# taylorlu/voicepuppet

Hardware: AMD Instinct MI355X
Metric: PixReferNet G+D step frames/sec @256x256 bs=32 (higher is better)
Workload: dtype bf16; 1 GPU; PixReferNet G+D training step (G + 3xD + VGG16-conv3_3 perceptual + TF-Adam x2), 256x256, ngf=ndf=64, global batch 32 = 32 per GPU; global_batch=32, per_gpu_batch=32, parallelism=dp1

## Files before the change

include/vp_hip.h:

```cpp
#ifndef VP_HIP_H_
#define VP_HIP_H_

#include <stddef.h>
#include <stdint.h>

#ifdef __cplusplus
extern "C" {
#endif

enum vp_status { VP_OK = 0, VP_ERR_ARG = -1, VP_ERR_HIP = -2, VP_ERR_WORKSPACE = -3, VP_ERR_STATE = -4 };
enum vp_dtype { VP_F32 = 0, VP_BF16 = 1 };
enum vp_act { VP_ACT_NONE = 0, VP_ACT_LRELU = 1, VP_ACT_RELU = 2, VP_ACT_TANH = 3, VP_ACT_SIGMOID = 4, VP_ACT_RELU6 = 5, VP_ACT_LEAKY = 6 };

int vp_version(void);
const char* vp_last_error(void);

typedef struct vp_pixrefer_desc {
  int batch;
  int height;
  int ngf, ndf;
  int dtype;
  int training;
  float l1_weight;
  float gan_weight;
// ... 97 lines not shown
  int batch, samples;
} vp_logmel_desc;
typedef struct vp_logmel vp_logmel_t;
size_t vp_logmel_workspace_bytes(const vp_logmel_desc* d);
int vp_logmel_frames(const vp_logmel_desc* d);
int vp_logmel_create(const vp_logmel_desc* d, void* workspace, size_t workspace_bytes, void* stream, vp_logmel_t** out);
void vp_logmel_destroy(vp_logmel_t* h);
int vp_logmel_forward(vp_logmel_t* h, const float* pcm, float* out, void* stream);

typedef struct vp_bfmnet_desc {
  int batch;
  int frames;
  int num_mel_bins;
  int trunk_dtype;
} vp_bfmnet_desc;
typedef struct vp_bfmnet vp_bfmnet_t;
size_t vp_bfmnet_param_count(void);
int vp_bfmnet_param_info(int index, char* name, int name_cap, size_t* offset, int* ndim, int64_t shape[4]);
size_t vp_bfmnet_workspace_bytes(const vp_bfmnet_desc* d);
int vp_bfmnet_create(const vp_bfmnet_desc* d, void* workspace, size_t workspace_bytes, const float* params,
                     void* stream, vp_bfmnet_t** out);
void vp_bfmnet_destroy(vp_bfmnet_t* h);
int vp_bfmnet_params_changed(vp_bfmnet_t* h);
int vp_bfmnet_forward(vp_bfmnet_t* h, const float* ears, const float* mfccs, const int* seq_len, float* out, void* stream);
int vp_bfmnet_set_decoder_dropout(vp_bfmnet_t* h, const float* mask0, const float* mask1);
int vp_bfmnet_tensor(vp_bfmnet_t* h, const char* name, void** ptr, int64_t shape[4]);

typedef struct vp_bfmstream_desc {
  int struct_bytes;
  int max_chunk_frames;
  int num_mel_bins;
  int trunk_dtype;
  int sample_rate;
  float lower_hz, upper_hz;
} vp_bfmstream_desc;
size_t vp_bfmstream_desc_size(void);
typedef struct vp_bfmstream vp_bfmstream_t;
int vp_bfmstream_context(const vp_bfmstream_desc* d, int* left_mel, int* right_mel, int* left_frames, int* right_frames, int* window_frames);
long long vp_bfmstream_frames_after(const vp_bfmstream_desc* d, long long samples, int finished);
size_t vp_bfmstream_workspace_bytes(const vp_bfmstream_desc* d);
int vp_bfmstream_create(const vp_bfmstream_desc* d, void* workspace, size_t workspace_bytes, const float* params, void* stream,
                        vp_bfmstream_t** out);
void vp_bfmstream_destroy(vp_bfmstream_t* h);
int vp_bfmstream_params_changed(vp_bfmstream_t* h);
int vp_bfmstream_reset(vp_bfmstream_t* h, void* stream);
int vp_bfmstream_ready(const vp_bfmstream_t* h, long long n_new_samples);
int vp_bfmstream_ready_finish(const vp_bfmstream_t* h);
int vp_bfmstream_push(vp_bfmstream_t* h, const float* pcm, long long n, const float* ears, float* coeff_out, void* stream);
int vp_bfmstream_finish(vp_bfmstream_t* h, const float* ears, float* coeff_out, void* stream);
int vp_bfmstream_tensor(vp_bfmstream_t* h, const char* name, void** ptr, int64_t shape[4]);
#define VP_BFMSTREAM_GROUP_MAX_SLOTS 128
typedef struct vp_bfmstream_group_desc {
  int struct_bytes;
  int slots;
  int max_chunk_frames;
  int num_mel_bins;
  int trunk_dtype;
  int sample_rate;
  float lower_hz, upper_hz;
} vp_bfmstream_group_desc;
size_t vp_bfmstream_group_desc_size(void);
typedef struct vp_bfmstream_group vp_bfmstream_group_t;
size_t vp_bfmstream_group_workspace_bytes(const vp_bfmstream_group_desc* d);
int vp_bfmstream_group_plan_info(const vp_bfmstream_group_desc* d, int bucket, int gemm, int info[8]);
int vp_bfmstream_group_create(const vp_bfmstream_group_desc* d, void* workspace, size_t workspace_bytes, const float* params, void* stream,
                              vp_bfmstream_group_t** out);
void vp_bfmstream_group_destroy(vp_bfmstream_group_t* h);
int vp_bfmstream_group_params_changed(vp_bfmstream_group_t* h);
int vp_bfmstream_group_reset_slot(vp_bfmstream_group_t* h, int slot, void* stream);
long long vp_bfmstream_group_ready(const vp_bfmstream_group_t* h, const long long* n, const int* finish, int* k);
int vp_bfmstream_group_push(vp_bfmstream_group_t* h, const float* pcm, const long long* n, const int* finish, const float* ears, float* coeff_out,
                            void* stream);
int vp_bfmstream_group_tensor(vp_bfmstream_group_t* h, const char* name, void** ptr, int64_t shape[4]);
int vp_gru_seq_state(const float* xg, const float* xc, const float* whg, const float* whc, float* hstate, float* out, int b, int t, int t0,
                     int n, void* stream);

int vp_maxpool2x2_fwd(const void* x, void* y, int n, int h, int w, int c, int dtype, void* stream);
int vp_maxpool2x2_bwd(const void* x, const void* dy, void* dx, int n, int h, int w, int c, int dtype, void* stream);
int vp_maxpool2x2_bwd_code(const void* code, const void* dy, void* dx, int n, int h, int w, int c, int dtype, void* stream);
int vp_composite_fwd(const float* gen_out4, const float* targets, float* out4, float* outputs, float* outputs_fg, int n, int hw,
                     void* stream);
int vp_gan_loss(const float* logits, void* seed_d, void* seed_g, float* predict, float* losses, int m, float gan_weight, int dtype,
                void* stream);
int vp_dwconv7x3_bn_act(const float* x, const float* w, const float* bias, float* y, int b, int h, int wd, int c, void* stream);
int vp_dwconv7x3_bn_act_t(const void* x, const float* w, const float* bias, void* y, int dtype, int b, int h, int wd, int c, void* stream);
int vp_conv_first_fwd(const float* x, const float* w, const float* bias, float* y, int b, int h, int w_in, int cout, void* stream);
size_t vp_dwproj_workspace_bytes(int ce, int cout);
int vp_dwproj_fwd(const float* ex, const float* w_dw, const float* b_dw, const float* w_proj, const float* b_proj, float* y, int add, int b, int h,
                  int w, int ce, int cout, void* workspace, void* stream);
int vp_maxpool_hw(const float* x, float* y, int b, int h, int w, int c, int kh, int kw, int sh, int sw, void* stream);
int vp_gru_seq(const float* xg, const float* xc, const float* whg, const float* whc, const int* seq_len, float* out, int b, int t,
               void* stream);

size_t vp_render_colors_workspace_bytes(int batch, int h, int w);
int vp_render_colors(unsigned char* image, unsigned char* face_mask, const float* vertices, const int* triangles,
                     const float* colors, float* depth_buffer, int ntri, int nver, int h, int w, int c, int batch,
                     void* workspace, void* stream);

typedef struct vp_bfm_model {
  int nver, ntri;
  const double* meanshape;
  const double* idBase;
  const double* exBase;
  const double* meantex;
  const double* texBase;
  const int* tri;
  const int* point_buf;
  double center[3];
  double focal, image_center;
  double sh[5];
} vp_bfm_model;
size_t vp_bfm_reconstruct_workspace_bytes(int nver, int ntri, int frames);
int vp_bfm_reconstruct(const vp_bfm_model* m, const float* coeff, const double* rotation, int frames, int shared_texture,
                       double* face_shape, double* face_texture, double* face_color, double* face_projection, double* z_buffer,
                       float* vertices, float* colors, void* workspace, size_t workspace_bytes, void* stream);
int vp_bfm_reconstruct_rows(const vp_bfm_model* m, const float* coeff, const double* rotation, int frames, const int* tex_src, int textures,
                            const int* tex_row, float* vertices, float* colors, void* workspace, size_t workspace_bytes, void* stream);

size_t vp_bn_train_workspace_bytes(size_t pixels, int c);
int vp_bn_train_fwd(const float* x, size_t pixels, int c, const float* beta, float eps, float* mean, float* var, float* rstd, float* scale,
                    float* shift, void* workspace, void* stream);
int vp_bn_train_bwd(const float* x, const float* dz, size_t pixels, int c, const float* mean, const float* rstd, float* dx, float* dbeta,
                    void* workspace, void* stream);
int vp_bn_act_train_bwd(const float* x, const float* da, size_t pixels, int c, const float* mean, const float* rstd, const float* shift, int act,
                        float* dx, float* dbeta, void* workspace, void* stream);
int vp_affine_act_fwd(const float* x, const float* scale, const float* shift, const float* mask, size_t pixels, int c, int act, float* y, void* stream);
int vp_affine_act_add_fwd(const float* x, const float* scale, const float* shift, const float* mask, const float* add, size_t pixels, int c, int act,
                          float* y, void* stream);
int vp_act_bwd(const float* dy, const float* ya, const float* mask, size_t n, int act, float* dx, void* stream);
int vp_dwconv7x3_raw(const float* x, const float* w, float* y, int b, int h, int wd, int c, void* stream);
int vp_dwconv7x3_bwd_data(const float* dy, const float* w, float* dx, int b, int h, int wd, int c, void* stream);
size_t vp_dwconv7x3_wgrad_workspace_bytes(int b, int h, int wd, int c);
int vp_dwconv7x3_wgrad(const float* x, const float* dy, float* dw, int b, int h, int wd, int c, void* workspace, void* stream);
int vp_maxpool_hw_bwd(const float* x, const float* dy, float* dx, int b, int h, int w, int c, int kh, int kw, int sh, int sw, void* stream);
int vp_stem_im2col(const float* x, float* col, int b, int h, int w, void* stream);
int vp_gru_train_fwd(const float* xg, const float* xc, const float* whg, const float* whc, const int* seq_len, float* out, float* r, float* u, float* c,
                     float* hprev, int b, int t, void* stream);
int vp_colsum_f32(const float* x, int rows, int cols, float* out, void* stream);
int vp_gru_split_recurrent(const float* gates_kernel, const float* cand_kernel, float* whg, float* whc, float* whg_t, float* whc_t, void* stream);
int vp_mul_f32(const float* a, const float* b, float* out, size_t n, void* stream);
int vp_add_ears_f32(float* out, const float* ears, int rows, void* stream);
int vp_gru_train_bwd(const float* dout, const float* whg_t, const float* whc_t, const int* seq_len, const float* r, const float* u, const float* c,
                     const float* hprev, float* dag, float* dac, int b, int t, void* stream);
int vp_vertex_loss_partials(int b, int j);
int vp_bfm_vertex_loss(const float* d, const float* vmask, const int* seq_len, int b, int t, int j, float* gd, double* partial, void* stream);
int vp_sumsq_partials(size_t n);
int vp_sumsq(const float* x, size_t n, double* partial, void* stream);
int vp_l2_regulariser(const float* params, const float* mask, float* grads, size_t n, float scale, double* partial, void* stream);
int vp_sum_f64(const double* partial, int n, double scale, const double* add, double* out, void* stream);
int vp_bfm_step_report(const double* loss_data, const double* reg, double half_l2, const double* sumsq, double* out3, void* stream);
int vp_clip_scale_f32(float* grads, size_t n, const double* sumsq, float clip, void* stream);
int vp_adam_tf_clipped(float* params, float* grads, float* m, float* v, size_t n, const float* lr_t, const double* sumsq, float clip, float beta1,
                       float beta2, float eps, void* stream);
int vp_moving_update(float* moving, const float* batch, const float* factor, size_t n, float decay, void* stream);

size_t vp_mm_workspace_bytes(int P, int K, int N);
int vp_mm_fwd_f32(const float* x, int ldx, const float* w, int ldw, int w_transposed, const float* bias, float* y, int ldy,
                  int P, int K, int N, void* workspace, void* stream);
int vp_mm_bwd_data_f32(const float* dy, int lddy, const float* w, int ldw, int w_transposed, float* dx, int lddx, int accumulate,
                       int P, int K, int N, void* workspace, void* stream);
int vp_mm_bwd_weight_f32(const float* x, int ldx, const float* dy, int lddy, float* dw, int P, int K, int k_real, int N,
                         void* workspace, void* stream);
size_t vp_mm_packed_bytes(int P, int K, int N, int dir);
size_t vp_mm_pack_desc_bytes(void);
int vp_mm_pack_desc(size_t w_off, int ldw, int w_transposed, int P, int K, int N, int dir, size_t dst_off, void* desc);
int vp_mm_pack_table(const void* device_descs, int n, const float* master, void* packed, void* stream);
// ... 81 lines not shown
```

voicepuppet_amd/_lib.py:

```python
import ctypes
import os

_HERE = os.path.dirname(os.path.abspath(__file__))
LIB_PATH = os.environ.get("VP_LIB", os.path.join(_HERE, "libvp_hip.so"))

VP_F32, VP_BF16 = 0, 1
ACT_NONE, ACT_LRELU, ACT_RELU, ACT_TANH, ACT_SIGMOID = 0, 1, 2, 3, 4


class PixReferDesc(ctypes.Structure):
  _fields_ = [("batch", ctypes.c_int), ("height", ctypes.c_int), ("ngf", ctypes.c_int), ("ndf", ctypes.c_int),
              ("dtype", ctypes.c_int), ("training", ctypes.c_int), ("l1_weight", ctypes.c_float),
              ("gan_weight", ctypes.c_float), ("per_sample_bn", ctypes.c_int),
              ("streams", ctypes.c_int), ("d_backward_fork", ctypes.c_int), ("d_beside_vgg", ctypes.c_int)]


class ConvDesc(ctypes.Structure):
  _fields_ = [("kind", ctypes.c_int), ("n", ctypes.c_int), ("h", ctypes.c_int), ("w", ctypes.c_int),
              ("cin", ctypes.c_int), ("cout", ctypes.c_int), ("ksize", ctypes.c_int), ("stride", ctypes.c_int),
              ("pad", ctypes.c_int), ("dtype", ctypes.c_int), ("in_act", ctypes.c_int), ("out_act", ctypes.c_int)]


class LogMelDesc(ctypes.Structure):
  _fields_ = [("sample_rate", ctypes.c_int), ("num_mel_bins", ctypes.c_int), ("win_length", ctypes.c_int),
# ... 112 lines not shown
    "vp_adam_tf": (ctypes.c_int, [_P, _P, _P, _P, ctypes.c_size_t, ctypes.c_int, ctypes.c_float, ctypes.c_float,
                                  ctypes.c_float, ctypes.c_float, _P]),
    "vp_conv_workspace_bytes": (ctypes.c_size_t, [ctypes.POINTER(ConvDesc)]),
    "vp_conv_fwd": (ctypes.c_int, [ctypes.POINTER(ConvDesc), _P, _P, _P, _P, _P, _P, _P, _P]),
    "vp_conv_bwd_data": (ctypes.c_int, [ctypes.POINTER(ConvDesc), _P, _P, _P, _P, _P]),
    "vp_conv_bwd_weight": (ctypes.c_int, [ctypes.POINTER(ConvDesc), _P, _P, _P, _P, _P, _P, _P]),
    "vp_conv3x3_c64_bwd_data_pooled_workspace_bytes": (ctypes.c_size_t, [ctypes.POINTER(ConvDesc)]),
    "vp_conv3x3_c64_bwd_data_pooled": (ctypes.c_int, [ctypes.POINTER(ConvDesc), _P, _P, _P, _P, _P, _P, ctypes.c_int, _P]),
    "vp_bn_workspace_bytes": (ctypes.c_size_t, [ctypes.c_int, ctypes.c_int, ctypes.c_int]),
    "vp_bn_stats": (ctypes.c_int, [_P, ctypes.c_int, ctypes.c_int, ctypes.c_int, _P, _P, ctypes.c_float, _P, _P, _P, _P, _P, _P]),
    "vp_logmel_workspace_bytes": (ctypes.c_size_t, [ctypes.POINTER(LogMelDesc)]),
    "vp_logmel_frames": (ctypes.c_int, [ctypes.POINTER(LogMelDesc)]),
    "vp_logmel_create": (ctypes.c_int, [ctypes.POINTER(LogMelDesc), _P, ctypes.c_size_t, _P, ctypes.POINTER(_P)]),
    "vp_logmel_destroy": (None, [_P]),
    "vp_logmel_forward": (ctypes.c_int, [_P, _P, _P, _P]),
    "vp_bfmnet_param_count": (ctypes.c_size_t, []),
    "vp_bfmnet_param_info": (ctypes.c_int, [ctypes.c_int, ctypes.c_char_p, ctypes.c_int, ctypes.POINTER(ctypes.c_size_t),
                                            ctypes.POINTER(ctypes.c_int), ctypes.POINTER(ctypes.c_int64)]),
    "vp_bfmnet_workspace_bytes": (ctypes.c_size_t, [ctypes.POINTER(BfmNetDesc)]),
    "vp_bfmnet_create": (ctypes.c_int, [ctypes.POINTER(BfmNetDesc), _P, ctypes.c_size_t, _P, _P, ctypes.POINTER(_P)]),
    "vp_bfmnet_destroy": (None, [_P]),
    "vp_bfmnet_params_changed": (ctypes.c_int, [_P]),
    "vp_bfmnet_forward": (ctypes.c_int, [_P, _P, _P, _P, _P, _P]),
    "vp_bfmnet_set_decoder_dropout": (ctypes.c_int, [_P, _P, _P]),
    "vp_bfmnet_tensor": (ctypes.c_int, [_P, ctypes.c_char_p, ctypes.POINTER(_P), ctypes.POINTER(ctypes.c_int64)]),
    "vp_bfmstream_desc_size": (ctypes.c_size_t, []),
    "vp_bfmstream_context": (ctypes.c_int, [ctypes.POINTER(BfmStreamDesc)] + [ctypes.POINTER(ctypes.c_int)] * 5),
    "vp_bfmstream_frames_after": (ctypes.c_longlong, [ctypes.POINTER(BfmStreamDesc), ctypes.c_longlong, ctypes.c_int]),
    "vp_bfmstream_workspace_bytes": (ctypes.c_size_t, [ctypes.POINTER(BfmStreamDesc)]),
    "vp_bfmstream_create": (ctypes.c_int, [ctypes.POINTER(BfmStreamDesc), _P, ctypes.c_size_t, _P, _P, ctypes.POINTER(_P)]),
    "vp_bfmstream_destroy": (None, [_P]),
    "vp_bfmstream_params_changed": (ctypes.c_int, [_P]),
    "vp_bfmstream_reset": (ctypes.c_int, [_P, _P]),
    "vp_bfmstream_ready": (ctypes.c_int, [_P, ctypes.c_longlong]),
    "vp_bfmstream_ready_finish": (ctypes.c_int, [_P]),
    "vp_bfmstream_push": (ctypes.c_int, [_P, _P, ctypes.c_longlong, _P, _P, _P]),
    "vp_bfmstream_finish": (ctypes.c_int, [_P, _P, _P, _P]),
    "vp_bfmstream_tensor": (ctypes.c_int, [_P, ctypes.c_char_p, ctypes.POINTER(_P), ctypes.POINTER(ctypes.c_int64)]),
    "vp_bfmstream_group_desc_size": (ctypes.c_size_t, []),
    "vp_puppet_desc_size": (ctypes.c_size_t, []),
    "vp_puppet_workspace_bytes": (ctypes.c_size_t, [ctypes.POINTER(PuppetDesc)]),
    "vp_puppet_create": (ctypes.c_int, [ctypes.POINTER(PuppetDesc), _P, ctypes.c_size_t, _P, ctypes.POINTER(_P)]),
    "vp_puppet_destroy": (None, [_P]),
    "vp_puppet_attach": (ctypes.c_int, [_P, ctypes.c_int, _P, _P, _P, ctypes.c_int, ctypes.c_int, ctypes.c_int, _P]),
    "vp_puppet_set_backgrounds": (ctypes.c_int, [_P, _P, ctypes.c_int]),
    "vp_puppet_splice": (ctypes.c_int, [_P, _P, ctypes.c_int, _P, ctypes.c_int, _P, _P]),
    "vp_puppet_condition": (ctypes.c_int, [_P, _P, ctypes.c_int, _P, ctypes.c_int, _P, _P, _P, _P]),
    "vp_puppet_tensor": (ctypes.c_int, [_P, ctypes.c_char_p, ctypes.POINTER(_P), ctypes.POINTER(ctypes.c_int64)]),
    "vp_puppet_slot_info": (ctypes.c_int, [_P, ctypes.c_int, ctypes.POINTER(ctypes.c_int)]),
    "vp_jpeg_desc_size": (ctypes.c_size_t, []),
    "vp_jpeg_workspace_bytes": (ctypes.c_size_t, [ctypes.POINTER(JpegDesc)]),
    "vp_jpeg_frame_capacity": (ctypes.c_size_t, [ctypes.POINTER(JpegDesc)]),
    "vp_jpeg_create": (ctypes.c_int, [ctypes.POINTER(JpegDesc), _P, ctypes.c_size_t, _P, ctypes.POINTER(_P)]),
    "vp_jpeg_encode": (ctypes.c_int, [_P, _P, ctypes.c_int, _P, ctypes.c_size_t, _P, _P]),
    "vp_jpeg_tensor": (ctypes.c_int, [_P, ctypes.c_char_p, ctypes.POINTER(_P), ctypes.POINTER(ctypes.c_int64)]),
    "vp_jpeg_header": (ctypes.c_int, [_P, _P, ctypes.c_size_t, ctypes.POINTER(ctypes.c_size_t)]),
    "vp_jpeg_destroy": (None, [_P]),
    "vp_pcmin_desc_size": (ctypes.c_size_t, []),
    "vp_pcmin_ratio": (ctypes.c_int, [ctypes.c_int, ctypes.c_int] + [ctypes.POINTER(ctypes.c_int)] * 4),
    "vp_pcmin_bank": (ctypes.c_int, [ctypes.c_int, ctypes.c_int, _P]),
    "vp_pcmin_samples_after": (ctypes.c_longlong, [ctypes.c_int, ctypes.c_int, ctypes.c_longlong, ctypes.c_int]),
    "vp_pcmin_workspace_bytes": (ctypes.c_size_t, [ctypes.POINTER(PcmInDesc)]),
    "vp_pcmin_create": (ctypes.c_int, [ctypes.POINTER(PcmInDesc), _P, ctypes.c_size_t, _P, ctypes.POINTER(_P)]),
    "vp_pcmin_destroy": (None, [_P]),
    "vp_pcmin_open_slot": (ctypes.c_int, [_P, ctypes.c_int, ctypes.c_int, ctypes.c_int, ctypes.c_int, _P]),
    "vp_pcmin_ready": (ctypes.c_longlong, [_P, ctypes.POINTER(ctypes.c_longlong), ctypes.POINTER(ctypes.c_int), ctypes.POINTER(ctypes.c_longlong)]),
    "vp_pcmin_push": (ctypes.c_int, [_P, _P, ctypes.POINTER(ctypes.c_longlong), ctypes.POINTER(ctypes.c_int), _P, _P]),
    "vp_bfm_reconstruct_rows": (ctypes.c_int, [ctypes.POINTER(BfmModel), _P, _P, ctypes.c_int, _P, ctypes.c_int, _P, _P, _P, _P, ctypes.c_size_t, _P]),
    "vp_bfmstream_group_workspace_bytes": (ctypes.c_size_t, [ctypes.POINTER(BfmStreamGroupDesc)]),
    "vp_bfmstream_group_plan_info": (ctypes.c_int, [ctypes.POINTER(BfmStreamGroupDesc), ctypes.c_int, ctypes.c_int, ctypes.POINTER(ctypes.c_int)]),
    "vp_bfmstream_group_create": (ctypes.c_int, [ctypes.POINTER(BfmStreamGroupDesc), _P, ctypes.c_size_t, _P, _P, ctypes.POINTER(_P)]),
    "vp_bfmstream_group_destroy": (None, [_P]),
    "vp_bfmstream_group_params_changed": (ctypes.c_int, [_P]),
    "vp_bfmstream_group_reset_slot": (ctypes.c_int, [_P, ctypes.c_int, _P]),
    "vp_bfmstream_group_ready": (ctypes.c_longlong, [_P, ctypes.POINTER(ctypes.c_longlong), ctypes.POINTER(ctypes.c_int), ctypes.POINTER(ctypes.c_int)]),
    "vp_bfmstream_group_push": (ctypes.c_int, [_P, _P, ctypes.POINTER(ctypes.c_longlong), ctypes.POINTER(ctypes.c_int), _P, _P, _P]),
    "vp_bfmstream_group_tensor": (ctypes.c_int, [_P, ctypes.c_char_p, ctypes.POINTER(_P), ctypes.POINTER(ctypes.c_int64)]),
    "vp_gru_seq_state": (ctypes.c_int, [_P, _P, _P, _P, _P, _P, ctypes.c_int, ctypes.c_int, ctypes.c_int, ctypes.c_int, _P]),
    "vp_maxpool2x2_fwd": (ctypes.c_int, [_P, _P, ctypes.c_int, ctypes.c_int, ctypes.c_int, ctypes.c_int, ctypes.c_int, _P]),
    "vp_maxpool2x2_bwd": (ctypes.c_int, [_P, _P, _P, ctypes.c_int, ctypes.c_int, ctypes.c_int, ctypes.c_int, ctypes.c_int, _P]),
    "vp_maxpool2x2_bwd_code": (ctypes.c_int, [_P, _P, _P, ctypes.c_int, ctypes.c_int, ctypes.c_int, ctypes.c_int, ctypes.c_int, _P]),
    "vp_composite_fwd": (ctypes.c_int, [_P, _P, _P, _P, _P, ctypes.c_int, ctypes.c_int, _P]),
    "vp_gan_loss": (ctypes.c_int, [_P, _P, _P, _P, _P, ctypes.c_int, ctypes.c_float, ctypes.c_int, _P]),
    "vp_dwconv7x3_bn_act": (ctypes.c_int, [_P, _P, _P, _P, ctypes.c_int, ctypes.c_int, ctypes.c_int, ctypes.c_int, _P]),
    "vp_dwconv7x3_bn_act_t": (ctypes.c_int, [_P, _P, _P, _P] + [ctypes.c_int] * 5 + [_P]),
    "vp_conv_first_fwd": (ctypes.c_int, [_P, _P, _P, _P] + [ctypes.c_int] * 4 + [_P]),
    "vp_dwproj_workspace_bytes": (ctypes.c_size_t, [ctypes.c_int, ctypes.c_int]),
    "vp_dwproj_fwd": (ctypes.c_int, [_P] * 6 + [ctypes.c_int] * 6 + [_P, _P]),
    "vp_maxpool_hw": (ctypes.c_int, [_P, _P, ctypes.c_int, ctypes.c_int, ctypes.c_int, ctypes.c_int, ctypes.c_int, ctypes.c_int, ctypes.c_int,
                                     ctypes.c_int, _P]),
    "vp_gru_seq": (ctypes.c_int, [_P, _P, _P, _P, _P, _P, ctypes.c_int, ctypes.c_int, _P]),
    "vp_bfm_reconstruct_workspace_bytes": (ctypes.c_size_t, [ctypes.c_int, ctypes.c_int, ctypes.c_int]),
    "vp_bfm_reconstruct": (ctypes.c_int, [_P, _P, _P, ctypes.c_int, ctypes.c_int, _P, _P, _P, _P, _P, _P, _P, _P, ctypes.c_size_t, _P]),
    "vp_render_colors_workspace_bytes": (ctypes.c_size_t, [ctypes.c_int, ctypes.c_int, ctypes.c_int]),
    "vp_render_colors": (ctypes.c_int, [_P, _P, _P, _P, _P, _P, ctypes.c_int, ctypes.c_int, ctypes.c_int, ctypes.c_int, ctypes.c_int,
                                        ctypes.c_int, _P, _P]),
    "vp_bn_train_workspace_bytes": (ctypes.c_size_t, [ctypes.c_size_t, ctypes.c_int]),
    "vp_bn_train_fwd": (ctypes.c_int, [_P, ctypes.c_size_t, ctypes.c_int, _P, ctypes.c_float, _P, _P, _P, _P, _P, _P, _P]),
    "vp_bn_train_bwd": (ctypes.c_int, [_P, _P, ctypes.c_size_t, ctypes.c_int, _P, _P, _P, _P, _P, _P]),
    "vp_affine_act_fwd": (ctypes.c_int, [_P, _P, _P, _P, ctypes.c_size_t, ctypes.c_int, ctypes.c_int, _P, _P]),
    "vp_affine_act_add_fwd": (ctypes.c_int, [_P, _P, _P, _P, _P, ctypes.c_size_t, ctypes.c_int, ctypes.c_int, _P, _P]),
    "vp_act_bwd": (ctypes.c_int, [_P, _P, _P, ctypes.c_size_t, ctypes.c_int, _P, _P]),
    "vp_dwconv7x3_raw": (ctypes.c_int, [_P, _P, _P, ctypes.c_int, ctypes.c_int, ctypes.c_int, ctypes.c_int, _P]),
    "vp_dwconv7x3_bwd_data": (ctypes.c_int, [_P, _P, _P, ctypes.c_int, ctypes.c_int, ctypes.c_int, ctypes.c_int, _P]),
    "vp_dwconv7x3_wgrad_workspace_bytes": (ctypes.c_size_t, [ctypes.c_int, ctypes.c_int, ctypes.c_int, ctypes.c_int]),
    "vp_bn_act_train_bwd": (ctypes.c_int, [_P, _P, ctypes.c_size_t, ctypes.c_int, _P, _P, _P, ctypes.c_int, _P, _P, _P, _P]),
    "vp_l2_regulariser": (ctypes.c_int, [_P, _P, _P, ctypes.c_size_t, ctypes.c_float, _P, _P]),
    "vp_adam_tf_clipped": (ctypes.c_int, [_P, _P, _P, _P, ctypes.c_size_t, _P, _P, ctypes.c_float, ctypes.c_float, ctypes.c_float, ctypes.c_float, _P]),
    "vp_moving_update": (ctypes.c_int, [_P, _P, _P, ctypes.c_size_t, ctypes.c_float, _P]),
    "vp_dwconv7x3_wgrad": (ctypes.c_int, [_P, _P, _P, ctypes.c_int, ctypes.c_int, ctypes.c_int, ctypes.c_int, _P, _P]),
    "vp_maxpool_hw_bwd": (ctypes.c_int, [_P, _P, _P] + [ctypes.c_int] * 8 + [_P]),
    "vp_stem_im2col": (ctypes.c_int, [_P, _P, ctypes.c_int, ctypes.c_int, ctypes.c_int, _P]),
    "vp_gru_train_fwd": (ctypes.c_int, [_P] * 10 + [ctypes.c_int, ctypes.c_int, _P]),
    "vp_gru_train_bwd": (ctypes.c_int, [_P] * 10 + [ctypes.c_int, ctypes.c_int, _P]),
    "vp_colsum_f32": (ctypes.c_int, [_P, ctypes.c_int, ctypes.c_int, _P, _P]),
    "vp_gru_split_recurrent": (ctypes.c_int, [_P] * 7),
    "vp_mul_f32": (ctypes.c_int, [_P, _P, _P, ctypes.c_size_t, _P]),
    "vp_add_ears_f32": (ctypes.c_int, [_P, _P, ctypes.c_int, _P]),
    "vp_vertex_loss_partials": (ctypes.c_int, [ctypes.c_int, ctypes.c_int]),
    "vp_bfm_vertex_loss": (ctypes.c_int, [_P, _P, _P, ctypes.c_int, ctypes.c_int, ctypes.c_int, _P, _P, _P]),
    "vp_sumsq_partials": (ctypes.c_int, [ctypes.c_size_t]),
    "vp_sum_f64": (ctypes.c_int, [_P, ctypes.c_int, ctypes.c_double, _P, _P, _P]),
    "vp_bfm_step_report": (ctypes.c_int, [_P, _P, ctypes.c_double, _P, _P, _P]),
    "vp_clip_scale_f32": (ctypes.c_int, [_P, ctypes.c_size_t, _P, ctypes.c_float, _P]),
    "vp_sumsq": (ctypes.c_int, [_P, ctypes.c_size_t, _P, _P]),
    "vp_bn_bwd": (ctypes.c_int, [_P, _P, _P, ctypes.c_int, ctypes.c_int, ctypes.c_int, _P, _P, _P, _P, _P, _P, _P]),
}

_lib = None


def lib():
  global _lib
  if _lib is None:
    if not os.path.exists(LIB_PATH):
      raise RuntimeError("libvp_hip.so is missing (%s): run `python -c 'import __graft_entry__ as g; g.build()'` "
                         "or `make -C voicepuppet_amd/csrc`.  There is no CPU fallback." % LIB_PATH)
    try:
      import torch
    except ImportError:
      pass
    l = ctypes.CDLL(LIB_PATH)
    for name, (res, args) in _SIGNATURES.items():
      try:
        fn = getattr(l, name)
      except AttributeError:
        if "VP_LIB" not in os.environ:
          raise
        continue
      fn.restype = res
      fn.argtypes = args
    if hasattr(l, "vp_pixrefer_desc_size") and l.vp_pixrefer_desc_size.argtypes is not None:
      want = int(l.vp_pixrefer_desc_size())
      if want != ctypes.sizeof(PixReferDesc):
        raise RuntimeError("%s: vp_pixrefer_desc is %d bytes in the library, %d in this binding" % (LIB_PATH, want, ctypes.sizeof(PixReferDesc)))
    if hasattr(l, "vp_bfmstream_desc_size") and l.vp_bfmstream_desc_size.argtypes is not None:
      want = int(l.vp_bfmstream_desc_size())
      if want != ctypes.sizeof(BfmStreamDesc):
        raise RuntimeError("%s: vp_bfmstream_desc is %d bytes in the library, %d in this binding" % (LIB_PATH, want, ctypes.sizeof(BfmStreamDesc)))
    if hasattr(l, "vp_bfmstream_group_desc_size") and l.vp_bfmstream_group_desc_size.argtypes is not None:
      want = int(l.vp_bfmstream_group_desc_size())
      if want != ctypes.sizeof(BfmStreamGroupDesc):
        raise RuntimeError("%s: vp_bfmstream_group_desc is %d bytes in the library, %d in this binding" % (LIB_PATH, want, ctypes.sizeof(BfmStreamGroupDesc)))
    if hasattr(l, "vp_puppet_desc_size") and l.vp_puppet_desc_size.argtypes is not None:
      want = int(l.vp_puppet_desc_size())
      if want != ctypes.sizeof(PuppetDesc):
# ... 21 lines not shown
```

voicepuppet_amd/csrc/conv_ops.h:

```cpp
#pragma once
#include <stdlib.h>
#include <string.h>

#include "launch.h"

namespace vp {

struct ConvGeomX : ConvGeom {
  int CoutT;
};

inline ConvGeomX make_geom(int kind, int ks, int stride, int pad, int N, int Hin, int Win, int Cin, int Cin_real, int Cout) {
  ConvGeomX g;
  g.kind = kind; g.ks = ks; g.stride = stride; g.pad = pad;
  g.N = N; g.Hin = Hin; g.Win = Win;
  if (kind == 0) { g.Hout = (Hin + 2 * pad - ks) / stride + 1; g.Wout = (Win + 2 * pad - ks) / stride + 1; }
  else { g.Hout = 2 * Hin; g.Wout = 2 * Win; }
  g.Cin = Cin; g.Cin_real = Cin_real; g.Cout = Cout;
  g.CoutT = Cout < 8 ? 8 : Cout;
  return g;
}

inline int kc_elems(int is_bf16) { return is_bf16 ? 32 : 16; }

// ... 11 lines not shown
    if (rows % 64 == 0) return 1;
    if (rows <= 16) return 2;
    return rows > 64 ? 0 : 1;
  }
  if (rows <= 64) return 5;
  return P > 16 ? 3 : 4;
}

constexpr int IGEMM_SPLITK_TARGET_DEFAULT = 64;
inline int& igemm_splitk_target_knob() { static int v = IGEMM_SPLITK_TARGET_DEFAULT; return v; }
inline int pick_igemm_splitk(int blocks, int nchunk) {
  const int target = igemm_splitk_target_knob();
  const int cap = plan_misc_knob(1);
  const int minchunk = plan_misc_knob(2);
  if (blocks >= 256 || blocks >= target) return 1;
  int s = (target + blocks - 1) / blocks;
  if (s > nchunk / minchunk) s = nchunk / minchunk;
  if (s > cap) s = cap;
  return s < 1 ? 1 : s;
}

inline void set_single_src(PixSrc& x, const void* p, int C, const float* a, const float* b, int act, int group_n) {
  x.ptr[0] = p; x.ptr[1] = nullptr; x.C[0] = C; x.C[1] = 0;
  x.aff_a[0] = a; x.aff_b[0] = b; x.aff_a[1] = nullptr; x.aff_b[1] = nullptr;
  x.act = act; x.group_n = group_n > 0 ? group_n : (1 << 30);
}

struct LaunchForm {
  bool bias = false, ref = false, xa_lrelu = false, xa_relu = false, x_affine = false;
  bool stats = false;
  int x_act = 0, ref_act = 0;
};

struct IgemmPlan {
  IgemmArgs a;
  int cfg;
  LaunchForm form;
  PackDesc pack;
  size_t pack_elems;
  size_t partial_bytes;
};

struct IgemmPin { int cfg, splitk; };

inline void finish_igemm(IgemmPlan& p, int rows, int is_bf16, const IgemmPin* pin = nullptr) {
  IgemmArgs& a = p.a;
  const int P = a.N * a.Hg * a.Wg;
  a.Kpad = round_up(a.ntaps * a.Cin, kc_elems(is_bf16));
  p.cfg = pick_igemm_cfg(rows, P, a.Kpad);
  if (!is_bf16 && a.ntaps == 1 && p.cfg == 0) {
    const long long b128 = (long long)((P + 127) / 128) * (rows / 128), b64 = 2 * b128;
    if (((b64 + 255) / 256) * 64 < ((b128 + 255) / 256) * 128) p.cfg = 1;
  }
  if (pin) p.cfg = pin->cfg;
  int bc, bp;
  igemm_tile(p.cfg, &bc, &bp);
  a.CoutPad = round_up(rows, bc);
  if (a.ntaps == 1) { a.log2Cin = 30; a.cin_mask = 0x3fffffff; }
  else { a.log2Cin = ilog2(a.Cin); a.cin_mask = a.Cin - 1; }
  const int blocks = ((P + bp - 1) / bp) * (a.CoutPad / bc) * a.nclass;
  a.splitk = pin ? pin->splitk : pick_igemm_splitk(blocks, a.Kpad / kc_elems(is_bf16));
  p.partial_bytes = a.splitk > 1 ? (size_t)a.nclass * a.splitk * P * a.CoutPad * sizeof(float) : 0;
  {
    const bool tc4 = p.cfg == 0 || p.cfg == 1 || p.cfg == 6 || p.cfg == 7 || p.cfg == 8 || p.cfg == 9;
    a.rowperm = (tc4 && rows % 64 == 0) ? 1 : 0;
    p.pack.perm = a.rowperm;
  }
  a.wp_rows = round_up(rows, 128);
  p.pack.rows_pad = a.wp_rows;
  p.pack.Kpad = a.Kpad;
  p.pack.kc = kc_elems(is_bf16);
  p.pack_elems = (size_t)a.nclass * a.wp_rows * a.Kpad;
}

inline int& patch_tiles_knob() { static int v = 7; return v; }
inline int& patch_small_knob() { static int v = 3; return v; }
inline int& patch_longk_knob() { static int v = 1; return v; }
inline int& patch3_knob() { static int v = 1; return v; }
inline int& wgrad_big_knob() { static int v = 1; return v; }
inline int& patch4_knob() { static int v = 1; return v; }
inline int& c64_knob() { static int v = 1; return v; }
inline int& pool_bwd_fused_knob() { static int v = 1; return v; }
inline int& cout1_knob() { static int v = 256; return v; }
inline int& wgrad1_rows_knob() { static int v = 512; return v; }
inline int& dc64_knob() { static int v = 1; return v; }
inline int& s2c64_knob() { static int v = 512; return v; }
inline int& s2c64_pair_knob() { static int v = 1; return v; }
constexpr int PATCH_MIN_BLOCKS_DEFAULT = 192;
inline int& patch_minblk_knob() { static int v = PATCH_MIN_BLOCKS_DEFAULT; return v; }

inline void patch_tile_hw(int bp, int* th, int* tw) { *th = bp == 128 ? 8 : 16; *tw = bp == 512 ? 32 : 16; }
inline int patch_tile_pixels(int bc) {
  const int k = patch_small_knob();
  if (bc == 256) return (k & 2) ? 128 : 256;
  return (k & 1) ? 256 : 512;
}

inline int patch_tile_rows(int rows, int on) {
  if ((on & 1) && rows % 256 == 0) return 256;
  if ((on & 2) && rows % 128 == 0) return 128;
  if ((on & 4) && rows % 64 == 0) return 64;
  return 0;
}

inline bool plan_patch_eligible(const IgemmPlan& p, int rows, int is_bf16, bool single_src, bool any_grid = false) {
  const int on = patch_tiles_knob();
  const int minblk = any_grid ? 0 : patch_minblk_knob();
  const IgemmArgs& a = p.a;
  const int kc = kc_elems(is_bf16);
  if (!on || !single_src || a.nclass != 1 || a.sh != 1 || a.sw != 1 || a.os != 1 || a.ntaps < 9 || a.Cin % kc || a.Cin < kc) return false;
  if (rows % 64 || a.Cout % 8 || a.ldY % 8 || a.Hg < 16 || a.Wg < 16 || a.Hof != a.Hg || a.Wof != a.Wg) return false;
  const bool p4 = patch4_knob() && is_bf16 && a.ntaps == 16 && rows % 128 == 0;
  if (!p4 && patch_longk_knob() && rows >= 512 && rows % 256 == 0 && a.ntaps * a.Cin >= 4096 && (long long)a.N * a.Hg * a.Wg >= 256 * 256) return false;
  const int bc = p4 ? 128 : patch_tile_rows(rows, on);
  if (!bc) return false;
  int th, tw;
  patch_tile_hw(p4 ? 256 : patch_tile_pixels(bc), &th, &tw);
  const long long blocks = (long long)a.N * ((a.Hg + th - 1) / th) * ((a.Wg + tw - 1) / tw) * (rows / bc);
  const long long p4min = (long long)a.ntaps * a.Cin >= 8192 ? 256 : 512;
  if (p4 && !any_grid && patch_minblk_knob() > 1) {
    if (blocks < p4min) return false;
  } else if (blocks < minblk) return false;
  if ((size_t)a.N * a.Hin * a.Win * a.Cin * (is_bf16 ? 2 : 4) >= 0x70000000ull) return false;
  int ks = 0;
  while (ks * ks < a.ntaps) ++ks;
  if (ks * ks != a.ntaps) return false;
  const int sh = a.taps[0].dh[ks] - a.taps[0].dh[0], sw = a.taps[0].dw[1] - a.taps[0].dw[0];
  if ((sh != 1 && sh != -1) || (sw != 1 && sw != -1)) return false;
  for (int t = 0; t < a.ntaps; ++t)
    if (a.taps[0].dh[t] != a.taps[0].dh[0] + (t / ks) * sh || a.taps[0].dw[t] != a.taps[0].dw[0] + (t % ks) * sw) return false;
  return true;
}
inline void plan_make_patch(IgemmPlan& p, int rows, int is_bf16) {
  IgemmArgs& a = p.a;
  const bool p4 = patch4_knob() && is_bf16 && a.ntaps == 16 && rows % 128 == 0;
  const int bc = p4 ? 128 : patch_tile_rows(rows, patch_tiles_knob());
  int ks = 0;
  while (ks * ks < a.ntaps) ++ks;
  a.kern = CK_PATCH; a.p_kw = ks;
  a.p_dhf = a.taps[0].dh[0]; a.p_dwf = a.taps[0].dw[0];
  a.p_dhs = a.taps[0].dh[ks] - a.taps[0].dh[0]; a.p_dws = a.taps[0].dw[1] - a.taps[0].dw[0];
  const int bp = p4 ? 256 : patch_tile_pixels(bc);
  p.cfg = bc == 256 ? (bp == 128 ? 15 : 10) : (bc == 128 ? (bp == 256 ? 13 : 11) : (bp == 256 ? 14 : 12));
  a.CoutPad = round_up(rows, bc);
  a.splitk = 1;
  p.partial_bytes = 0;
  a.rowperm = 1;
  p.pack.perm = 1;
  p.pack.kswap = 1;
}

inline int& patch_xcd_knob() { static int v = 0; return v; }
inline int& patch2_knob() { static int v = 1; return v; }
inline bool plan_patch2_eligible(const IgemmPlan& p, int rows, int is_bf16, int c0, int c1) {
  const IgemmArgs& a = p.a;
  const int kc = kc_elems(is_bf16);
  if (!patch2_knob() || a.nclass != 4 || a.ntaps != 4 || a.os != 2 || a.sh != 1 || a.sw != 1) return false;
  if (c0 + c1 != a.Cin || c0 % (2 * kc) || c1 % (2 * kc) || c0 < 2 * kc) return false;
  if (rows % 64 || rows > 128 || a.Cout % 8 || a.ldY % 8 || a.Hg < 16 || a.Wg < 16 || a.Hof != 2 * a.Hg || a.Wof != 2 * a.Wg) return false;
  const long long blocks = (long long)a.N * ((a.Hg + 15) / 16) * ((a.Wg + 15) / 16) * 4;
  if (blocks < patch_minblk_knob()) return false;
  const size_t cmax = c0 > c1 ? c0 : c1;
  if ((size_t)a.N * a.Hin * a.Win * cmax * (is_bf16 ? 2 : 4) >= 0x70000000ull) return false;
  for (int cls = 0; cls < 4; ++cls)
    for (int t = 0; t < 4; ++t)
      if (a.taps[cls].dh[t] != a.taps[cls].dh[3] + 1 - (t >> 1) || a.taps[cls].dw[t] != a.taps[cls].dw[3] + 1 - (t & 1)) return false;
// ... 280 lines not shown
```

voicepuppet_amd/csrc/launch.h:

```cpp
#pragma once
#include <hip/hip_runtime.h>

#include "conv_args.h"
#include "pointwise_args.h"

namespace vp {

hipError_t launch_igemm(const IgemmArgs& a, int is_bf16, int cfg, hipStream_t st);
void igemm_tile(int cfg, int* bc, int* bp);
hipError_t launch_igemm_patch(const IgemmArgs& a, int is_bf16, int bc, int bp, hipStream_t st);
bool patch3_eligible(const IgemmArgs& a, int is_bf16);
hipError_t launch_igemm_patch3(const IgemmArgs& a, int is_bf16, int bc, int bp, hipStream_t st);
bool patch4_eligible(const IgemmArgs& a, int is_bf16);
hipError_t launch_igemm_patch4(const IgemmArgs& a, hipStream_t st);
bool conv_cin8_eligible(const IgemmArgs& a, int is_bf16);
bool conv_cout8_eligible(const IgemmArgs& a, int is_bf16);
bool conv_dcout8_eligible(const IgemmArgs& a, int is_bf16);
bool conv_cout4_eligible(const IgemmArgs& a, int is_bf16);
bool conv_kernel_ok(const IgemmArgs& a, int is_bf16);
const char* conv_kernel_name(int kern);
bool conv_c64_eligible(const IgemmArgs& a, int is_bf16);
hipError_t launch_conv_c64(const IgemmArgs& a, hipStream_t st);
bool conv_dc64_eligible(const IgemmArgs& a, int is_bf16);
hipError_t launch_conv_dc64(const IgemmArgs& a, hipStream_t st);
int conv_dc64_grid(const IgemmArgs& a);
bool conv_dc256_eligible(const IgemmArgs& a, int is_bf16);
int conv_dc256_grid(const IgemmArgs& a);
hipError_t launch_conv_dc256(const IgemmArgs& a, hipStream_t st);
bool conv_s2c64_eligible(const IgemmArgs& a, int is_bf16);
int conv_s2c64_grid(const IgemmArgs& a);
int conv_s2c64_tiles_per_image(const IgemmArgs& a);
hipError_t launch_conv_s2c64(const IgemmArgs& a, hipStream_t st);
bool conv_cout1_bwd_eligible(const Cout1Args& a);
hipError_t launch_conv_cout1_bwd(const Cout1Args& a, hipStream_t st);
bool conv_cout1_wgrad_eligible(const Cout1Args& a);
hipError_t launch_conv_cout1_wgrad(const Cout1Args& a, hipStream_t st);
hipError_t launch_cout1_wgrad_prof(const Cout1Args& a, hipStream_t st);
hipError_t launch_cout1_bwd_prof(const Cout1Args& a, hipStream_t st);
hipError_t launch_igemm_patch2(const IgemmArgs& a, int is_bf16, int bc, int bp, hipStream_t st);
hipError_t launch_igemm_smallp(const IgemmArgs& a, int is_bf16, hipStream_t st);
struct SmallPArgs;
hipError_t launch_smallp(const SmallPArgs& s, int is_bf16, hipStream_t st);
hipError_t launch_smallp_fused(const SmallPArgs& s, int is_bf16, hipStream_t st);
hipError_t launch_wgrad(const WgradArgs& a, int is_bf16, int cfg, hipStream_t st);
bool wgrad_mm_eligible(const WgradArgs& a, int cfg);
hipError_t launch_wgrad_mm(const WgradArgs& a, int cfg, hipStream_t st);
hipError_t launch_wgrad_tr(const WgradArgs& a, hipStream_t st, const char** variant = nullptr, int* tile_cols = nullptr);
void wgrad_tile(int cfg, int* bm, int* bn);

void profile_enable(int on);
void profile_tag(const char* tag);
size_t profile_collect(char* out, size_t cap);

hipError_t launch_pack_weights(const PackDesc* d_descs, int ndesc, const float* master, void* packed, int is_bf16, hipStream_t st);
hipError_t launch_pack_weights_one(const PackDesc& d, const float* master, void* packed, int is_bf16, hipStream_t st);
int bn_nchunk(int Pg, int C, int G, int is_bf16);
hipError_t launch_bn_stats(const BnArgs& a, int is_bf16, hipStream_t st);
hipError_t launch_bn_finalize(const BnArgs& a, hipStream_t st);
bool bn_small(const BnArgs& a);
hipError_t launch_bn_small_fwd(const BnArgs& a, void* out_lrelu, void* out_relu, int is_bf16, hipStream_t st);
hipError_t launch_bn_small_bwd(const BnArgs& a, int is_bf16, hipStream_t st);
hipError_t launch_bn_bwd(const BnArgs& a, int is_bf16, hipStream_t st);
hipError_t launch_bn_bwd_tail(const BnArgs& a, int is_bf16, hipStream_t st);
hipError_t launch_colsum(const BnArgs& a, int creal, float* out, int accumulate, int is_bf16, hipStream_t st);
hipError_t launch_colsum_tail(const BnArgs& a, int creal, float* out, int accumulate, hipStream_t st);
hipError_t launch_act_apply(const void* y, const float* sc, const float* sh, int C, int Pg, size_t npix,
                            void* out_lrelu, void* out_relu, int is_bf16, hipStream_t st);
hipError_t launch_tap_gather(const TapArgs& a, hipStream_t st);
hipError_t launch_tap_spread(const TapArgs& a, int is_bf16, hipStream_t st);
hipError_t launch_frame_pack(const FramePackArgs& a, hipStream_t st);
hipError_t launch_pack_inputs(const PackInputsArgs& a, int is_bf16, hipStream_t st);
int composite_nblocks(int N, int HW);
hipError_t launch_composite_fwd(const CompositeArgs& a, int is_bf16, hipStream_t st);
hipError_t launch_composite_bwd(const CompositeArgs& a, int is_bf16, hipStream_t st);
hipError_t launch_gan_loss(const GanLossArgs& a, int is_bf16, hipStream_t st);
int perceptual_nblocks(size_t half, int is_bf16);
hipError_t launch_perceptual(const PerceptualArgs& a, int is_bf16, hipStream_t st);
hipError_t launch_loss_final(const LossFinalArgs& a, hipStream_t st);
hipError_t launch_maxpool_fwd(const void* x, void* y, int B, int H, int W, int C, int is_bf16, hipStream_t st);
hipError_t launch_maxpool_bwd(const void* x, const void* dy, void* dx, int B, int H, int W, int C, int is_bf16, hipStream_t st);
hipError_t launch_maxpool_bwd_code(const void* code, const void* dy, void* dx, int B, int H, int W, int C, int is_bf16, hipStream_t st);
hipError_t launch_relu_bwd(const void* y, void* d, size_t n, int is_bf16, hipStream_t st);
hipError_t launch_adam(const AdamArgs& a, hipStream_t st);
hipError_t launch_fetch(const FetchArgs& a, hipStream_t st);
hipError_t launch_grad_pack_bf16(const float* src, void* dst, size_t n, hipStream_t st);
hipError_t launch_grad_unpack_bf16(const void* src, float* dst, size_t n, float scale, hipStream_t st);

struct ConvGeom {
  int kind;
  int ks, stride, pad;
  int N, Hin, Win, Hout, Wout;
  int Cin, Cin_real;
  int Cout;
};

inline int ilog2(int v) { int l = 0; while ((1 << l) < v) ++l; return l; }
inline int round_up(int v, int m) { return (v + m - 1) / m * m; }

}
```

voicepuppet_amd/csrc/ops_api.hip:

```cpp
#include <string.h>

#include <string>

#include "conv_ops.h"
#include "errors.h"
#include "audio_args.h"
#include "launch.h"
#include "vp_common.h"

using namespace vp;

namespace {

bool conv_desc_ok(const vp_conv_desc* d) {
  if (!d || d->n < 1 || d->h < 1 || d->w < 1) return false;
  if (d->cin < 8 || (d->cin & (d->cin - 1))) return false;
  if (d->kind == 1 && (d->ksize != 4 || d->stride != 2 || d->pad != 1)) return false;
  if (d->kind != 0 && d->kind != 1) return false;
  if (d->ksize < 1 || d->ksize > 4 || d->stride < 1 || d->stride > 2) return false;
  if (d->kind == 0 && d->stride == 2 && (d->ksize != 4 || d->pad != 1 || (d->h & 1) || (d->w & 1))) return false;
  return d->dtype == VP_F32 || d->dtype == VP_BF16;
}

ConvGeomX geom_of(const vp_conv_desc* d) {
  return make_geom(d->kind, d->ksize, d->stride, d->pad, d->n, d->h, d->w, d->cin, d->cin, d->cout);
}

size_t align256(size_t v) { return (v + 255) & ~(size_t)255; }

const void* zero_page(char* ws, size_t used, hipStream_t st) {
  char* z = ws + align256(used);
  (void)hipMemsetAsync(z, 0, 256, st);
  return z;
}

}

extern "C" {

int vp_pixrefer_pack_frames(const unsigned char* example_frames, const unsigned char* current_frames, const int* crops,
                            int n, int img_size, float* inputs, float* fg_inputs, float* targets, float* masks, void* stream) {
  if (!example_frames || !current_frames || !crops || !inputs || !fg_inputs || !targets || !masks || n < 1 || img_size < 2) {
    set_err("vp_pixrefer_pack_frames: bad argument");
    return VP_ERR_ARG;
  }
  FramePackArgs a;
  a.ex = example_frames; a.cur = current_frames; a.crops = crops;
  a.inputs = inputs; a.fg_inputs = fg_inputs; a.targets = targets; a.masks = masks;
  a.N = n; a.S = img_size;
  VP_HIP_CHECK(launch_frame_pack(a, (hipStream_t)stream));
  return VP_OK;
}

extern "C" void vp_phase_marks_enable(int on);

int vp_tune(const char* key, int value) {
  if (!key) return VP_ERR_ARG;
  const std::string k(key);
  if (k == "patch_tiles") { patch_tiles_knob() = value; return VP_OK; }
  if (k == "patch_min_blocks") { patch_minblk_knob() = value < 0 ? PATCH_MIN_BLOCKS_DEFAULT : value; return VP_OK; }
  if (k == "patch_small_tiles") { patch_small_knob() = value; return VP_OK; }
  if (k == "patch_long_k_on_256") { patch_longk_knob() = value; return VP_OK; }
  if (k == "wgrad_tr") { wgrad_tr_knob() = value; return VP_OK; }
  if (k == "patch3") { patch3_knob() = value; return VP_OK; }
  if (k == "c64") { c64_knob() = value; return VP_OK; }
  if (k == "dc64") { dc64_knob() = value; return VP_OK; }
  if (k == "pool_bwd_fused") { pool_bwd_fused_knob() = value < 0 || value > 4 ? 1 : value; return VP_OK; }
  if (k == "cout1_wgrad_rows" && value > 0) { wgrad1_rows_knob() = value; return VP_OK; }
  if (k == "cout1_bwd") { cout1_knob() = value < 0 ? 256 : value; return VP_OK; }
  if (k == "s2c64") { s2c64_knob() = value; return VP_OK; }
  if (k == "wgrad_big") { wgrad_big_knob() = value; return VP_OK; }
  if (k == "patch4") { patch4_knob() = value; return VP_OK; }
  if (k == "s2c64_pair") { s2c64_pair_knob() = value; return VP_OK; }
  if (k == "bfm_dwproj") { bfm_dwproj_knob() = value; return VP_OK; }
  if (k == "patch2") { patch2_knob() = value; return VP_OK; }
  if (k == "patch_xcd") { patch_xcd_knob() = value; return VP_OK; }
  if (k == "smallp_max_pixels") { smallp_knob() = value; return VP_OK; }
  if (k == "igemm_splitk_target") { igemm_splitk_target_knob() = value < 0 ? IGEMM_SPLITK_TARGET_DEFAULT : value; return VP_OK; }
  if (k == "wgrad_fixed_x10") { wgrad_cost_knob(0) = value; return VP_OK; }
  if (k == "wgrad_slab_tile_x1000") { wgrad_cost_knob(2) = value < 0 ? 150 : value; return VP_OK; }
  if (k == "wgrad_slab_x100") { wgrad_cost_knob(1) = value; return VP_OK; }
  if (k == "smallp_split_target") { plan_misc_knob(0) = value; return VP_OK; }
  if (k == "igemm_splitk_cap") { plan_misc_knob(1) = value; return VP_OK; }
  if (k == "igemm_splitk_minchunk") { plan_misc_knob(2) = value; return VP_OK; }
  if (k == "wgrad_resident_blocks") { plan_misc_knob(3) = value; return VP_OK; }
  if (k == "igemm_small_grid") { igemm_small_grid_knob() = value; return VP_OK; }
  if (k == "thin_blocks_cout8" && value > 0) { thin_blocks_knob(0) = value; return VP_OK; }
  if (k == "thin_blocks_dcout8" && value > 0) { thin_blocks_knob(1) = value; return VP_OK; }
  if (k == "thin_blocks_cout4" && value > 0) { thin_blocks_knob(2) = value; return VP_OK; }
  if (k == "thin_blocks_cin8" && value > 0) { thin_blocks_knob(3) = value; return VP_OK; }
  if (k == "phase_marks") { vp_phase_marks_enable(value); return VP_OK; }
  set_err("vp_tune: unknown key %s", key);
  return VP_ERR_ARG;
}

static unsigned* smallp_counter_page(char* ws, size_t used, const IgemmArgs& a, hipStream_t st) {
  unsigned* c = (unsigned*)(ws + align256(used) + 256);
  (void)hipMemsetAsync(c, 0, (size_t)smallp_counters(a) * sizeof(unsigned), st);
  return c;
}

size_t vp_conv_workspace_bytes(const vp_conv_desc* d) {
  if (!conv_desc_ok(d)) return 0;
  const int bf = d->dtype == VP_BF16, es = bf ? 2 : 4;
  const ConvGeomX g = geom_of(d);
  size_t best = 0;
  {
    IgemmPlan p = plan_fwd(g, 0, bf);
    best = align256(p.pack_elems * es) + p.partial_bytes;
    plan_kernel(p, g.Cout, bf, d->cin, 0, FAM_SMALLP, LaunchForm{});
    if (p.a.kern == CK_SMALLP) {
      const size_t b = align256(p.pack_elems * es) + align256(p.partial_bytes) + 512 + (size_t)smallp_counters(p.a) * sizeof(unsigned);
      if (b > best) best = b;
    }
  }
  if ((d->cout & (d->cout - 1)) == 0 && d->cout >= 8) {
    IgemmPlan p = plan_bwd_data(g, 0, 0, d->cin, d->cin, d->cin, bf);
    size_t b = align256(p.pack_elems * es) + p.partial_bytes;
    if (b > best) best = b;
    plan_kernel(p, d->cin, bf, d->cout, 0, FAM_SMALLP, LaunchForm{});
    if (p.a.kern == CK_SMALLP) {
      b = align256(p.pack_elems * es) + align256(p.partial_bytes) + 512 + (size_t)smallp_counters(p.a) * sizeof(unsigned);
      if (b > best) best = b;
    }
    for (int plain = 0; plain < 2; ++plain) {
      WgradPlan w = plan_wgrad(g, bf, plain != 0);
      if (w.partial_bytes + 512 > best) best = w.partial_bytes + 512;
    }
  }
  return best + 1024;
}

int vp_conv_fwd(const vp_conv_desc* d, const void* x, const float* in_scale, const float* in_shift,
                const float* w, const float* bias, void* y, void* workspace, void* stream) {
  if (!conv_desc_ok(d) || !x || !w || !y || !workspace) { set_err("vp_conv_fwd: bad argument"); return VP_ERR_ARG; }
  const int bf = d->dtype == VP_BF16, es = bf ? 2 : 4;
  hipStream_t st = (hipStream_t)stream;
  const ConvGeomX g = geom_of(d);
  IgemmPlan p = plan_fwd(g, 0, bf);
  p.a.out_act = d->out_act;
  LaunchForm f;
  f.bias = bias != nullptr; f.x_affine = in_scale != nullptr; f.x_act = d->in_act;
  const bool plain = d->in_act == ACT_NONE && !in_scale;
  plan_kernel(p, g.Cout, bf, d->cin, 0, plain ? (FAM_SMALLP | FAM_PATCH | FAM_PATCH2 | (d->out_act == ACT_NONE ? FAM_S2C64 : 0)) : 0, f);
  char* ws = (char*)workspace;
  VP_HIP_CHECK(launch_pack_weights_one(p.pack, w, ws, bf, st));
  IgemmArgs a = p.a;
  set_single_src(a.x, x, d->cin, in_scale, in_shift, d->in_act, 0);
  a.Wp = ws;
  a.partial = (float*)(ws + align256(p.pack_elems * es));
  a.Y = y; a.bias = bias;
  a.zeros = zero_page(ws, align256(p.pack_elems * es) + p.partial_bytes, st);
// ... 95 lines not shown

static bool bn_ok(int pixels, int c, int dtype) {
  const int e = dtype == VP_BF16 ? 8 : 4;
  return pixels >= 1 && c >= e && c % e == 0 && 256 % (c / e) == 0 && (dtype == VP_F32 || dtype == VP_BF16);
}

int vp_bn_stats(const void* y, int pixels, int c, int dtype, const float* gamma, const float* beta, float eps,
                float* scale, float* shift, float* mean, float* rstd, void* workspace, void* stream) {
  if (!bn_ok(pixels, c, dtype) || !y || !gamma || !beta || !scale || !shift || !mean || !rstd || !workspace) {
    set_err("vp_bn_stats: bad argument");
    return VP_ERR_ARG;
  }
  BnArgs b;
  memset(&b, 0, sizeof(b));
  b.y = y; b.C = c; b.G = 1; b.Pg = pixels;
  b.nchunk = bn_nchunk(pixels, c, 1, dtype == VP_BF16);
  b.partial = (double*)workspace;
  b.gamma = gamma; b.beta = beta; b.aff_a = scale; b.aff_b = shift; b.mu = mean; b.rstd = rstd; b.eps = eps;
  VP_HIP_CHECK(launch_bn_stats(b, dtype == VP_BF16, (hipStream_t)stream));
  return VP_OK;
}

int vp_bn_bwd(const void* y, const void* dz, void* dy, int pixels, int c, int dtype, const float* gamma,
              const float* mean, const float* rstd, float* dgamma, float* dbeta, void* workspace, void* stream) {
  if (!bn_ok(pixels, c, dtype) || !y || !dz || !dy || !gamma || !mean || !rstd || !dgamma || !dbeta || !workspace) {
    set_err("vp_bn_bwd: bad argument");
    return VP_ERR_ARG;
  }
  BnArgs b;
  memset(&b, 0, sizeof(b));
  b.y = y; b.dz = dz; b.dy = dy; b.C = c; b.G = 1; b.Pg = pixels;
  b.nchunk = bn_nchunk(pixels, c, 1, dtype == VP_BF16);
  b.partial = (double*)workspace;
  float* f = (float*)((char*)workspace + (size_t)b.nchunk * 2 * c * sizeof(double));
  b.c1 = f; b.c2 = f + c;
  b.gamma = gamma; b.mu = const_cast<float*>(mean); b.rstd = const_cast<float*>(rstd);
  b.dgamma = dgamma; b.dbeta = dbeta;
  VP_HIP_CHECK(launch_bn_bwd(b, dtype == VP_BF16, (hipStream_t)stream));
  return VP_OK;
}


int vp_maxpool2x2_fwd(const void* x, void* y, int n, int h, int w, int c, int dtype, void* stream) {
  const int e = dtype == VP_BF16 ? 8 : 4;
  if (!x || !y || n < 1 || h < 2 || w < 2 || (h & 1) || (w & 1) || c < e || c % e) { set_err("vp_maxpool2x2_fwd: bad argument"); return VP_ERR_ARG; }
  VP_HIP_CHECK(launch_maxpool_fwd(x, y, n, h, w, c, dtype == VP_BF16, (hipStream_t)stream));
  return VP_OK;
}

int vp_maxpool2x2_bwd(const void* x, const void* dy, void* dx, int n, int h, int w, int c, int dtype, void* stream) {
  const int e = dtype == VP_BF16 ? 8 : 4;
  if (!x || !dy || !dx || n < 1 || h < 2 || w < 2 || (h & 1) || (w & 1) || c < e || c % e) { set_err("vp_maxpool2x2_bwd: bad argument"); return VP_ERR_ARG; }
  VP_HIP_CHECK(launch_maxpool_bwd(x, dy, dx, n, h, w, c, dtype == VP_BF16, (hipStream_t)stream));
  return VP_OK;
}

int vp_maxpool2x2_bwd_code(const void* code, const void* dy, void* dx, int n, int h, int w, int c, int dtype, void* stream) {
  const int e = dtype == VP_BF16 ? 8 : 4;
  if (!code || !dy || !dx || n < 1 || h < 2 || w < 2 || (h & 1) || (w & 1) || c < e || c % e) { set_err("vp_maxpool2x2_bwd_code: bad argument"); return VP_ERR_ARG; }
  VP_HIP_CHECK(launch_maxpool_bwd_code(code, dy, dx, n, h, w, c, dtype == VP_BF16, (hipStream_t)stream));
  return VP_OK;
}

int vp_composite_fwd(const float* gen_out4, const float* targets, float* out4, float* outputs, float* outputs_fg, int n, int hw,
                     void* stream) {
  if (!gen_out4 || !targets || !out4 || !outputs || !outputs_fg || n < 1 || hw < 1) { set_err("vp_composite_fwd: bad argument"); return VP_ERR_ARG; }
  CompositeArgs ca;
  memset(&ca, 0, sizeof(ca));
  ca.y4 = gen_out4; ca.targets = targets; ca.o4 = out4; ca.outputs = outputs; ca.outputs_fg = outputs_fg; ca.N = n; ca.HW = hw; ca.train = 0;
  VP_HIP_CHECK(launch_composite_fwd(ca, 0, (hipStream_t)stream));
  return VP_OK;
}

int vp_gan_loss(const float* logits, void* seed_d, void* seed_g, float* predict, float* losses, int m, float gan_weight, int dtype,
                void* stream) {
  if (!logits || !seed_d || !seed_g || !predict || !losses || m < 1) { set_err("vp_gan_loss: bad argument"); return VP_ERR_ARG; }
  GanLossArgs ga;
  memset(&ga, 0, sizeof(ga));
  ga.logits = logits; ga.dl_d = seed_d; ga.dl_g = seed_g; ga.predict = predict; ga.losses = losses; ga.M = m; ga.gan_weight = gan_weight;
  VP_HIP_CHECK(launch_gan_loss(ga, dtype == VP_BF16, (hipStream_t)stream));
  return VP_OK;
}

int vp_dwconv7x3_bn_act(const float* x, const float* w, const float* bias, float* y, int b, int h, int wd, int c, void* stream) {
  if (!x || !w || !bias || !y || b < 1 || h < 1 || wd < 1 || c < 4 || (c & 3)) { set_err("vp_dwconv7x3_bn_act: bad argument"); return VP_ERR_ARG; }
  VP_HIP_CHECK(launch_dwconv7x3(x, w, bias, y, 0, b, h, wd, c, (hipStream_t)stream));
  return VP_OK;
}

int vp_dwconv7x3_bn_act_t(const void* x, const float* w, const float* bias, void* y, int dtype, int b, int h, int wd, int c, void* stream) {
  if (!x || !w || !bias || !y || b < 1 || h < 1 || wd < 1 || c < 4 || (c & 3) || (dtype != VP_F32 && dtype != VP_BF16)) {
    set_err("vp_dwconv7x3_bn_act_t: bad argument"); return VP_ERR_ARG;
  }
  VP_HIP_CHECK(launch_dwconv7x3(x, w, bias, y, dtype == VP_BF16, b, h, wd, c, (hipStream_t)stream));
  return VP_OK;
}

int vp_conv_first_fwd(const float* x, const float* w, const float* bias, float* y, int b, int h, int w_in, int cout, void* stream) {
  if (!x || !w || !bias || !y || b < 1 || h < 1 || w_in < 1 || cout < 1) { set_err("vp_conv_first_fwd: bad argument"); return VP_ERR_ARG; }
  int pt, ho, pl, wo;
  same_pad(h, 9, 1, &pt, &ho);
  same_pad(w_in, 5, 2, &pl, &wo);
  VP_HIP_CHECK(launch_conv_first(x, w, bias, y, 0, b, h, w_in, wo, cout, pt, pl, (hipStream_t)stream));
  return VP_OK;
}

static IgemmPlan dwproj_pack_plan(int pixels, int ce, int cout) {
  IgemmPlan p = plan_fwd(make_geom(0, 1, 1, 0, 1, pixels, 1, ce, ce, cout), 0, 0);
  p.pack.s_ch = cout;
  p.pack.dst_off = 0;
  p.pack.perm = 0; p.a.rowperm = 0;
  return p;
}

size_t vp_dwproj_workspace_bytes(int ce, int cout) {
  if (ce < 16 || ce % 16 || cout < 1) return 0;
  return align256((size_t)22 * ce * sizeof(float)) + align256(dwproj_pack_plan(1, ce, cout).pack_elems * sizeof(float)) + 256;
}

int vp_dwproj_fwd(const float* ex, const float* w_dw, const float* b_dw, const float* w_proj, const float* b_proj, float* y, int add, int b, int h,
                  int w, int ce, int cout, void* workspace, void* stream) {
  if (!ex || !w_dw || !b_dw || !w_proj || !b_proj || !y || !workspace || b < 1 || h < 1 || w < 1) { set_err("vp_dwproj_fwd: bad argument"); return VP_ERR_ARG; }
  if (!dwproj_eligible(w, ce, cout)) {
    set_err("vp_dwproj_fwd: no kernel for mel width %d, %d expanded and %d output channels (dwproj_eligible)", w, ce, cout);
    return VP_ERR_ARG;
  }
  const size_t ex_bytes = (size_t)b * h * w * ce * sizeof(float);
  if (ex_bytes >= 0xF0000000ull) {
    set_err("vp_dwproj_fwd: the expanded tensor is %zu bytes, the kernel's 32-bit lane offsets stop below 0xF0000000 (%llu)", ex_bytes, 0xF0000000ull);
    return VP_ERR_ARG;
  }
  hipStream_t st = (hipStream_t)stream;
  float* wdw22 = (float*)workspace;
  float* packed = (float*)((char*)workspace + align256((size_t)22 * ce * sizeof(float)));
  VP_HIP_CHECK(hipMemcpyAsync(wdw22, w_dw, (size_t)21 * ce * sizeof(float), hipMemcpyDeviceToDevice, st));
  VP_HIP_CHECK(hipMemcpyAsync(wdw22 + (size_t)21 * ce, b_dw, (size_t)ce * sizeof(float), hipMemcpyDeviceToDevice, st));
  const IgemmPlan p = dwproj_pack_plan(b * h * w, ce, cout);
  VP_HIP_CHECK(launch_pack_weights_one(p.pack, w_proj, packed, 0, st));
  VP_HIP_CHECK(launch_dwproj(ex, wdw22, packed, p.a.wp_rows, b_proj, y, add ? 1 : 0, b, h, w, ce, cout, st));
  return VP_OK;
}

int vp_maxpool_hw(const float* x, float* y, int b, int h, int w, int c, int kh, int kw, int sh, int sw, void* stream) {
  if (!x || !y || b < 1 || h < 1 || w < 1 || c < 4 || (c & 3) || kh < 1 || kw < 1 || sh < 1 || sw < 1) { set_err("vp_maxpool_hw: bad argument"); return VP_ERR_ARG; }
  const int ho = (h + sh - 1) / sh, wo = (w + sw - 1) / sw;
  const int ph = (ho - 1) * sh + kh - h, pw = (wo - 1) * sw + kw - w;
  const int pt = ph > 0 ? ph / 2 : 0, pl = pw > 0 ? pw / 2 : 0;
  VP_HIP_CHECK(launch_maxpool_same(x, y, 0, 0, b, h, w, c, kh, kw, sh, sw, pt, pl, ho, wo, (hipStream_t)stream));
  return VP_OK;
}

int vp_gru_seq(const float* xg, const float* xc, const float* whg, const float* whc, const int* seq_len, float* out, int b, int t,
               void* stream) {
  if (!xg || !xc || !whg || !whc || !seq_len || !out || b < 1 || t < 1) { set_err("vp_gru_seq: bad argument"); return VP_ERR_ARG; }
  VP_HIP_CHECK(launch_gru_seq(xg, xc, whg, whc, seq_len, out, b, t, (hipStream_t)stream));
  return VP_OK;
}

int vp_gru_seq_state(const float* xg, const float* xc, const float* whg, const float* whc, float* hstate, float* out, int b, int t, int t0,
                     int n, void* stream) {
  if (!xg || !xc || !whg || !whc || !hstate || !out || b < 1 || t < 1 || t0 < 0 || n < 0 || t0 + n > t) {
    set_err("vp_gru_seq_state: bad argument"); return VP_ERR_ARG;
  }
  if (n == 0) return VP_OK;
  VP_HIP_CHECK(launch_gru_state(xg, xc, whg, whc, hstate, out, b, t, t0, n, (hipStream_t)stream));
  return VP_OK;
// ... 13 lines not shown
```

voicepuppet_amd/csrc/plan_pixrefer.hip:

```cpp
#include <math.h>
#include <stdio.h>
#include <string.h>

#include <mutex>
#include <string>
#include <utility>
#include <vector>

#include "conv_ops.h"
#include "errors.h"
#include "launch.h"
#include "smallp_args.h"
#include "vp_common.h"

namespace vp {

thread_local char g_err[512] = "";
void set_err(const char* fmt, ...) {
  va_list ap;
  va_start(ap, fmt);
  vsnprintf(g_err, sizeof(g_err), fmt, ap);
  va_end(ap);
}

// ... 28 lines not shown
  bool dz2_written = false;
  void* xa[3] = {nullptr, nullptr, nullptr};
  bool need_act[3] = {false, false, false};
  BnBuf bn{};
  int producer = -1;
  int n_bwd_consumers = 0;
  int dz_writes = 0;
  bool bn_bwd_done = false;
  bool hi = false;
  void* dz32 = nullptr;
  double* cs_part = nullptr;
  int cs_chunks = 0;
  int pb_cap = 0, pbg_cap = 0;
  int bst_chunks = 0, bst_chunks_g = 0;
  size_t elems() const { return (size_t)N * H * W * C; }
};

struct Layer {
  std::string scope;
  ConvGeomX g;
  int src[2] = {-1, -1};
  int nsrc = 1;
  int in_act = ACT_NONE;
  int out_act = ACT_NONE;
  int out = -1;
  bool has_bn = false;
  size_t w_off = 0, b_off = 0, gamma_off = 0, beta_off = 0;
  size_t pk_fwd = 0, pk_bwd[2] = {0, 0}, pk_bwd_alt[2] = {0, 0};
  bool need_bwd[2] = {false, false};
  IgemmPlan fwd, bwd[2], bwd_alt[2];
  IgemmPlan bwd_pair;
  size_t pk_bwd_pair = 0;
  bool has_pair = false;
  IgemmPlan fwd_half;
  size_t pk_fwd_half = 0;
  bool has_fwd_half = false;
  WgradPlan wg;
  size_t desc0 = 0, desc1 = 0;
  bool tapgemm = false;
  bool fwd_stats = false;
  float* tap_S = nullptr;
  void* tap_dyS = nullptr;
  unsigned* sp_cnt_fwd = nullptr;
  unsigned* sp_cnt_bwd[2] = {nullptr, nullptr};
  unsigned* sp_cnt_pair = nullptr;
};

struct ParamInfo { std::string name; size_t off; int ndim; int64_t shape[4]; };

struct Net {
  std::vector<Tens> t;
  std::vector<Layer> l;
  std::vector<ParamInfo> manifest;
  size_t nparams = 0;
  int batch = 0, groups = 1;
  float* params = nullptr;
  float* grads = nullptr;
  char* packed = nullptr;
  size_t packed_elems = 0;
  std::vector<PackDesc> descs;
  PackDesc* d_descs = nullptr;
  unsigned* sp_cnt = nullptr;
  size_t sp_cnt_n = 0;
};

}

using namespace vp;

struct vp_pixrefer {
  vp_pixrefer_desc d;
  int bf16, es;
  Net G, D, V;
  void *gin, *gfg, *din, *vin;
  float *y4, *o4, *outputs, *outputs_fg, *logits, *predict, *losses;
  void *dl_d, *dl_g, *d_din, *d_vin, *dy4, *df3;
  void *vpool1, *vpool2, *d_vpool1, *d_vpool2;
  unsigned char* vpool_code[2];
  bool pool_codes_written;
  bool pool_fuse_ok[2];
  bool pool_bwd_fused;
  bool pool_dz_stale[2];
  double *comp_partial, *perc_partial, *bn_partial;
  char* scratch;
  char* scratch2;
  double* bn_partial2;
  char* scratch3;
  double* bn_partial3;
  char* scratch4;
  double* bn_partial4;
  hipStream_t side, branch;
  hipStream_t branch2;
  hipEvent_t ev_b2join;
  bool use_b2;
  hipEvent_t ev_fork, ev_join, ev_bfork, ev_bjoin;
  hipEvent_t ev_upd_b, ev_upd_m;
  bool overlap, forked;
  int bst_count;
  int bst_on;
  int vgg_fork_layer;
  bool store_first_raw;
  bool ov_on;
  int dfork_point;
  bool dsplit_on;
  hipEvent_t mark[64];
  int nmark;
  bool marks_made;
  int dfork_pending;
  void* zeros;
  size_t scratch_bytes;
  int n_comp, n_perc;
  struct { bool active, d_done; float *m_g, *v_g, *m_d, *v_d; float lr_t_g, lr_t_d, beta1, beta2, eps; } upd;
  int upd_mask;
  bool params_dirty;
  bool vgg_dirty;
  const float *in_targets, *in_masks;
};

namespace vp {

static int add_tensor(Net& n, const std::string& name, int N, int H, int W, int C, bool has_bn, bool is_input) {
  Tens t;
  t.name = name; t.N = N; t.H = H; t.W = W; t.C = C; t.has_bn = has_bn; t.is_input = is_input;
  n.t.push_back(t);
  return (int)n.t.size() - 1;
}

static void add_param(Net& n, const std::string& name, std::initializer_list<int64_t> shape, size_t* off_out) {
  ParamInfo p;
  p.name = name; p.off = n.nparams; p.ndim = (int)shape.size();
  size_t cnt = 1;
  int i = 0;
  for (auto s : shape) { p.shape[i++] = s; cnt *= (size_t)s; }
  for (; i < 4; ++i) p.shape[i] = 1;
  *off_out = n.nparams;
  n.nparams += cnt;
  n.manifest.push_back(p);
}

static int add_layer(Net& n, const std::string& prefix, const std::string& scope, int kind, int ks, int stride, int pad,
                     std::initializer_list<int> srcs, int cin_real, int cout, bool has_bn, int in_act, int out_act,
                     const char* wname, const char* bname) {
  Layer L;
  L.scope = scope;
  L.nsrc = 0;
  int cin = 0;
  for (int s : srcs) {
    L.src[L.nsrc++] = s; cin += n.t[s].C;
    if (in_act != ACT_NONE) n.t[s].need_act[in_act] = true;
  }
  const Tens& t0 = n.t[L.src[0]];
  L.g = make_geom(kind, ks, stride, pad, n.batch, t0.H, t0.W, cin, cin_real, cout);
  L.in_act = in_act; L.out_act = out_act; L.has_bn = has_bn;
  const std::string base = prefix + scope + "/";
  if (kind == 0) add_param(n, base + wname, {ks, ks, cin_real, cout}, &L.w_off);
  else add_param(n, base + wname, {4, 4, cout, cin_real}, &L.w_off);
  add_param(n, base + bname, {cout}, &L.b_off);
  if (has_bn) {
    add_param(n, base + "batch_normalization/gamma", {cout}, &L.gamma_off);
    add_param(n, base + "batch_normalization/beta", {cout}, &L.beta_off);
  }
  L.out = add_tensor(n, scope, n.batch, L.g.Hout, L.g.Wout, L.g.CoutT, has_bn, false);
  n.t[L.out].producer = (int)n.l.size();
  n.l.push_back(L);
  return L.out;
}

static void build_generator(Net& n, int N, int H, int ngf, int groups = 1) {
  n.batch = N; n.groups = groups;
  const int tin = add_tensor(n, "inputs", N, H, H, 8, false, true);
  const int tfg = add_tensor(n, "fg_inputs", N, H, H, 8, false, true);
  const char* CK = "conv2d/kernel"; const char* CB = "conv2d/bias";
  const char* DK = "conv2d_transpose/kernel"; const char* DB = "conv2d_transpose/bias";
  const std::string P = "generator/";
  int e1 = add_layer(n, P, "encoder_1", 0, 4, 2, 1, {tin}, 6, ngf, false, ACT_NONE, ACT_NONE, CK, CB);
  int e2 = add_layer(n, P, "encoder_2", 0, 4, 2, 1, {e1}, ngf, ngf * 2, true, ACT_LRELU, ACT_NONE, CK, CB);
  int e3 = add_layer(n, P, "encoder_3", 0, 4, 2, 1, {e2}, ngf * 2, ngf * 2, true, ACT_LRELU, ACT_NONE, CK, CB);
  int e4 = add_layer(n, P, "encoder_4", 0, 4, 2, 1, {e3}, ngf * 2, ngf * 4, true, ACT_LRELU, ACT_NONE, CK, CB);
  int f1 = add_layer(n, P, "encoder_fg_1", 0, 4, 2, 1, {tfg}, 3, ngf, false, ACT_NONE, ACT_NONE, CK, CB);
  int f2 = add_layer(n, P, "encoder_fg_2", 0, 4, 2, 1, {f1}, ngf, ngf * 2, true, ACT_LRELU, ACT_NONE, CK, CB);
  int f3 = add_layer(n, P, "encoder_fg_3", 0, 4, 2, 1, {f2}, ngf * 2, ngf * 2, true, ACT_LRELU, ACT_NONE, CK, CB);
  int f4 = add_layer(n, P, "encoder_fg_4", 0, 4, 2, 1, {f3}, ngf * 2, ngf * 4, true, ACT_LRELU, ACT_NONE, CK, CB);
  int m2 = add_layer(n, P, "merged_encoder_2", 0, 4, 2, 1, {e4, f4}, ngf * 8, ngf * 4, true, ACT_LRELU, ACT_NONE, CK, CB);
  int m3 = add_layer(n, P, "merged_encoder_3", 0, 4, 2, 1, {m2}, ngf * 4, ngf * 8, true, ACT_LRELU, ACT_NONE, CK, CB);
  int m4 = add_layer(n, P, "merged_encoder_4", 0, 4, 2, 1, {m3}, ngf * 8, ngf * 8, true, ACT_LRELU, ACT_NONE, CK, CB);
  int m5 = add_layer(n, P, "merged_encoder_5", 0, 4, 2, 1, {m4}, ngf * 8, ngf * 8, true, ACT_LRELU, ACT_NONE, CK, CB);
  int d5 = add_layer(n, P, "merged_decoder_5", 1, 4, 2, 1, {m5}, ngf * 8, ngf * 8, true, ACT_RELU, ACT_NONE, DK, DB);
  int d4 = add_layer(n, P, "merged_decoder_4", 1, 4, 2, 1, {d5, m4}, ngf * 16, ngf * 8, true, ACT_RELU, ACT_NONE, DK, DB);
  int d3 = add_layer(n, P, "merged_decoder_3", 1, 4, 2, 1, {d4, m3}, ngf * 16, ngf * 4, true, ACT_RELU, ACT_NONE, DK, DB);
  int d2 = add_layer(n, P, "merged_decoder_2", 1, 4, 2, 1, {d3, m2}, ngf * 8, ngf * 4, true, ACT_RELU, ACT_NONE, DK, DB);
  int c4 = add_layer(n, P, "merged2_decoder_4", 1, 4, 2, 1, {d2, e4}, ngf * 8, ngf * 2, true, ACT_RELU, ACT_NONE, DK, DB);
  int c3 = add_layer(n, P, "merged2_decoder_3", 1, 4, 2, 1, {c4, e3}, ngf * 4, ngf * 2, true, ACT_RELU, ACT_NONE, DK, DB);
  int c2 = add_layer(n, P, "merged2_decoder_2", 1, 4, 2, 1, {c3, e2}, ngf * 4, ngf, true, ACT_RELU, ACT_NONE, DK, DB);
  add_layer(n, P, "decoder_1", 1, 4, 2, 1, {c2, e1}, ngf * 2, 4, false, ACT_RELU, ACT_NONE, DK, DB);
// ... 206 lines not shown
  }
}

static void carve_net(Net& n, Arena& ar, int es, bool training) {
  for (Tens& t : n.t) {
    if (t.name == "decoder_1" || t.name == "layer_5") {
      continue;
    }
    if (!t.is_input) t.y = ar.alloc(t.elems() * (t.hi ? sizeof(float) : (size_t)es));
    for (int k = 1; k < 3; ++k) if (t.need_act[k]) t.xa[k] = ar.alloc(t.elems() * es);
    if (t.has_bn) {
      const size_t gc = (size_t)n.groups * t.C * sizeof(float);
      t.bn.a = (float*)ar.alloc(gc); t.bn.b = (float*)ar.alloc(gc);
      t.bn.mu = (float*)ar.alloc(gc); t.bn.rstd = (float*)ar.alloc(gc);
      t.bn.c1 = (float*)ar.alloc(gc); t.bn.c2 = (float*)ar.alloc(gc);
      t.bn.c1g = (float*)ar.alloc(gc); t.bn.c2g = (float*)ar.alloc(gc);
      t.bn.pb = (training && t.pb_cap) ? (double*)ar.alloc((size_t)n.groups * t.pb_cap * 2 * t.C * sizeof(double)) : nullptr;
      t.bn.pbg = (training && t.pbg_cap) ? (double*)ar.alloc((size_t)t.pbg_cap * 2 * t.C * sizeof(double)) : nullptr;
    }
  }
  for (Layer& L : n.l) {
    if (!L.tapgemm) continue;
    const size_t q = (size_t)L.g.N * L.g.Hin * L.g.Win * 16;
    L.tap_S = (float*)ar.alloc(q * sizeof(float));
    L.tap_dyS = ar.alloc(q * es);
  }
  n.packed = (char*)ar.alloc(n.packed_elems * es);
  n.d_descs = (PackDesc*)ar.alloc(n.descs.size() * sizeof(PackDesc));
  n.sp_cnt = (unsigned*)ar.alloc((n.sp_cnt_n + 1) * sizeof(unsigned));
  {
    unsigned* c = n.sp_cnt;
    for (Layer& L : n.l) {
      if (L.fwd.a.kern == CK_SMALLP) { L.sp_cnt_fwd = c; c += c ? smallp_counters(L.fwd.a) : 0; }
      for (int s = 0; s < L.nsrc && training; ++s)
        if (L.need_bwd[s] && L.bwd[s].a.kern == CK_SMALLP) { L.sp_cnt_bwd[s] = c; c += c ? smallp_counters(L.bwd[s].a) : 0; }
      if (training && L.has_pair && L.bwd_pair.a.kern == CK_SMALLP) { L.sp_cnt_pair = c; c += c ? smallp_counters(L.bwd_pair.a) : 0; }
    }
  }
}

static size_t carve_all(vp_pixrefer* h, char* base, size_t cap, std::vector<std::pair<size_t, size_t>>* track = nullptr) {
  Arena ar{base, 0, cap};
  ar.track = track;
  const vp_pixrefer_desc& d = h->d;
  const int N = d.batch, H = d.height, es = h->es;
  const size_t px = (size_t)N * H * H;
  h->gin = ar.alloc(px * 8 * es);
  h->gfg = ar.alloc(px * 8 * es);
  h->y4 = (float*)ar.alloc(px * 4 * sizeof(float));
  h->o4 = (float*)ar.alloc(px * 4 * sizeof(float));
  h->outputs = (float*)ar.alloc(px * 3 * sizeof(float));
  h->outputs_fg = (float*)ar.alloc(px * 3 * sizeof(float));
  h->losses = (float*)ar.alloc(8 * sizeof(float));
  h->G.t[0].y = h->gin; h->G.t[1].y = h->gfg;
  carve_net(h->G, ar, es, d.training);
  if (d.training) {
    const int hd = H / 8 - 2;
    const size_t M = (size_t)N * hd * hd;
    h->din = ar.alloc(3 * px * 8 * es);
    h->vin = ar.alloc(2 * px * 8 * es);
    h->logits = (float*)ar.alloc(3 * M * sizeof(float));
    h->predict = (float*)ar.alloc(2 * M * sizeof(float));
    h->dl_d = ar.alloc(3 * M * 8 * es);
    h->dl_g = ar.alloc(M * 8 * es);
    h->d_din = ar.alloc(px * 8 * es);
    h->d_vin = ar.alloc(px * 8 * es);
    h->dy4 = ar.alloc(px * 8 * es);
    h->D.t[0].y = h->din; h->V.t[0].y = h->vin;
    carve_net(h->D, ar, es, true);
    carve_net(h->V, ar, es, true);
    for (Tens& t : h->G.t) if (!t.is_input && t.name != "decoder_1") { t.dz = ar.alloc(t.elems() * es); if (t.hi) t.dz32 = ar.alloc(t.elems() * sizeof(float)); }
    for (Tens& t : h->D.t) if (!t.is_input && t.name != "layer_5") { t.dz = ar.alloc(t.elems() * es); t.dz2 = ar.alloc(t.elems() / 3 * es); }
    for (Net* n : {&h->G, &h->D})
      for (Tens& t : n->t) if (h->bf16 && !t.is_input && !t.has_bn && t.C == 64) t.cs_part = (double*)ar.alloc((size_t)512 * 2 * 64 * sizeof(double));
    for (Tens& t : h->V.t) if (!t.is_input) t.dz = ar.alloc(t.elems() / 2 * es);
    for (const Tens& t : h->V.t) {
      if (t.name == "pool1") h->vpool_code[0] = (unsigned char*)ar.alloc(t.elems() / 2);
      if (t.name == "pool2") h->vpool_code[1] = (unsigned char*)ar.alloc(t.elems() / 2);
    }
    h->n_comp = composite_nblocks(N, H * H);
    h->n_perc = perceptual_nblocks((size_t)N * (H / 4) * (H / 4) * 256, h->bf16);
    h->comp_partial = (double*)ar.alloc((size_t)h->n_comp * 2 * sizeof(double));
    h->perc_partial = (double*)ar.alloc((size_t)h->n_perc * sizeof(double));
  }
  h->zeros = ar.alloc(256);
  h->bn_partial = (double*)ar.alloc((size_t)1024 * 2 * 512 * sizeof(double));
  h->scratch = (char*)ar.alloc(h->scratch_bytes);
  if (d.training) {
    h->bn_partial2 = (double*)ar.alloc((size_t)1024 * 2 * 512 * sizeof(double));
    h->scratch2 = (char*)ar.alloc(h->scratch_bytes);
    h->bn_partial3 = (double*)ar.alloc((size_t)1024 * 2 * 512 * sizeof(double));
    h->scratch3 = (char*)ar.alloc(h->scratch_bytes);
    h->bn_partial4 = (double*)ar.alloc((size_t)1024 * 2 * 512 * sizeof(double));
    h->scratch4 = (char*)ar.alloc(h->scratch_bytes);
  }
  return ar.off + 256;
}

static IgemmArgs pool_fused_view(const IgemmPlan& p) {
  static unsigned char set[16] = {};
  IgemmArgs v = launch_view(p, p.form);
  v.pool_code = set;
  v.pool_src = 1;
  return v;
}

static void init_handle(vp_pixrefer* h, const vp_pixrefer_desc* d) {
  h->d = *d;
  h->bf16 = d->dtype == VP_BF16;
  h->es = h->bf16 ? 2 : 4;
  build_generator(h->G, d->batch, d->height, d->ngf, (!d->training && d->per_sample_bn) ? d->batch : 1);
  size_t smax = 0;
  plan_net(h->G, h->bf16, d->training, d->training, 0, &smax);
  if (d->training) {
    build_discriminator(h->D, d->batch, d->height, d->ndf);
    plan_net(h->D, h->bf16, true, true, d->batch, &smax);
    build_vgg(h->V, d->batch, d->height);
    for (Layer& L : h->V.l) L.g.N = 2 * d->batch;
    plan_net(h->V, h->bf16, true, false, d->batch, &smax, true);
    for (const Layer& L : h->V.l) {
      if (L.scope != "conv1/conv1_2" && L.scope != "conv2/conv2_2") continue;
      const int k = L.scope == "conv2/conv2_2", knob = pool_bwd_fused_knob();
      const IgemmArgs& ba = L.bwd_alt[0].a;
      const bool big = !k || (long long)ba.N * (ba.Hg / 4) * (ba.Wg / 16) >= 4096;
      h->pool_fuse_ok[k] = ((knob == 1 && big) || knob == 2 + k || knob == 4) && h->bf16 && conv_kernel_ok(pool_fused_view(L.bwd_alt[0]), h->bf16);
    }
  }
  h->scratch_bytes = smax + 256;
  h->params_dirty = true;
  h->vgg_dirty = true;
}

static bool valid_desc(const vp_pixrefer_desc* d) {
  if (!d) { set_err("pixrefer descriptor: null"); return false; }
  if (d->batch < 1 || d->height < 256 || d->height % 256 != 0) { set_err("pixrefer descriptor: batch %d / height %d (height must be a multiple of 256)", d->batch, d->height); return false; }
  if (d->ngf < 8 || (d->ngf & (d->ngf - 1)) || d->ndf < 8 || (d->ndf & (d->ndf - 1))) { set_err("pixrefer descriptor: ngf %d / ndf %d must be powers of two >= 8", d->ngf, d->ndf); return false; }
  if (d->ngf > 64 || d->ndf > 64) { set_err("pixrefer descriptor: ngf %d / ndf %d > 64 exceed the batch-norm workspace (512 channels)", d->ngf, d->ndf); return false; }
  if (!d->training && d->per_sample_bn && d->batch > 1024) { set_err("pixrefer descriptor: per-sample batch-norm supports at most 1024 frames per call (got %d)", d->batch); return false; }
  if (d->dtype != VP_F32 && d->dtype != VP_BF16) { set_err("pixrefer descriptor: dtype %d", d->dtype); return false; }
  if ((d->streams != 0 && d->streams != 1 && d->streams != 3 && d->streams != 4) || d->d_backward_fork < 0 || d->d_backward_fork > 3 || d->d_beside_vgg < 0 ||
      d->d_beside_vgg > 2) {
    set_err("pixrefer descriptor: schedule fields streams %d / d_backward_fork %d / d_beside_vgg %d", d->streams, d->d_backward_fork, d->d_beside_vgg);
    return false;
  }
  return true;
}

static void fill_src(const Net& n, const Layer& L, PixSrc& x, int group_n, int sample0, int group0, int es) {
  for (int s = 0; s < 2; ++s) {
    x.ptr[s] = nullptr; x.C[s] = 0; x.aff_a[s] = nullptr; x.aff_b[s] = nullptr;
  }
  for (int s = 0; s < L.nsrc; ++s) {
    const Tens& t = n.t[L.src[s]];
    const void* base = (L.in_act != ACT_NONE) ? t.xa[L.in_act] : t.y;
    x.ptr[s] = (const char*)base + (size_t)sample0 * t.H * t.W * t.C * es;
    x.C[s] = t.C;
  }
  x.act = ACT_NONE;
  x.group_n = group_n;
  (void)group0;
}

static int run_pack(vp_pixrefer* h, Net& n, hipStream_t st) {
  if (n.descs.empty()) return VP_OK;
  VP_HIP_CHECK(launch_pack_weights(n.d_descs, (int)n.descs.size(), n.params, n.packed, h->bf16, st));
  return VP_OK;
// ... 47 lines not shown
static int run_layer_fwd_half(vp_pixrefer* h, Net& n, Layer& L, int half, hipStream_t st, void* pool_out = nullptr, bool pool_only = false,
                              unsigned char* pool_code = nullptr) {
  IgemmArgs a = L.fwd_half.a;
  a.pool_out = pool_out;
  a.pool_only = pool_out && pool_only ? 1 : 0;
  a.pool_code = a.pool_only ? pool_code : nullptr;
  const int nb = a.N;
  fill_src(n, L, a.x, nb, half * nb, 0, h->es);
  a.Wp = n.packed + L.pk_fwd_half * h->es;
  Tens& to = n.t[L.out];
  a.Y = (char*)to.y + (size_t)half * nb * to.H * to.W * to.C * h->es;
  a.bias = n.params + L.b_off;
  a.partial = nullptr;
  a.zeros = h->zeros;
  profile_tag((L.scope + (half ? ":fwd1" : ":fwd0")).c_str());
  VP_HIP_CHECK(launch_igemm(a, h->bf16, L.fwd_half.cfg, st));
  return VP_OK;
}

static bool first_layer_acts_fused(const vp_pixrefer* h, const Net& n, const Layer& L) {
  return first_layer_shape(h->bf16, n, L) && L.fwd.a.kern == CK_CIN8;
}

static int run_layer_fwd(vp_pixrefer* h, Net& n, Layer& L, hipStream_t st, void* pool_out = nullptr, int ss = 0) {
  IgemmArgs a = L.fwd.a;
  a.pool_out = pool_out;
  fill_src(n, L, a.x, n.batch / n.groups, 0, 0, h->es);
  a.Wp = n.packed + L.pk_fwd * h->es;
  Tens& to = n.t[L.out];
  a.Y = L.tapgemm ? L.tap_S : to.y;
  a.bias = L.has_bn || L.tapgemm ? nullptr : n.params + L.b_off;
  a.partial = (float*)scratch_of(h, ss);
  a.zeros = h->zeros;
  if (a.kern == CK_SMALLP) {
    SmallPArgs sp;
    memset(&sp, 0, sizeof(sp));
    a.sp_cnt = L.sp_cnt_fwd;
    sp.g = a;
    for (int c = 0; c < 4; ++c) sp.tap_mask[c] = a.sp_mask[c];
    sp.slab = a.partial; sp.cnt = a.sp_cnt; sp.part = bnp_of(h, ss);
    sp.mode = L.has_bn ? SP_FWD_BN : SP_PLAIN;
    sp.hi = to.hi ? 1 : 0;
    if (L.has_bn) {
      sp.gamma = n.params + L.gamma_off; sp.beta = n.params + L.beta_off;
      sp.aff_a = to.bn.a; sp.aff_b = to.bn.b; sp.mu = to.bn.mu; sp.rstd = to.bn.rstd;
      sp.out_lrelu = to.need_act[ACT_LRELU] ? to.xa[ACT_LRELU] : nullptr;
      sp.out_relu = to.need_act[ACT_RELU] ? to.xa[ACT_RELU] : nullptr;
      sp.eps = 1e-5f;
    }
    profile_tag((L.scope + ":fwd").c_str());
    VP_HIP_CHECK(launch_smallp_fused(sp, h->bf16, st));
    if (!L.has_bn && (to.need_act[ACT_LRELU] || to.need_act[ACT_RELU]))
      VP_HIP_CHECK(launch_act_apply(to.y, nullptr, nullptr, to.C, (n.batch / n.groups) * to.H * to.W, (size_t)to.N * to.H * to.W,
                                    to.xa[ACT_LRELU], to.xa[ACT_RELU], h->bf16, st));
    return VP_OK;
  }
  bool fused_stats = false;
  int stat_chunks = 0;
  if (L.has_bn && a.kern == CK_DC256 && n.groups == 1) {
    stat_chunks = 2 * conv_dc256_grid(a);
    a.bn_part = bnp_of(h, ss); a.bn_tpg = 1 << 30; a.bn_nchunk = stat_chunks;
    fused_stats = true;
  } else if (L.has_bn && a.kern == CK_S2C64) {
    const int grid = conv_s2c64_grid(a);
    if ((size_t)n.groups * grid * 2 * to.C <= (size_t)1024 * 2 * 512 && n.groups <= 32) {
      stat_chunks = grid;
      a.bn_part = bnp_of(h, ss); a.bn_tpg = (n.batch / n.groups) * conv_s2c64_tiles_per_image(a); a.bn_nchunk = grid;
      fused_stats = true;
    }
  } else if (L.fwd_stats) {
    stat_chunks = epi_stat_chunks(L.fwd, n.batch, n.groups);
    a.bn_part = bnp_of(h, ss); a.bn_tpg = stat_chunks / a.nclass; a.bn_nchunk = stat_chunks;
    fused_stats = true;
  }
  bool acts_fused = false;
  if (first_layer_acts_fused(h, n, L)) {
    a.xa_lrelu = to.need_act[ACT_LRELU] ? to.xa[ACT_LRELU] : nullptr;
    a.xa_relu = to.need_act[ACT_RELU] ? to.xa[ACT_RELU] : nullptr;
    if (!h->store_first_raw) a.Y = nullptr;
    acts_fused = true;
  }
  profile_tag((L.scope + ":fwd").c_str());
  VP_HIP_CHECK(launch_igemm(a, h->bf16, L.fwd.cfg, st));
  if (L.tapgemm) {
    TapArgs ta;
    memset(&ta, 0, sizeof(ta));
    ta.S = L.tap_S; ta.bias = n.params + L.b_off; ta.y = (float*)to.y;
    ta.N = L.g.N; ta.Hin = L.g.Hin; ta.Win = L.g.Win; ta.Hout = L.g.Hout; ta.Wout = L.g.Wout; ta.ks = L.g.ks; ta.pad = L.g.pad;
    VP_HIP_CHECK(launch_tap_gather(ta, st));
  }
  bool acts_done = acts_fused;
  if (L.has_bn) {
    const int rc = run_bn_stats(h, n, L, fused_stats ? stat_chunks : 0, st, ss);
    if (rc < 0) return rc;
    acts_done = rc == 1;
  }
  if (!acts_done && (to.need_act[ACT_LRELU] || to.need_act[ACT_RELU])) {
    VP_HIP_CHECK(launch_act_apply(to.y, L.has_bn ? to.bn.a : nullptr, L.has_bn ? to.bn.b : nullptr, to.C,
                                  (n.batch / n.groups) * to.H * to.W, (size_t)to.N * to.H * to.W,
                                  to.xa[ACT_LRELU], to.xa[ACT_RELU], h->bf16, st));
  }
  return VP_OK;
}

static int run_layer_bwd(vp_pixrefer* h, Net& n, Layer& L, const void* dy, bool want_dw, bool alt,
                         int sample0, int nb, int group0, hipStream_t st, int ss = 0, bool gpass = false, int parts = 7) {
  const int es = h->es;
  if (!(parts & 1)) want_dw = false;
  char* scratch = scratch_of(h, ss);
  double* bn_partial = bnp_of(h, ss);
  const int group_n = n.batch / n.groups;
  if (want_dw) {
    WgradArgs w = L.wg.a;
    PixSrc xs;
    fill_src(n, L, xs, group_n, sample0, group0, es);
    PixSrc ds;
    set_single_src(ds, dy, L.g.CoutT, nullptr, nullptr, ACT_NONE, 0);
    if (L.g.kind == 0) { w.g = xs; w.d = ds; } else { w.g = ds; w.d = xs; }
    bool own_wgrad = false;
    if (L.tapgemm && h->bf16 && cout1_knob() > 0 && L.nsrc == 1 && !n.t[L.src[0]].is_input && !n.t[L.src[0]].hi && n.t[L.src[0]].xa[L.in_act] &&
        L.g.ks == 4 && L.g.stride == 1) {
      Tens& tx = n.t[L.src[0]];
      Cout1Args c;
      memset(&c, 0, sizeof(c));
      c.dy = dy; c.ld_dy = L.g.CoutT;
      c.ref = (const char*)tx.xa[L.in_act] + (size_t)sample0 * tx.H * tx.W * tx.C * es;
      c.N = nb; c.H = tx.H; c.W = tx.W; c.C = tx.C; c.Ho = L.g.Hout; c.Wo = L.g.Wout; c.ks = L.g.ks; c.pad = L.g.pad;
      c.slabs = (float*)scratch; c.dW = n.grads + L.w_off;
      const long long px = (long long)nb * tx.H * tx.W;
      const size_t cap = h->scratch_bytes / ((size_t)16 * 512 * sizeof(float));
      c.rows = (int)(px / 96 < wgrad1_rows_knob() ? px / 96 : wgrad1_rows_knob());
      if ((size_t)c.rows > cap) c.rows = (int)cap;
      if (c.rows >= 1 && L.g.Cin == 512 && conv_cout1_wgrad_eligible(c)) {
        profile_tag((L.scope + ":wgrad").c_str());
        VP_HIP_CHECK(launch_cout1_wgrad_prof(c, st));
        own_wgrad = true;
      }
    }
    if (L.tapgemm && !own_wgrad) {
      TapArgs ta;
      memset(&ta, 0, sizeof(ta));
      ta.dy = dy; ta.dyS = L.tap_dyS; ta.ld_dy = L.g.CoutT;
      ta.N = nb; ta.Hin = L.g.Hin; ta.Win = L.g.Win; ta.Hout = L.g.Hout; ta.Wout = L.g.Wout; ta.ks = L.g.ks; ta.pad = L.g.pad;
      VP_HIP_CHECK(launch_tap_spread(ta, h->bf16, st));
      set_single_src(w.g, L.tap_dyS, 16, nullptr, nullptr, ACT_NONE, 0);
      w.d = xs;
    }
    w.partial = (float*)scratch;
    w.dW = n.grads + L.w_off;
    w.accumulate = 0;
    w.zeros = h->zeros;
    if (!own_wgrad) {
      profile_tag((L.scope + ":wgrad").c_str());
      VP_HIP_CHECK(launch_wgrad(w, h->bf16, L.wg.cfg, st));
    }
    float* db = n.grads + L.b_off;
    if (L.has_bn) {
    } else {
      BnArgs b;
      memset(&b, 0, sizeof(b));
      b.y = dy; b.C = L.g.CoutT; b.G = 1; b.Pg = nb * L.g.Hout * L.g.Wout;
      b.nchunk = bn_nchunk(b.Pg, b.C, 1, h->bf16);
      b.partial = bn_partial;
      Tens& to = n.t[L.out];
      if (to.cs_chunks > 0 && dy == to.dz) {
        b.partial = to.cs_part; b.nchunk = to.cs_chunks;
        to.cs_chunks = 0;
// ... 271 lines not shown
  std::vector<std::pair<size_t, size_t>> regs;
  char* const base = reinterpret_cast<char*>((uintptr_t)1 << 40);
  carve_all(h, base, need, &regs);
  int rc = VP_OK;
  auto fail = [&](const char* fmt, auto... args) { if (rc == VP_OK) { set_err(fmt, args...); rc = VP_ERR_STATE; } };
  size_t prev_end = 0;
  for (size_t i = 0; i < regs.size(); ++i) {
    if (regs[i].first % 256) fail("region %zu at %zu: not 256-byte aligned", i, regs[i].first);
    if (regs[i].first < prev_end) fail("region %zu at %zu overlaps the previous one (ends %zu)", i, regs[i].first, prev_end);
    prev_end = regs[i].first + regs[i].second;
  }
  if (prev_end + 256 > need + 256 || prev_end > need) fail("carved %zu bytes of a %zu-byte workspace", prev_end, need);
  auto region_of = [&](const void* p, size_t bytes, const char* what) {
    if (!p) { fail("%s: null", what); return; }
    const size_t off = (size_t)((const char*)p - base);
    for (const auto& r : regs)
      if (off >= r.first && off + bytes <= r.first + r.second) return;
    fail("%s: [%zu, +%zu) is not inside a carved region", what, off, bytes);
  };
  const int es = h->es;
  for (Net* n : {&h->G, &h->D, &h->V}) {
    if (n->t.empty()) continue;
    for (const Tens& t : n->t) {
      const std::string nm = t.name;
      if (t.name == "decoder_1" || t.name == "layer_5") continue;
      region_of(t.y, t.elems() * (t.hi ? 4 : es), (nm + ".y").c_str());
      for (int k = 1; k < 3; ++k) if (t.need_act[k]) region_of(t.xa[k], t.elems() * es, (nm + ".xa").c_str());
      if (t.has_bn) {
        const size_t gc = (size_t)n->groups * t.C * sizeof(float);
        for (const float* p : {t.bn.a, t.bn.b, t.bn.mu, t.bn.rstd, t.bn.c1, t.bn.c2, t.bn.c1g, t.bn.c2g}) region_of(p, gc, (nm + ".bn").c_str());
        if (d->training && t.pb_cap) region_of(t.bn.pb, (size_t)n->groups * t.pb_cap * 2 * t.C * sizeof(double), (nm + ".bn.pb").c_str());
        if (d->training && t.pbg_cap) region_of(t.bn.pbg, (size_t)t.pbg_cap * 2 * t.C * sizeof(double), (nm + ".bn.pbg").c_str());
        if ((size_t)n->groups * t.C > (size_t)1024 * 512) fail("%s: %d groups x %d channels exceed the batch-norm partial rows", nm.c_str(), n->groups, t.C);
      }
      if (t.cs_part) region_of(t.cs_part, (size_t)512 * 2 * 64 * sizeof(double), (nm + ".cs_part").c_str());
      if (d->training && !t.is_input) {
        const size_t div = n == &h->V ? 2 : 1;
        region_of(t.dz, t.elems() / div * es, (nm + ".dz").c_str());
        if (t.hi) region_of(t.dz32, t.elems() * 4, (nm + ".dz32").c_str());
        if (n == &h->D) region_of(t.dz2, t.elems() / 3 * es, (nm + ".dz2").c_str());
      }
    }
    region_of(n->packed, n->packed_elems * es, "packed weights");
    region_of(n->d_descs, n->descs.size() * sizeof(PackDesc), "pack descriptors");
    for (const PackDesc& p : n->descs) {
      const size_t pe = (size_t)p.nclass * p.Kpad * p.rows_pad;
      if (p.dst_off + pe > n->packed_elems) fail("pack block [%zu, +%zu) outside the %zu-element packed arena", p.dst_off, pe, n->packed_elems);
      if (p.src_off >= n->nparams) fail("pack source %zu outside the %zu-float parameter arena", p.src_off, n->nparams);
    }
    size_t pend = 0;
    for (const ParamInfo& p : n->manifest) {
      size_t cnt = 1;
      for (int i = 0; i < 4; ++i) cnt *= (size_t)p.shape[i];
      if (p.off != pend) fail("parameter %s at %zu: arena not contiguous (expected %zu)", p.name.c_str(), p.off, pend);
      pend = p.off + cnt;
    }
    if (pend != n->nparams) fail("parameter manifest covers %zu of %zu floats", pend, n->nparams);
    for (const Layer& L : n->l) {
      auto plan_ok = [&](const IgemmPlan& p, const char* what) {
        if (p.partial_bytes > h->scratch_bytes) fail("%s %s: split-K slab %zu > scratch %zu", L.scope.c_str(), what, p.partial_bytes, h->scratch_bytes);
        if (p.a.splitk < 1 || p.a.CoutPad < p.a.Cout) fail("%s %s: splitk %d CoutPad %d", L.scope.c_str(), what, p.a.splitk, p.a.CoutPad);
        if (!conv_kernel_ok(launch_view(p, p.form), h->bf16))
          fail("%s %s: the launch is outside the preconditions of its kernel %s", L.scope.c_str(), what, conv_kernel_name(p.a.kern));
      };
      plan_ok(L.fwd, "fwd");
      if (L.has_fwd_half) plan_ok(L.fwd_half, "fwd_half");
      if (d->training && L.has_pair) plan_ok(L.bwd_pair, "bwd_pair");
      if (d->training)
        for (int s2 = 0; s2 < L.nsrc; ++s2) if (L.need_bwd[s2]) { plan_ok(L.bwd[s2], "bwd"); if (n == &h->D || n == &h->V) plan_ok(L.bwd_alt[s2], "bwd_alt"); }
      if (d->training && n != &h->V && L.wg.partial_bytes > h->scratch_bytes) fail("%s wgrad: slab %zu > scratch %zu", L.scope.c_str(), L.wg.partial_bytes, h->scratch_bytes);
      if (L.tapgemm) { region_of(L.tap_S, (size_t)L.g.N * L.g.Hin * L.g.Win * 16 * 4, "tap_S"); region_of(L.tap_dyS, (size_t)L.g.N * L.g.Hin * L.g.Win * 16 * es, "tap_dyS"); }
    }
  }
  const size_t px = (size_t)d->batch * d->height * d->height;
  region_of(h->gin, px * 8 * es, "gin"); region_of(h->gfg, px * 8 * es, "gfg");
  region_of(h->y4, px * 4 * 4, "y4"); region_of(h->o4, px * 4 * 4, "o4");
  region_of(h->outputs, px * 3 * 4, "outputs"); region_of(h->outputs_fg, px * 3 * 4, "outputs_fg");
  region_of(h->scratch, h->scratch_bytes, "scratch"); region_of(h->bn_partial, (size_t)1024 * 2 * 512 * 8, "bn_partial");
  if (d->training) {
    const int hd = d->height / 8 - 2;
    const size_t M = (size_t)d->batch * hd * hd;
    region_of(h->din, 3 * px * 8 * es, "din"); region_of(h->vin, 2 * px * 8 * es, "vin");
    region_of(h->logits, 3 * M * 4, "logits"); region_of(h->predict, 2 * M * 4, "predict");
    region_of(h->dl_d, 3 * M * 8 * es, "dl_d"); region_of(h->dl_g, M * 8 * es, "dl_g");
    region_of(h->d_din, px * 8 * es, "d_din"); region_of(h->d_vin, px * 8 * es, "d_vin"); region_of(h->dy4, px * 8 * es, "dy4");
    for (const Tens& t : h->V.t) {
      if (t.name == "pool1") region_of(h->vpool_code[0], t.elems() / 2, "pool1 codes");
      if (t.name == "pool2") region_of(h->vpool_code[1], t.elems() / 2, "pool2 codes");
    }
    for (const Layer& L : h->V.l) {
      const int k = L.scope == "conv2/conv2_2";
      if ((L.scope != "conv1/conv1_2" && !k) || !h->pool_fuse_ok[k]) continue;
      const Tens& tp = h->V.t[L.out + 1];
      if (tp.name != (k ? "pool2" : "pool1") || tp.H * 2 != h->V.t[L.out].H || tp.C != h->V.t[L.out].C) fail("%s: the tensor behind it is not its 2x2 pool", L.scope.c_str());
      if (L.bwd_alt[0].a.kern != CK_C64 || !conv_kernel_ok(pool_fused_view(L.bwd_alt[0]), h->bf16)) fail("%s bwd_alt: no pooled-source form of kernel %s", L.scope.c_str(), conv_kernel_name(L.bwd_alt[0].a.kern));
      region_of(tp.dz, tp.elems() / 2 * es, (tp.name + ".dz (pooled-source read)").c_str());
      region_of(h->vpool_code[k], tp.elems() / 2, (tp.name + " codes (pooled-source read)").c_str());
    }
    region_of(h->scratch2, h->scratch_bytes, "scratch2"); region_of(h->scratch3, h->scratch_bytes, "scratch3");
    region_of(h->scratch4, h->scratch_bytes, "scratch4"); region_of(h->bn_partial4, (size_t)1024 * 2 * 512 * 8, "bn_partial4");
    region_of(h->bn_partial2, (size_t)1024 * 2 * 512 * 8, "bn_partial2"); region_of(h->bn_partial3, (size_t)1024 * 2 * 512 * 8, "bn_partial3");
  }
  delete h;
  return rc;
}

struct StreamPool {
  int dev = -1;
  hipStream_t side = nullptr, branch = nullptr, branch2 = nullptr;
};
static StreamPool g_pool;
static std::mutex g_pool_mu;

static int pool_streams(bool want_b2, hipStream_t* side, hipStream_t* branch, hipStream_t* branch2) {
  std::lock_guard<std::mutex> lk(g_pool_mu);
  int dev = 0;
  VP_HIP_CHECK(hipGetDevice(&dev));
  if (g_pool.dev >= 0 && g_pool.dev != dev) { set_err("the step executor's streams were created on device %d, this plan is on device %d (one device per process)", g_pool.dev, dev); return VP_ERR_STATE; }
  if (!g_pool.side) {
    int prio_lo = 0, prio_hi = 0;
    (void)hipDeviceGetStreamPriorityRange(&prio_lo, &prio_hi);
    VP_HIP_CHECK(hipStreamCreateWithPriority(&g_pool.side, hipStreamNonBlocking, prio_lo));
    VP_HIP_CHECK(hipStreamCreateWithFlags(&g_pool.branch, hipStreamNonBlocking));
    g_pool.dev = dev;
  }
  if (want_b2 && !g_pool.branch2) VP_HIP_CHECK(hipStreamCreateWithFlags(&g_pool.branch2, hipStreamNonBlocking));
  if (side) *side = g_pool.side;
  if (branch) *branch = g_pool.branch;
  if (branch2) *branch2 = g_pool.branch2;
  return VP_OK;
}

int vp_reserve_streams(void) { return pool_streams(true, nullptr, nullptr, nullptr); }

void* vp_host_stream(void) {
  hipStream_t b2 = nullptr;
  if (pool_streams(true, nullptr, nullptr, &b2)) return nullptr;
  return (void*)b2;
}

int vp_pixrefer_create(const vp_pixrefer_desc* d, void* workspace, size_t workspace_bytes,
                       float* params_g, float* params_d, const float* params_vgg,
                       float* grads_g, float* grads_d, void* stream, vp_pixrefer_t** out) {
  if (!valid_desc(d) || !workspace || !params_g || !out) { set_err("vp_pixrefer_create: bad argument"); return VP_ERR_ARG; }
  if (d->training && (!params_d || !params_vgg || !grads_g || !grads_d)) { set_err("training needs D/VGG params and grad arenas"); return VP_ERR_ARG; }
  vp_pixrefer* h = new vp_pixrefer{};
  init_handle(h, d);
  const size_t need = carve_all(h, nullptr, 0);
  if (workspace_bytes < need) { set_err("workspace too small: %zu < %zu", workspace_bytes, need); delete h; return VP_ERR_WORKSPACE; }
  carve_all(h, (char*)workspace, workspace_bytes);
  h->G.params = params_g; h->G.grads = grads_g;
  h->D.params = params_d; h->D.grads = grads_d;
  h->V.params = const_cast<float*>(params_vgg);
  for (Tens& t : h->G.t) if (t.name == "decoder_1") { t.y = h->y4; t.dz = h->dy4; }
  hipStream_t st = (hipStream_t)stream;
  VP_HIP_CHECK(hipMemsetAsync(h->zeros, 0, 256, st));
  if (d->training) for (Tens& t : h->D.t) if (t.name == "layer_5") { t.y = h->logits; t.dz = h->dl_d; }
  for (Net* n : {&h->G, &h->D, &h->V}) {
    if (n->descs.empty()) continue;
    VP_HIP_CHECK(hipMemcpyAsync(n->d_descs, n->descs.data(), n->descs.size() * sizeof(PackDesc), hipMemcpyHostToDevice, st));
    VP_HIP_CHECK(hipMemsetAsync(n->sp_cnt, 0, (n->sp_cnt_n + 1) * sizeof(unsigned), st));
  }
  VP_HIP_CHECK(hipStreamSynchronize(st));
  h->overlap = false; h->forked = false;
  h->bst_on = 1; h->vgg_fork_layer = 3;
  h->ov_on = true; h->store_first_raw = false; h->dfork_point = d->d_backward_fork ? d->d_backward_fork - 1 : 2; h->dsplit_on = d->d_beside_vgg != 1;
  if (d->training && d->streams != 1) {
    { const int rc = pool_streams(false, &h->side, &h->branch, &h->branch2); if (rc) { delete h; return rc; } }
    VP_HIP_CHECK(hipEventCreateWithFlags(&h->ev_fork, hipEventDisableTiming));
    VP_HIP_CHECK(hipEventCreateWithFlags(&h->ev_join, hipEventDisableTiming));
    h->use_b2 = d->streams != 3;
    VP_HIP_CHECK(hipEventCreateWithFlags(&h->ev_b2join, hipEventDisableTiming));
    VP_HIP_CHECK(hipEventCreateWithFlags(&h->ev_bfork, hipEventDisableTiming));
    VP_HIP_CHECK(hipEventCreateWithFlags(&h->ev_bjoin, hipEventDisableTiming));
    VP_HIP_CHECK(hipEventCreateWithFlags(&h->ev_upd_b, hipEventDisableTiming));
    VP_HIP_CHECK(hipEventCreateWithFlags(&h->ev_upd_m, hipEventDisableTiming));
    h->overlap = true;
  }
  *out = h;
  return VP_OK;
}

void vp_pixrefer_destroy(vp_pixrefer_t* h) {
  if (!h) return;
  if (h->marks_made) for (int i = 0; i < 64; ++i) (void)hipEventDestroy(h->mark[i]);
  if (h->overlap) {
    (void)hipStreamSynchronize(h->side);
    (void)hipEventDestroy(h->ev_fork);
    (void)hipEventDestroy(h->ev_join);
    (void)hipStreamSynchronize(h->branch);
    (void)hipEventDestroy(h->ev_bfork);
    (void)hipEventDestroy(h->ev_bjoin);
    (void)hipEventDestroy(h->ev_b2join);
    if (h->branch2) (void)hipStreamSynchronize(h->branch2);
    (void)hipEventDestroy(h->ev_upd_b);
    (void)hipEventDestroy(h->ev_upd_m);
  }
  delete h;
}

int vp_pixrefer_params_changed(vp_pixrefer_t* h) {
  if (!h) return VP_ERR_ARG;
  h->params_dirty = true;
  h->vgg_dirty = true;
  h->upd_mask = 0;
  return VP_OK;
}

int vp_pixrefer_optimizer_stepped(vp_pixrefer_t* h) {
  if (!h) return VP_ERR_ARG;
  h->params_dirty = true;
  return VP_OK;
}

static int forward_impl(vp_pixrefer_t* h, const float* inputs, const float* fg_inputs, int fg_c, const float* targets, const float* masks, void* stream);

int vp_pixrefer_forward(vp_pixrefer_t* h, const float* inputs, const float* fg_inputs,
                        const float* targets, const float* masks, void* stream) {
  return forward_impl(h, inputs, fg_inputs, 6, targets, masks, stream);
}

int vp_pixrefer_forward_fg3(vp_pixrefer_t* h, const float* inputs, const float* fg_inputs3, const float* targets, void* stream) {
  if (h && h->d.training) { set_err("vp_pixrefer_forward_fg3: inference plans only (the training graph reads fg_inputs[..., 3:], pixrefer.py:297,321)"); return VP_ERR_STATE; }
  return forward_impl(h, inputs, fg_inputs3, 3, targets, nullptr, stream);
}

size_t vp_pixrefer_desc_size(void) { return sizeof(vp_pixrefer_desc); }

static int forward_impl(vp_pixrefer_t* h, const float* inputs, const float* fg_inputs, int fg_c, const float* targets, const float* masks, void* stream) {
  if (!h || !inputs || !fg_inputs || !targets) { set_err("vp_pixrefer_forward: null argument"); return VP_ERR_ARG; }
  const vp_pixrefer_desc& d = h->d;
  if (d.training && !masks) { set_err("vp_pixrefer_forward: masks required when training"); return VP_ERR_ARG; }
  hipStream_t st = (hipStream_t)stream;
  const int N = d.batch, H = d.height, bf = h->bf16;
  int rc;
  if (h->params_dirty) {
    if ((rc = run_pack(h, h->G, st))) return rc;
    if (d.training) {
      if ((rc = run_pack(h, h->D, st))) return rc;
      if (h->vgg_dirty) { if ((rc = run_pack(h, h->V, st))) return rc; h->vgg_dirty = false; }
    }
    h->params_dirty = false;
  }
  h->in_targets = targets; h->in_masks = masks;
  PackInputsArgs pi;
  memset(&pi, 0, sizeof(pi));
  pi.inputs = inputs; pi.fg_inputs = fg_inputs; pi.gin = h->gin; pi.gfg = h->gfg; pi.din = h->din; pi.vin = h->vin;
  pi.N = N; pi.HW = H * H; pi.train = d.training; pi.fg_c = fg_c;
  phase_mark(h, st, 0);
  VP_HIP_CHECK(launch_pack_inputs(pi, bf, st));

  bool split_vgg = d.training && h->overlap && h->ov_on;
  if (split_vgg) for (Layer& L : h->V.l) split_vgg = split_vgg && L.has_fwd_half;
  auto vgg_real_half = [&]() -> int {
    VP_HIP_CHECK(hipEventRecord(h->ev_fork, st));
    VP_HIP_CHECK(hipStreamWaitEvent(h->side, h->ev_fork, 0));
    Net& Vs = h->V;
    for (size_t i = 0; i < Vs.l.size(); ++i) {
      Layer& L = Vs.l[i];
      const bool pooled = L.scope == "conv1/conv1_2" || L.scope == "conv2/conv2_2";
      const bool fuse = pooled && plan_can_pool(L.fwd_half);
      if ((rc = run_layer_fwd_half(h, Vs, L, 0, h->side, fuse ? Vs.t[L.out + 1].y : nullptr, true))) return rc;
      if (pooled && !fuse) {
        const Tens& ti = Vs.t[L.out];
        Tens& tp = Vs.t[L.out + 1];
        VP_HIP_CHECK(launch_maxpool_fwd(ti.y, tp.y, N, ti.H, ti.W, ti.C, bf, h->side));
      }
    }
    VP_HIP_CHECK(hipEventRecord(h->ev_join, h->side));
    return VP_OK;
  };
  bool vgg_real_started = false;
  if (split_vgg && h->vgg_fork_layer <= 0) { if ((rc = vgg_real_half())) return rc; vgg_real_started = true; }

  const bool split_enc = d.training && h->overlap && h->ov_on;
  if (split_enc) {
    VP_HIP_CHECK(hipEventRecord(h->ev_bfork, st));
    VP_HIP_CHECK(hipStreamWaitEvent(h->branch, h->ev_bfork, 0));
    for (Layer& L : h->G.l) if (L.scope.rfind("encoder_fg_", 0) == 0) if ((rc = run_layer_fwd(h, h->G, L, h->branch, nullptr, 2))) return rc;
    VP_HIP_CHECK(hipEventRecord(h->ev_bjoin, h->branch));
  }
  for (Layer& L : h->G.l) {
    if (split_enc && L.scope.rfind("encoder_fg_", 0) == 0) continue;
    if (split_enc && L.scope == "merged_encoder_2") VP_HIP_CHECK(hipStreamWaitEvent(st, h->ev_bjoin, 0));
    if (split_vgg && !vgg_real_started && (int)(&L - &h->G.l[0]) >= h->vgg_fork_layer) { if ((rc = vgg_real_half())) return rc; vgg_real_started = true; }
    if (g_phase_detail) phase_mark(h, st, 8 + (int)(&L - &h->G.l[0]));
    if ((rc = run_layer_fwd(h, h->G, L, st))) return rc;
  }

  if (split_vgg && !vgg_real_started) { if ((rc = vgg_real_half())) return rc; vgg_real_started = true; }
  CompositeArgs ca;
  memset(&ca, 0, sizeof(ca));
  ca.y4 = h->y4; ca.targets = targets; ca.masks = masks; ca.o4 = h->o4; ca.outputs = h->outputs; ca.outputs_fg = h->outputs_fg;
  ca.din = h->din; ca.vin = h->vin; ca.partial = h->comp_partial; ca.N = N; ca.HW = H * H; ca.train = d.training;
  VP_HIP_CHECK(launch_composite_fwd(ca, bf, st));
  phase_mark(h, st, 1);
  if (!d.training) return VP_OK;

  const bool split_d = h->overlap && h->ov_on && h->dsplit_on;
  hipStream_t sd = split_d ? h->branch : st;
  const int ssd = split_d ? 2 : 0;
  if (split_d) {
    VP_HIP_CHECK(hipEventRecord(h->ev_bfork, st));
    VP_HIP_CHECK(hipStreamWaitEvent(h->branch, h->ev_bfork, 0));
  }
  for (Layer& L : h->D.l) if ((rc = run_layer_fwd(h, h->D, L, sd, nullptr, ssd))) return rc;
  const int hd = H / 8 - 2;
  GanLossArgs ga;
  memset(&ga, 0, sizeof(ga));
  ga.logits = h->logits; ga.dl_d = h->dl_d; ga.dl_g = h->dl_g; ga.predict = h->predict; ga.losses = h->losses;
  ga.M = N * hd * hd; ga.gan_weight = d.gan_weight;
  VP_HIP_CHECK(launch_gan_loss(ga, bf, sd));
  if (split_d) VP_HIP_CHECK(hipEventRecord(h->ev_bjoin, h->branch));

  Net& V = h->V;
  bool codes = split_vgg && bf && !h->store_first_raw && h->vpool_code[0] && h->vpool_code[1];
  for (Layer& L : V.l)
    if (L.scope == "conv1/conv1_2" || L.scope == "conv2/conv2_2") codes = codes && plan_can_pool(L.fwd_half);
  h->pool_codes_written = codes;
  auto vgg_half = [&](int half, hipStream_t s2) -> int {
    for (size_t i = 0; i < V.l.size(); ++i) {
      Layer& L = V.l[i];
      int rc2;
      const bool pooled = L.scope == "conv1/conv1_2" || L.scope == "conv2/conv2_2";
      const bool fuse = pooled && plan_can_pool(L.fwd_half);
      const Tens& ti = V.t[L.out];
      Tens& tp = V.t[pooled ? L.out + 1 : L.out];
      const size_t oi = (size_t)half * N * ti.H * ti.W * ti.C * h->es, op = (size_t)half * N * tp.H * tp.W * tp.C * h->es;
      const bool code = fuse && codes && half == 1;
      if ((rc2 = run_layer_fwd_half(h, V, L, half, s2, fuse ? (char*)tp.y + op : nullptr, code, code ? h->vpool_code[L.scope == "conv2/conv2_2"] : nullptr))) return rc2;
      if (pooled && !fuse) VP_HIP_CHECK(launch_maxpool_fwd((const char*)ti.y + oi, (char*)tp.y + op, N, ti.H, ti.W, ti.C, bf, s2));
    }
    return VP_OK;
  };
  if (split_vgg) {
    if ((rc = vgg_half(1, st))) return rc;
    VP_HIP_CHECK(hipStreamWaitEvent(st, h->ev_join, 0));
  } else {
    for (size_t i = 0; i < V.l.size(); ++i) {
      Layer& L = V.l[i];
      const bool pooled = L.scope == "conv1/conv1_2" || L.scope == "conv2/conv2_2";
      const bool fuse = pooled && plan_can_pool(L.fwd);
      if ((rc = run_layer_fwd(h, V, L, st, fuse ? V.t[L.out + 1].y : nullptr))) return rc;
      if (pooled && !fuse) {
        const Tens& ti = V.t[L.out];
        Tens& tp = V.t[L.out + 1];
        VP_HIP_CHECK(launch_maxpool_fwd(ti.y, tp.y, ti.N, ti.H, ti.W, ti.C, bf, st));
      }
    }
  }
  const Tens& f3 = V.t.back();
  PerceptualArgs pa;
  memset(&pa, 0, sizeof(pa));
  pa.f3 = f3.y; pa.df3 = f3.dz; pa.partial = h->perc_partial; pa.half = f3.elems() / 2; pa.l1_weight = d.l1_weight;
  VP_HIP_CHECK(launch_perceptual(pa, bf, st));

  if (split_d) VP_HIP_CHECK(hipStreamWaitEvent(st, h->ev_bjoin, 0));
  LossFinalArgs lf;
  memset(&lf, 0, sizeof(lf));
  lf.comp_partial = h->comp_partial; lf.n_comp = h->n_comp; lf.perc_partial = h->perc_partial; lf.n_perc = h->n_perc;
  lf.n_out = (double)N * H * H * 3; lf.n_feat = (double)pa.half; lf.losses = h->losses;
  lf.l1_weight = d.l1_weight; lf.gan_weight = d.gan_weight;
  VP_HIP_CHECK(launch_loss_final(lf, st));
  phase_mark(h, st, 2);
  return VP_OK;
}

static int backward_d_on(vp_pixrefer_t* h, hipStream_t st, bool side);
static int fork_d(vp_pixrefer_t* h, hipStream_t st);

static int update_range(vp_pixrefer_t* h, Net& n, float* m, float* v, float lr_t, size_t off0, size_t off1, int l0, int l1, hipStream_t s) {
  if (off1 > off0) {
    AdamArgs a;
    a.p = n.params + off0; a.g = n.grads + off0; a.m = m + off0; a.v = v + off0; a.n = off1 - off0;
    a.lr_t = lr_t; a.beta1 = h->upd.beta1; a.beta2 = h->upd.beta2; a.eps = h->upd.eps;
    VP_HIP_CHECK(launch_adam(a, s));
  }
  const size_t d0 = n.l[l0].desc0, d1 = n.l[l1].desc1;
  if (d1 > d0) VP_HIP_CHECK(launch_pack_weights(n.d_descs + d0, (int)(d1 - d0), n.params, n.packed, h->bf16, s));
  return VP_OK;
}
static int update_d(vp_pixrefer_t* h, hipStream_t s) {
  h->upd.d_done = true;
  return update_range(h, h->D, h->upd.m_d, h->upd.v_d, h->upd.lr_t_d, 0, h->D.nparams, 0, (int)h->D.l.size() - 1, s);
}

int vp_pixrefer_backward(vp_pixrefer_t* h, void* stream) {
  if (!h || !h->d.training) { set_err("vp_pixrefer_backward: needs a training plan"); return VP_ERR_STATE; }
  hipStream_t st = (hipStream_t)stream;
  if (!h->overlap || !h->ov_on) {
    int rc = vp_pixrefer_backward_d(h, stream);
    if (rc) return rc;
    return vp_pixrefer_backward_g(h, stream);
  }
  int rc;
  h->dfork_pending = h->dfork_point;
  if (h->dfork_pending == 0 && (rc = fork_d(h, st))) { h->dfork_pending = 0; return rc; }
  rc = vp_pixrefer_backward_g(h, stream);
  h->dfork_pending = 0;
  if (rc) return rc;
  VP_HIP_CHECK(hipStreamWaitEvent(st, h->ev_join, 0));
  phase_mark(h, st, 7);
  return VP_OK;
}

static int fork_d(vp_pixrefer_t* h, hipStream_t st) {
  h->dfork_pending = 0;
  VP_HIP_CHECK(hipEventRecord(h->ev_fork, st));
  VP_HIP_CHECK(hipStreamWaitEvent(h->side, h->ev_fork, 0));
  int rc = backward_d_on(h, h->side, true);
  if (rc) return rc;
  if (h->upd.active && h->dfork_point == 2 && (rc = update_d(h, h->side))) return rc;
  VP_HIP_CHECK(hipEventRecord(h->ev_join, h->side));
  return VP_OK;
}

int vp_pixrefer_backward_update(vp_pixrefer_t* h, float* m_g, float* v_g, float* m_d, float* v_d, int step_t_g, int step_t_d,
                                float lr, float beta1, float beta2, float eps, void* stream) {
  if (!h || !h->d.training) { set_err("vp_pixrefer_backward_update: needs a training plan"); return VP_ERR_STATE; }
  if (!m_g || !v_g || !m_d || !v_d || step_t_g < 1 || step_t_d < 1) { set_err("vp_pixrefer_backward_update: bad argument"); return VP_ERR_ARG; }
  auto lr_t = [&](int t) { return (float)((double)lr * sqrt(1.0 - pow((double)beta2, t)) / (1.0 - pow((double)beta1, t))); };
  h->upd.active = true; h->upd.d_done = false;
  h->upd.m_g = m_g; h->upd.v_g = v_g; h->upd.m_d = m_d; h->upd.v_d = v_d;
  h->upd.lr_t_g = lr_t(step_t_g); h->upd.lr_t_d = lr_t(step_t_d); h->upd.beta1 = beta1; h->upd.beta2 = beta2; h->upd.eps = eps;
  int rc = vp_pixrefer_backward(h, stream);
  if (!rc && !h->upd.d_done) rc = update_d(h, (hipStream_t)stream);
  h->upd.active = false;
  if (rc) return rc;
  h->params_dirty = false;
  return VP_OK;
}

int vp_pixrefer_update_bucket(vp_pixrefer_t* h, int which, int bucket, float* m, float* v, int step_t, float lr, float beta1, float beta2,
                              float eps, void* stream) {
  if (!h || !h->d.training || !m || !v || step_t < 1 || which < 0 || which > 1 || bucket < 0 || bucket > (which ? 0 : 2)) {
    set_err("vp_pixrefer_update_bucket: bad argument");
    return VP_ERR_ARG;
  }
  const float lr_t = (float)((double)lr * sqrt(1.0 - pow((double)beta2, step_t)) / (1.0 - pow((double)beta1, step_t)));
  h->upd.beta1 = beta1; h->upd.beta2 = beta2; h->upd.eps = eps;
  int rc;
  if (which == 1) {
    rc = update_range(h, h->D, m, v, lr_t, 0, h->D.nparams, 0, (int)h->D.l.size() - 1, (hipStream_t)stream);
    h->upd_mask |= 8;
  } else {
    Net& G = h->G;
    int i_md5 = -1, i_me2 = -1;
    for (int i = 0; i < (int)G.l.size(); ++i) {
      if (G.l[i].scope == "merged_decoder_5") i_md5 = i;
      if (G.l[i].scope == "merged_encoder_2") i_me2 = i;
    }
    const int l0 = bucket == 0 ? i_md5 : (bucket == 1 ? i_me2 : 0);
    const int l1 = bucket == 0 ? (int)G.l.size() - 1 : (bucket == 1 ? i_md5 - 1 : i_me2 - 1);
    const size_t off0 = G.l[l0].w_off, off1 = l1 + 1 < (int)G.l.size() ? G.l[l1 + 1].w_off : G.nparams;
    rc = update_range(h, G, m, v, lr_t, off0, off1, l0, l1, (hipStream_t)stream);
    h->upd_mask |= 1 << bucket;
  }
  if (rc) return rc;
  if (h->upd_mask == 15) { h->upd_mask = 0; h->params_dirty = false; }
  return VP_OK;
}

int vp_pixrefer_backward_d(vp_pixrefer_t* h, void* stream) {
  if (!h || !h->d.training) { set_err("vp_pixrefer_backward_d: needs a training plan"); return VP_ERR_STATE; }
  return backward_d_on(h, (hipStream_t)stream, false);
}

int vp_pixrefer_backward_d_fork(vp_pixrefer_t* h, void* stream) {
  if (!h || !h->d.training) { set_err("vp_pixrefer_backward_d_fork: needs a training plan"); return VP_ERR_STATE; }
  hipStream_t st = (hipStream_t)stream;
  h->forked = h->overlap && h->ov_on;
  if (!h->forked) return backward_d_on(h, st, false);
  h->dfork_pending = h->dfork_point;
  if (h->dfork_pending == 0) return fork_d(h, st);
  return VP_OK;
}

void* vp_pixrefer_side_stream(vp_pixrefer_t* h) { return (h && h->overlap) ? (void*)h->side : nullptr; }

int vp_pixrefer_use_streams(vp_pixrefer_t* h, int n) {
  if (!h || (n != 3 && n != 4)) { set_err("vp_pixrefer_use_streams: 3 or 4"); return VP_ERR_ARG; }
  h->use_b2 = (n == 4) && h->overlap;
  return VP_OK;
}

int vp_pixrefer_set_option(vp_pixrefer_t* h, const char* key, int value) {
  if (!h || !key) { set_err("vp_pixrefer_set_option: null argument"); return VP_ERR_ARG; }
  const std::string k(key);
  if (k == "overlap") { h->ov_on = value != 0; return VP_OK; }
  if (k == "d_backward_fork") { h->dfork_point = value < 0 ? 0 : (value > 2 ? 2 : value); return VP_OK; }
  if (k == "d_beside_vgg") { h->dsplit_on = value != 0; return VP_OK; }
  if (k == "store_first_raw") { h->store_first_raw = value != 0; return VP_OK; }
  if (k == "bwd_sums_in_epilogue") { h->bst_on = value < 0 ? 0 : (value > 2 ? 2 : value); return VP_OK; }
  if (k == "vgg_real_fork") { h->vgg_fork_layer = value < 0 ? 0 : value; return VP_OK; }
  set_err("vp_pixrefer_set_option: unknown key %s", key);
  return VP_ERR_ARG;
}

long long vp_pixrefer_counter(vp_pixrefer_t* h, const char* key) {
  if (!h || !key) return -1;
  if (std::string(key) == "bwd_sums_launches") return h->bst_count;
  if (std::string(key) == "pool_codes_written") return h->pool_codes_written ? 1 : 0;
  if (std::string(key) == "pool_bwd_fused") return h->pool_bwd_fused ? 1 : 0;
  return -1;
}

int vp_pixrefer_backward_d_join(vp_pixrefer_t* h, void* stream) {
  if (!h || !h->d.training) { set_err("vp_pixrefer_backward_d_join: needs a training plan"); return VP_ERR_STATE; }
  if (h->forked && h->dfork_pending) {
    const int rc = fork_d(h, (hipStream_t)stream);
    if (rc) return rc;
  }
  if (h->forked) VP_HIP_CHECK(hipStreamWaitEvent((hipStream_t)stream, h->ev_join, 0));
  h->forked = false;
  return VP_OK;
}

static int backward_d_on(vp_pixrefer_t* h, hipStream_t st, bool side) {
  const int N = h->d.batch;
  int rc;
  Net& D = h->D;

  for (Tens& t : D.t) { t.dz_written = false; t.bst_chunks = 0; t.cs_chunks = 0; }
  for (int i = (int)D.l.size() - 1; i >= 0; --i) {
    Layer& L = D.l[i];
    Tens& to = D.t[L.out];
    if (L.has_bn) if ((rc = run_bn_bwd(h, D, L, true, 0, 3 * N, 0, 3, st, side ? 1 : 0))) return rc;
    const bool save = L.need_bwd[0];
    if (i == 0) L.need_bwd[0] = false;
    rc = run_layer_bwd(h, D, L, to.dz, true, false, 0, 3 * N, 0, st, side ? 1 : 0);
    L.need_bwd[0] = save;
    if (rc) return rc;
  }

  return VP_OK;
}

int vp_pixrefer_backward_g(vp_pixrefer_t* h, void* stream) { return vp_pixrefer_backward_g_stage(h, -1, stream); }

int vp_pixrefer_backward_g_stages(void) { return 3; }

int vp_pixrefer_backward_g_stage(vp_pixrefer_t* h, int stage, void* stream) {
  if (!h || !h->d.training) { set_err("vp_pixrefer_backward_g: needs a training plan"); return VP_ERR_STATE; }
  if (stage > 2) { set_err("vp_pixrefer_backward_g_stage: stage must be < 3"); return VP_ERR_ARG; }
  hipStream_t st = (hipStream_t)stream;
  const vp_pixrefer_desc& d = h->d;
  const int N = d.batch, H = d.height, bf = h->bf16, es = h->es;
  int rc;
  Net &G = h->G, &D = h->D, &V = h->V;
  int i_md5 = -1, i_me2 = -1;
  for (int i = 0; i < (int)G.l.size(); ++i) {
    if (G.l[i].scope == "merged_decoder_5") i_md5 = i;
    if (G.l[i].scope == "merged_encoder_2") i_me2 = i;
  }
  const int l_hi = stage <= 0 ? (int)G.l.size() - 1 : (stage == 1 ? i_md5 - 1 : i_me2 - 1);
  const int l_lo = stage < 0 ? 0 : (stage == 0 ? i_md5 : (stage == 1 ? i_me2 : 0));
  if (stage <= 0) {
  const bool split_d = h->overlap && h->ov_on && h->dsplit_on;
  hipStream_t sd = split_d ? h->branch : st;
  const int ssd = split_d ? 2 : 0;
  if (split_d) {
    VP_HIP_CHECK(hipEventRecord(h->ev_bfork, st));
    VP_HIP_CHECK(hipStreamWaitEvent(h->branch, h->ev_bfork, 0));
  }
  for (Tens& t : D.t) { t.dz2_written = false; t.bst_chunks_g = 0; }
  for (int i = (int)D.l.size() - 1; i >= 0; --i) {
    Layer& L = D.l[i];
    Tens& to = D.t[L.out];
    if (L.has_bn) if ((rc = run_bn_bwd(h, D, L, false, 2 * N, N, 2, 1, sd, ssd, true))) return rc;
    const void* dy = (i == (int)D.l.size() - 1) ? h->dl_g : to.dz2;
    if ((rc = run_layer_bwd(h, D, L, dy, false, true, 2 * N, N, 2, sd, ssd, true))) return rc;
  }
  if (split_d) VP_HIP_CHECK(hipEventRecord(h->ev_bjoin, h->branch));
  if (h->dfork_pending == 1 && (rc = fork_d(h, st))) return rc;
  for (Tens& t : V.t) t.dz_written = false;
  h->pool_bwd_fused = false;
  h->pool_dz_stale[0] = h->pool_dz_stale[1] = false;
  for (int i = (int)V.l.size() - 1; i >= 0; --i) {
    Layer& L = V.l[i];
    Tens& to = V.t[L.out];
    Tens& ti = V.t[L.src[0]];
    IgemmArgs a = L.bwd_alt[0].a;
    set_single_src(a.x, to.dz, L.g.CoutT, nullptr, nullptr, ACT_NONE, 0);
    const int pk = L.scope == "conv2/conv2_2";
    if ((pk || L.scope == "conv1/conv1_2") && h->pool_dz_stale[pk]) {
      a.x.ptr[0] = V.t[L.out + 1].dz;
      a.pool_code = h->vpool_code[pk];
      a.pool_src = 1;
    }
    a.Wp = V.packed + L.pk_bwd_alt[0] * es;
    a.partial = (float*)h->scratch;
    const bool from_pool = (ti.name == "pool1" || ti.name == "pool2");
    if (ti.is_input) {
      a.Y = h->d_vin;
    } else {
      a.Y = ti.dz;
      if (!from_pool) {
        a.ref = (const char*)ti.y + ti.elems() / 2 * es;
        a.ref_act = ACT_RELU;
      }
    }
    a.zeros = h->zeros;
    profile_tag((L.scope + ":bwd").c_str());
    VP_HIP_CHECK(launch_igemm(a, bf, L.bwd_alt[0].cfg, st));
    if (from_pool) {
      const int ci = L.src[0] - 1;
      Tens& tc = V.t[ci];
      const char* xin = (const char*)tc.y + tc.elems() / 2 * es;
      const int k = ti.name == "pool2";
      if (h->pool_codes_written && h->pool_fuse_ok[k]) {
        h->pool_dz_stale[k] = true;
        h->pool_bwd_fused = true;
      } else if (h->pool_codes_written) VP_HIP_CHECK(launch_maxpool_bwd_code(h->vpool_code[k], ti.dz, tc.dz, N, tc.H, tc.W, tc.C, bf, st));
      else VP_HIP_CHECK(launch_maxpool_bwd(xin, ti.dz, tc.dz, N, tc.H, tc.W, tc.C, bf, st));
    }
  }
  if (split_d) VP_HIP_CHECK(hipStreamWaitEvent(st, h->ev_bjoin, 0));
  if (h->dfork_pending == 2 && (rc = fork_d(h, st))) return rc;
  CompositeArgs ca;
  memset(&ca, 0, sizeof(ca));
  ca.targets = h->in_targets; ca.masks = h->in_masks; ca.o4 = h->o4; ca.outputs = h->outputs;
  ca.d_din = h->d_din; ca.d_vin = h->d_vin; ca.dy4 = h->dy4; ca.N = N; ca.HW = H * H; ca.l1_weight = d.l1_weight;
  VP_HIP_CHECK(launch_composite_bwd(ca, bf, st));
  phase_mark(h, st, 3);
  for (Tens& t : G.t) { t.dz_written = false; t.dz_writes = 0; t.bn_bwd_done = false; t.bst_chunks = 0; t.cs_chunks = 0; }
  }
  const bool split_enc = h->overlap && h->ov_on && l_lo == 0;
  const bool wsplit = h->overlap && h->ov_on;
  bool forked = false, fg_forked = false;
  bool b2_used = false;
  for (int i = l_hi; i >= l_lo; --i) {
    Layer& L = G.l[i];
    Tens& to = G.t[L.out];
    const bool fg = split_enc && L.scope.rfind("encoder_fg_", 0) == 0;
    if (fg && !fg_forked) {
      VP_HIP_CHECK(hipEventRecord(h->ev_bfork, st));
      if (h->use_b2 && !h->branch2) { const int rc2 = pool_streams(true, nullptr, nullptr, &h->branch2); if (rc2) return rc2; }
      VP_HIP_CHECK(hipStreamWaitEvent(h->use_b2 ? h->branch2 : h->branch, h->ev_bfork, 0));
      forked = fg_forked = true;
      b2_used = h->use_b2;
    }
    hipStream_t s2 = fg ? (h->use_b2 ? h->branch2 : h->branch) : st;
    const int ss = fg ? (h->use_b2 ? 3 : 2) : 0;
    if (i == i_md5 - 1) phase_mark(h, st, 4);
    if (i == i_me2 - 1) phase_mark(h, st, 5);
    if (g_phase_detail && !fg) phase_mark(h, st, 32 + i);
    if (L.has_bn) if ((rc = run_bn_bwd(h, G, L, true, 0, N, 0, 1, s2, ss))) return rc;
    if (wsplit && !fg) {
      VP_HIP_CHECK(hipEventRecord(h->ev_bfork, st));
      VP_HIP_CHECK(hipStreamWaitEvent(h->branch, h->ev_bfork, 0));
      forked = true;
      if ((rc = run_layer_bwd(h, G, L, to.dz, true, false, 0, N, 0, h->branch, 2, false, 1))) return rc;
      if ((rc = run_layer_bwd(h, G, L, to.dz, true, false, 0, N, 0, st, 0, false, 6))) return rc;
    } else {
      if ((rc = run_layer_bwd(h, G, L, to.dz, true, false, 0, N, 0, s2, ss))) return rc;
    }
    if (h->upd.active && (i == i_md5 || i == i_me2 || i == 0)) {
      const int l0 = i, l1 = i == i_md5 ? (int)G.l.size() - 1 : (i == i_me2 ? i_md5 - 1 : i_me2 - 1);
      const size_t off0 = G.l[l0].w_off, off1 = l1 + 1 < (int)G.l.size() ? G.l[l1 + 1].w_off : G.nparams;
      hipStream_t su = st;
      const bool on_side = h->overlap && h->ov_on && h->dfork_pending == 0 && h->dfork_point >= 0;
      if (h->overlap && h->ov_on && on_side) {
        VP_HIP_CHECK(hipEventRecord(h->ev_upd_b, h->branch));
        VP_HIP_CHECK(hipEventRecord(h->ev_upd_m, st));
        VP_HIP_CHECK(hipStreamWaitEvent(h->side, h->ev_upd_b, 0));
        VP_HIP_CHECK(hipStreamWaitEvent(h->side, h->ev_upd_m, 0));
        if (b2_used) {
          VP_HIP_CHECK(hipEventRecord(h->ev_b2join, h->branch2));
          VP_HIP_CHECK(hipStreamWaitEvent(h->side, h->ev_b2join, 0));
        }
        su = h->side;
      } else if (h->overlap && h->ov_on) {
        VP_HIP_CHECK(hipEventRecord(h->ev_bfork, st));
        VP_HIP_CHECK(hipStreamWaitEvent(h->branch, h->ev_bfork, 0));
        if (b2_used) {
          VP_HIP_CHECK(hipEventRecord(h->ev_b2join, h->branch2));
          VP_HIP_CHECK(hipStreamWaitEvent(h->branch, h->ev_b2join, 0));
        }
        su = h->branch; forked = true;
      }
      if ((rc = update_range(h, G, h->upd.m_g, h->upd.v_g, h->upd.lr_t_g, off0, off1, l0, l1, su))) return rc;
      if (h->overlap && h->ov_on && on_side) VP_HIP_CHECK(hipEventRecord(h->ev_join, h->side));
    }
  }
  if (forked) {
    if (g_phase_detail && (stage < 0 || stage == 2)) phase_mark(h, st, 60);
    VP_HIP_CHECK(hipEventRecord(h->ev_bjoin, h->branch));
    VP_HIP_CHECK(hipStreamWaitEvent(st, h->ev_bjoin, 0));
    if (b2_used) {
      VP_HIP_CHECK(hipEventRecord(h->ev_b2join, h->branch2));
      VP_HIP_CHECK(hipStreamWaitEvent(st, h->ev_b2join, 0));
    }
  }
  if (stage < 0 || stage == 2) phase_mark(h, st, 6);
  return VP_OK;
}

int vp_profile_enable(int on) { profile_enable(on); return VP_OK; }
size_t vp_profile_collect(char* json, size_t cap) { return profile_collect(json, cap); }

int vp_pixrefer_tensor(vp_pixrefer_t* h, const char* name, void** ptr, int64_t shape[4], int* dtype) {
  if (!h || !name || !ptr) return VP_ERR_ARG;
  const int N = h->d.batch, H = h->d.height;
  auto ret = [&](void* p, int64_t a, int64_t b, int64_t c, int64_t e, int dt) {
    *ptr = p;
    if (shape) { shape[0] = a; shape[1] = b; shape[2] = c; shape[3] = e; }
    if (dtype) *dtype = dt;
    return p ? VP_OK : VP_ERR_STATE;
  };
  const std::string s(name);
  const int cd = h->bf16 ? VP_BF16 : VP_F32;
  if (s == "Outputs_raw") return ret(h->outputs, N, H, H, 3, VP_F32);
  if (s == "Outputs_FG") return ret(h->outputs_fg, N, H, H, 3, VP_F32);
  if (s == "gen_out4") return ret(h->o4, N, H, H, 4, VP_F32);
  if (s == "losses") return ret(h->losses, 8, 1, 1, 1, VP_F32);
  const int hd = H / 8 - 2;
  if (s == "Predict") return ret(h->predict, 2, N, hd, hd, VP_F32);
  if (s == "logits") return ret(h->logits, 3 * N, hd, hd, 1, VP_F32);
  if (s == "d_gen_out4") return ret(h->dy4, N, H, H, 8, cd);
  if (s == "d_din") return ret(h->d_din, N, H, H, 8, cd);
  if (s == "d_vin") return ret(h->d_vin, N, H, H, 8, cd);
  const size_t c = s.find('/');
  if (c == std::string::npos) return VP_ERR_ARG;
  const std::string net = s.substr(0, c);
  std::string rest = s.substr(c + 1);
  Net* n = net == "g" ? &h->G : net == "d" ? &h->D : net == "v" ? &h->V : nullptr;
  if (!n) return VP_ERR_ARG;
  std::string field;
  const size_t k = rest.find(':');
  if (k != std::string::npos) { field = rest.substr(k + 1); rest = rest.substr(0, k); }
  for (Tens& t : n->t) {
    if (t.name != rest) continue;
    if (field.empty() && !h->store_first_raw && t.producer >= 0 && first_layer_acts_fused(h, *n, n->l[t.producer])) {
      set_err("vp_pixrefer_tensor: the raw output of %s is not stored (its kernel writes the consumers' activations); vp_pixrefer_set_option(h, \"store_first_raw\", 1) before the forward pass", s.c_str());
      return VP_ERR_STATE;
    }
    if (field.empty() && n == &h->V && h->pool_codes_written && (t.name == "conv1/conv1_2" || t.name == "conv2/conv2_2")) {
      set_err("vp_pixrefer_tensor: the full-resolution output of %s is not stored (the step keeps its 2x2 max pool and the pool's arg-max codes); vp_pixrefer_set_option(h, \"store_first_raw\", 1) before the forward pass", s.c_str());
      return VP_ERR_STATE;
    }
    if (field.empty()) return ret(t.y, t.N, t.H, t.W, t.is_f32 ? (t.name == "decoder_1" ? 4 : 1) : t.C, (t.is_f32 || t.hi) ? VP_F32 : cd);
    if (field == "dz32") return t.hi ? ret(t.dz32, t.N, t.H, t.W, t.C, VP_F32) : VP_ERR_ARG;
    if (field == "dy" && n == &h->V && (t.name == "conv1/conv1_2" || t.name == "conv2/conv2_2") && h->pool_dz_stale[t.name == "conv2/conv2_2"]) {
      const int k = t.name == "conv2/conv2_2";
      const Tens& tp = n->t[(&t - n->t.data()) + 1];
      VP_HIP_CHECK(hipDeviceSynchronize());
      VP_HIP_CHECK(launch_maxpool_bwd_code(h->vpool_code[k], tp.dz, t.dz, t.N / 2, t.H, t.W, t.C, h->bf16, nullptr));
      VP_HIP_CHECK(hipDeviceSynchronize());
      h->pool_dz_stale[k] = false;
    }
    if (field == "dy") return ret(t.dz, n == &h->V ? t.N / 2 : t.N, t.H, t.W, t.C, cd);
    if (!t.has_bn) return VP_ERR_ARG;
    if (field == "scale") return ret(t.bn.a, n->groups, t.C, 1, 1, VP_F32);
    if (field == "shift") return ret(t.bn.b, n->groups, t.C, 1, 1, VP_F32);
    if (field == "mean") return ret(t.bn.mu, n->groups, t.C, 1, 1, VP_F32);
    if (field == "rstd") return ret(t.bn.rstd, n->groups, t.C, 1, 1, VP_F32);
    return VP_ERR_ARG;
  }
  return VP_ERR_ARG;
}

int vp_pixrefer_fetch(vp_pixrefer_t* h, int what, void* dst, void* stream) {
  if (!h || !dst || what < 0 || what > 3) { set_err("vp_pixrefer_fetch: bad argument"); return VP_ERR_ARG; }
  FetchArgs f;
  memset(&f, 0, sizeof(f));
  f.raw3 = h->outputs; f.fg3 = h->outputs_fg; f.o4 = h->o4; f.dst = dst;
  f.npix = (size_t)h->d.batch * h->d.height * h->d.height;
  f.mode = what;
  if (what == 3 && h->d.training) {
    VP_HIP_CHECK(hipMemcpyAsync(dst, h->outputs_fg, f.npix * 3 * sizeof(float), hipMemcpyDeviceToDevice, (hipStream_t)stream));
    return VP_OK;
  }
  VP_HIP_CHECK(launch_fetch(f, (hipStream_t)stream));
  return VP_OK;
}

int vp_grad_pack_bf16(const float* src, void* dst_bf16, size_t n, void* stream) {
  if (!src || !dst_bf16 || n < 1 || ((uintptr_t)src & 31) || ((uintptr_t)dst_bf16 & 15)) { set_err("vp_grad_pack_bf16: bad argument"); return VP_ERR_ARG; }
  VP_HIP_CHECK(launch_grad_pack_bf16(src, dst_bf16, n, (hipStream_t)stream));
  return VP_OK;
}
int vp_grad_unpack_bf16(const void* src_bf16, float* dst, size_t n, float scale, void* stream) {
  if (!src_bf16 || !dst || n < 1 || ((uintptr_t)dst & 31) || ((uintptr_t)src_bf16 & 15)) { set_err("vp_grad_unpack_bf16: bad argument"); return VP_ERR_ARG; }
  VP_HIP_CHECK(launch_grad_unpack_bf16(src_bf16, dst, n, scale, (hipStream_t)stream));
  return VP_OK;
}

int vp_adam_tf(float* params, const float* grads, float* m, float* v, size_t n, int step_t,
               float lr, float beta1, float beta2, float eps, void* stream) {
  if (!params || !grads || !m || !v || step_t < 1) { set_err("vp_adam_tf: bad argument"); return VP_ERR_ARG; }
  AdamArgs a;
  a.p = params; a.g = grads; a.m = m; a.v = v; a.n = n;
  a.lr_t = (float)((double)lr * sqrt(1.0 - pow((double)beta2, step_t)) / (1.0 - pow((double)beta1, step_t)));
  a.beta1 = beta1; a.beta2 = beta2; a.eps = eps;
  VP_HIP_CHECK(launch_adam(a, (hipStream_t)stream));
  return VP_OK;
}

}
```

voicepuppet_amd/csrc/pointwise.hip:

```cpp
#include "pointwise_args.h"
#include "vp_common.h"

namespace vp {

template <int NV>
__device__ __forceinline__ void block_sum(double (&v)[NV], double* sm ) {
  const int lane = threadIdx.x & 63, wave = threadIdx.x >> 6, nw = blockDim.x >> 6;
#pragma unroll
  for (int i = 0; i < NV; ++i) v[i] = wave_sum(v[i]);
  __syncthreads();
  if (lane == 0)
#pragma unroll
    for (int i = 0; i < NV; ++i) sm[i * 16 + wave] = v[i];
  __syncthreads();
  if (threadIdx.x == 0)
#pragma unroll
    for (int i = 0; i < NV; ++i) {
      double s = 0;
      for (int w = 0; w < nw; ++w) s += sm[i * 16 + w];
      v[i] = s;
    }
}

template <typename T>
// ... 344 lines not shown
#pragma unroll
    for (int e = 0; e < E; ++e) { mu[e] = a.mu[grp * a.C + c0 + e]; rs[e] = a.rstd[grp * a.C + c0 + e]; }
    double s0[E], s1[E];
#pragma unroll
    for (int e = 0; e < E; ++e) { s0[e] = 0; s1[e] = 0; }
    for (int p = threadIdx.x; p < a.Pg; p += 256) {
      float fy[E], fd[E];
      Elem<T>::unpack(*reinterpret_cast<const uint4*>(y + (size_t)p * a.C), fy);
      Elem<T>::unpack(*reinterpret_cast<const uint4*>(dz + (size_t)p * a.C), fd);
#pragma unroll
      for (int e = 0; e < E; ++e) { s0[e] += fd[e]; s1[e] += (double)fd[e] * ((fy[e] - mu[e]) * rs[e]); }
    }
    block_sum2<E>(s0, s1, sm);
    float c1[E], c2[E];
#pragma unroll
    for (int e = 0; e < E; ++e) {
      c1[e] = (float)(s0[e] / a.Pg); c2[e] = (float)(s1[e] / a.Pg);
      db[e] += s0[e]; dg[e] += s1[e];
      if (threadIdx.x == 0) { a.c1[grp * a.C + c0 + e] = c1[e]; a.c2[grp * a.C + c0 + e] = c2[e]; }
    }
    for (int p = threadIdx.x; p < a.Pg; p += 256) {
      float fy[E], fd[E];
      Elem<T>::unpack(*reinterpret_cast<const uint4*>(y + (size_t)p * a.C), fy);
      Elem<T>::unpack(*reinterpret_cast<const uint4*>(dz + (size_t)p * a.C), fd);
#pragma unroll
      for (int e = 0; e < E; ++e) {
        const float zh = (fy[e] - mu[e]) * rs[e];
        fd[e] = a.gamma[c0 + e] * rs[e] * (fd[e] - c1[e] - zh * c2[e]);
      }
      *reinterpret_cast<uint4*>(dy + (size_t)p * a.C) = Elem<T>::pack(fd);
    }
    __syncthreads();
  }
  if (threadIdx.x == 0 && a.dgamma) {
#pragma unroll
    for (int e = 0; e < E; ++e) {
      a.dgamma[c0 + e] = (float)dg[e] + (a.accumulate ? a.dgamma[c0 + e] : 0.f);
      a.dbeta[c0 + e] = (float)db[e] + (a.accumulate ? a.dbeta[c0 + e] : 0.f);
    }
  }
  if (threadIdx.x == 0 && a.dbias_zero) {
#pragma unroll
    for (int e = 0; e < E; ++e) a.dbias_zero[c0 + e] = 0.f;
  }
}

template <typename T>
__global__ __launch_bounds__(256) void act_apply_kernel(const T* __restrict__ y, const float* __restrict__ sc, const float* __restrict__ sh,
                                                        int C, int Pg, size_t npix, T* __restrict__ out_lrelu, T* __restrict__ out_relu) {
  constexpr int E = Elem<T>::E;
  const int ncg = C / E;
  const size_t total = npix * ncg;
  const bool fixed = 256 % ncg == 0;
  int cur = -1;
  float fsc[E], fsh[E];
  for (size_t i = (size_t)blockIdx.x * 256 + threadIdx.x; i < total; i += (size_t)gridDim.x * 256) {
    const int cg = (int)(i % ncg);
    const size_t pix = i / ncg;
    float f[E], o[E];
    Elem<T>::unpack(*reinterpret_cast<const uint4*>(y + pix * C + cg * E), f);
    if (sc) {
      const int grp = (int)(pix / Pg);
      if (grp != cur || !fixed) {
        cur = grp;
#pragma unroll
        for (int e = 0; e < E; ++e) { fsc[e] = sc[grp * C + cg * E + e]; fsh[e] = sh[grp * C + cg * E + e]; }
      }
#pragma unroll
      for (int e = 0; e < E; ++e) f[e] = fmaf(fsc[e], f[e], fsh[e]);
    }
    if (out_lrelu) {
#pragma unroll
      for (int e = 0; e < E; ++e) o[e] = act_apply(ACT_LRELU, f[e]);
      *reinterpret_cast<uint4*>(out_lrelu + pix * C + cg * E) = Elem<T>::pack(o);
    }
    if (out_relu) {
#pragma unroll
      for (int e = 0; e < E; ++e) o[e] = act_apply(ACT_RELU, f[e]);
      *reinterpret_cast<uint4*>(out_relu + pix * C + cg * E) = Elem<T>::pack(o);
    }
  }
}

__global__ __launch_bounds__(256) void tap_gather_kernel(TapArgs a) {
  const size_t total = (size_t)a.N * a.Hout * a.Wout;
  const size_t p = (size_t)blockIdx.x * 256 + threadIdx.x;
  if (p >= total) return;
  const int j = (int)(p % a.Wout), i = (int)((p / a.Wout) % a.Hout), n = (int)(p / ((size_t)a.Wout * a.Hout));
  float acc = 0.f;
  for (int kh = 0; kh < a.ks; ++kh) {
    const int qi = i + kh - a.pad;
    if (qi < 0 || qi >= a.Hin) continue;
    for (int kw = 0; kw < a.ks; ++kw) {
      const int qj = j + kw - a.pad;
      if (qj < 0 || qj >= a.Win) continue;
      acc += a.S[(((size_t)n * a.Hin + qi) * a.Win + qj) * 16 + kh * a.ks + kw];
    }
  }
  a.y[p] = acc + a.bias[0];
}

template <typename T>
__global__ __launch_bounds__(256) void tap_spread_kernel(TapArgs a) {
  constexpr int E = Elem<T>::E;
  const size_t total = (size_t)a.N * a.Hin * a.Win;
  const size_t q = (size_t)blockIdx.x * 256 + threadIdx.x;
  if (q >= total) return;
  const int qj = (int)(q % a.Win), qi = (int)((q / a.Win) % a.Hin), n = (int)(q / ((size_t)a.Win * a.Hin));
  const T* dy = (const T*)a.dy;
  float f[16];
#pragma unroll
  for (int t = 0; t < 16; ++t) {
    const int i = qi - t / 4 + a.pad, j = qj - t % 4 + a.pad;
    const bool ok = i >= 0 && i < a.Hout && j >= 0 && j < a.Wout;
    f[t] = ok ? Elem<T>::ld(dy + (((size_t)n * a.Hout + i) * a.Wout + j) * a.ld_dy) : 0.f;
  }
  T* o = (T*)a.dyS + q * 16;
#pragma unroll
  for (int e = 0; e < 16; e += E) {
    float g[E];
#pragma unroll
    for (int k = 0; k < E; ++k) g[k] = f[e + k];
    *reinterpret_cast<uint4*>(o + e) = Elem<T>::pack(g);
  }
}

template <typename T> __device__ __forceinline__ void store8(T* p, const float (&f)[8]);
template <> __device__ __forceinline__ void store8<float>(float* p, const float (&f)[8]) {
  reinterpret_cast<float4*>(p)[0] = make_float4(f[0], f[1], f[2], f[3]);
  reinterpret_cast<float4*>(p)[1] = make_float4(f[4], f[5], f[6], f[7]);
}
template <> __device__ __forceinline__ void store8<bf16>(bf16* p, const float (&f)[8]) {
  *reinterpret_cast<uint4*>(p) = Elem<bf16>::pack(f);
}

template <typename T>
__global__ __launch_bounds__(256) void pack_inputs_kernel(const PackInputsArgs a) {
  const size_t total = (size_t)a.N * a.HW;
  for (size_t i = (size_t)blockIdx.x * 256 + threadIdx.x; i < total; i += (size_t)gridDim.x * 256) {
    float in[6], fg[6];
#pragma unroll
    for (int c = 0; c < 6; ++c) { in[c] = a.inputs[i * 6 + c] * 2.f - 1.f; fg[c] = c < a.fg_c ? a.fg_inputs[i * a.fg_c + c] * 2.f - 1.f : -1.f; }
    { const float f[8] = {in[0], in[1], in[2], in[3], in[4], in[5], 0.f, 0.f}; store8<T>(reinterpret_cast<T*>(a.gin) + i * 8, f); }
    { const float f[8] = {fg[0], fg[1], fg[2], 0.f, 0.f, 0.f, 0.f, 0.f}; store8<T>(reinterpret_cast<T*>(a.gfg) + i * 8, f); }
    if (a.train) {
      T* din = reinterpret_cast<T*>(a.din);
      { const float f[8] = {in[3], in[4], in[5], fg[3], fg[4], fg[5], 0.f, 0.f}; store8<T>(din + i * 8, f); }
      { const float f[8] = {in[0], in[1], in[2], fg[0], fg[1], fg[2], 0.f, 0.f}; store8<T>(din + (total + i) * 8, f); }
      { const float f[8] = {in[3], in[4], in[5], 0.f, 0.f, 0.f, 0.f, 0.f}; store8<T>(din + (2 * total + i) * 8, f); }
      { const float f[8] = {fg[3], fg[4], fg[5], 0.f, 0.f, 0.f, 0.f, 0.f}; store8<T>(reinterpret_cast<T*>(a.vin) + i * 8, f); }
    }
  }
}

__device__ __forceinline__ void resize_coord(int d, int rsize, int S, int& s0, int& s1, float& w1) {
  const float f = (float)(((double)d + 0.5) * ((double)rsize / (double)S) - 0.5);
  int s = (int)floorf(f);
  float w = f - (float)s;
  if (s < 0) { s = 0; w = 0.f; }
  if (s >= rsize - 1) { s = rsize - 1; w = 0.f; }
  s0 = s; s1 = min(s + 1, rsize - 1); w1 = w;
}

__global__ __launch_bounds__(256) void frame_pack_kernel(const FramePackArgs a) {
  const int S = a.S;
  const size_t total = (size_t)a.N * S * S * 2;
  for (size_t i = (size_t)blockIdx.x * 256 + threadIdx.x; i < total; i += (size_t)gridDim.x * 256) {
    const int role = (int)(i & 1);
    const size_t pix = i >> 1;
    const int x = (int)(pix % S), y = (int)((pix / S) % S), n = (int)(pix / ((size_t)S * S));
    const int* cr = a.crops + (n * 2 + role) * 3;
    const int rx = cr[0], ry = cr[1], rsize = cr[2];
    int y0, y1, x0, x1;
    float wy, wx;
    resize_coord(y, rsize, S, y0, y1, wy);
    resize_coord(x, rsize, S, x0, x1, wx);
    const unsigned char* f = (role ? a.cur : a.ex) + (size_t)n * S * 3 * S * 3;
    float v[3][3];
#pragma unroll
    for (int p = 0; p < 3; ++p) {
      const unsigned char* r0 = f + ((size_t)(rx + y0) * 3 * S + p * S + ry) * 3;
      const unsigned char* r1 = f + ((size_t)(rx + y1) * 3 * S + p * S + ry) * 3;
// ... 12 lines not shown
      a.fg_inputs[pix * 6 + role * 3 + c] = v[0][c] * v[2][c];
      if (role) { a.targets[pix * 3 + c] = v[0][c]; a.masks[pix * 3 + c] = v[2][c]; }
    }
  }
}

template <typename T>
__global__ __launch_bounds__(256) void composite_fwd_kernel(const CompositeArgs a) {
  const size_t total = (size_t)a.N * a.HW;
  double acc[2] = {0, 0};
  for (size_t i = (size_t)blockIdx.x * 256 + threadIdx.x; i < total; i += (size_t)gridDim.x * 256) {
    const float4 y = reinterpret_cast<const float4*>(a.y4)[i];
    const float o[4] = {tanhf(y.x), tanhf(y.y), tanhf(y.z), tanhf(y.w)};
    reinterpret_cast<float4*>(a.o4)[i] = make_float4(o[0], o[1], o[2], o[3]);
    const float al = (o[3] + 1.f) * 0.5f;
    float ofg[3];
#pragma unroll
    for (int c = 0; c < 3; ++c) {
      const float tg = a.targets[i * 3 + c] * 2.f - 1.f;
      const float out = o[c] * al + tg * (1.f - al);
      ofg[c] = o[c] * al + al - 1.f;
      a.outputs[i * 3 + c] = out;
      a.outputs_fg[i * 3 + c] = ofg[c];
      if (a.train) {
        acc[0] += fabsf(tg - out);
        acc[1] += fabsf(a.masks[i * 3 + c] - al);
      }
    }
    if (a.train) {
      T* d = reinterpret_cast<T*>(a.din) + (2 * total + i) * 8;
      T* v = reinterpret_cast<T*>(a.vin) + (total + i) * 8;
      float head[3];
      if (sizeof(T) == 2) {
        const uint2 h = *reinterpret_cast<const uint2*>(d);
        head[0] = __uint_as_float(h.x << 16); head[1] = __uint_as_float(h.x & 0xffff0000u); head[2] = __uint_as_float(h.y << 16);
      } else {
        const float4 h = *reinterpret_cast<const float4*>(d);
        head[0] = h.x; head[1] = h.y; head[2] = h.z;
      }
      const float fd[8] = {head[0], head[1], head[2], ofg[0], ofg[1], ofg[2], 0.f, 0.f};
      const float fv[8] = {ofg[0], ofg[1], ofg[2], 0.f, 0.f, 0.f, 0.f, 0.f};
      store8<T>(d, fd);
      store8<T>(v, fv);
    }
  }
  if (a.train) {
    __shared__ double sm[64];
    block_sum<2>(acc, sm);
    if (threadIdx.x == 0) { a.partial[blockIdx.x * 2] = acc[0]; a.partial[blockIdx.x * 2 + 1] = acc[1]; }
  }
}

template <typename T>
__global__ __launch_bounds__(256) void composite_bwd_kernel(const CompositeArgs a) {
  const size_t total = (size_t)a.N * a.HW;
  const float s = a.l1_weight / (float)((double)total * 3.0);
  for (size_t i = (size_t)blockIdx.x * 256 + threadIdx.x; i < total; i += (size_t)gridDim.x * 256) {
    const float4 o4 = reinterpret_cast<const float4*>(a.o4)[i];
    const float o[4] = {o4.x, o4.y, o4.z, o4.w};
    const float al = (o[3] + 1.f) * 0.5f;
    const T* dd = reinterpret_cast<const T*>(a.d_din) + i * 8 + 3;
    const T* dv = reinterpret_cast<const T*>(a.d_vin) + i * 8;
    float dout[8] = {0, 0, 0, 0, 0, 0, 0, 0};
    float dal = 0.f;
#pragma unroll
    for (int c = 0; c < 3; ++c) {
      const float tg = a.targets[i * 3 + c] * 2.f - 1.f;
      const float out = a.outputs[i * 3 + c];
      const float df = tg - out, dm = a.masks[i * 3 + c] - al;
      const float d_out = -s * ((df > 0.f) - (df < 0.f));
      const float d_al = -s * ((dm > 0.f) - (dm < 0.f));
      const float d_fg = Elem<T>::ld(dd + c) + Elem<T>::ld(dv + c);
      dout[c] = (d_out + d_fg) * al;
      dal += d_out * (o[c] - tg) + d_fg * (o[c] + 1.f) + d_al;
    }
    dout[3] = dal * 0.5f;
#pragma unroll
    for (int c = 0; c < 4; ++c) dout[c] *= (1.f - o[c] * o[c]);
    store8<T>(reinterpret_cast<T*>(a.dy4) + i * 8, dout);
  }
}

template <typename T>
__global__ __launch_bounds__(1024) void gan_loss_kernel(const GanLossArgs a) {
  const float eps = 1e-12f;
  double acc[2] = {0, 0};
  const float invM = 1.f / (float)a.M;
  T* dld = reinterpret_cast<T*>(a.dl_d);
  T* dlg = reinterpret_cast<T*>(a.dl_g);
  for (int i = threadIdx.x; i < a.M; i += 1024) {
    const float p0 = 1.f / (1.f + expf(-a.logits[i]));
    const float p1 = 1.f / (1.f + expf(-a.logits[a.M + i]));
    const float pf = 1.f / (1.f + expf(-a.logits[2 * a.M + i]));
    const float pr = (p0 + p1) * 0.5f;
    a.predict[i] = pr; a.predict[a.M + i] = pf;
    acc[0] += -(logf(pr + eps) * 2.f + logf(1.f - pf + eps));
    acc[1] += -logf(pf + eps);
    const float dpr = -2.f / (pr + eps) * invM * 0.5f;
    float f[8] = {0, 0, 0, 0, 0, 0, 0, 0};
    f[0] = dpr * p0 * (1.f - p0); store8<T>(dld + (size_t)i * 8, f);
    f[0] = dpr * p1 * (1.f - p1); store8<T>(dld + (size_t)(a.M + i) * 8, f);
    f[0] = 1.f / (1.f - pf + eps) * invM * pf * (1.f - pf); store8<T>(dld + (size_t)(2 * a.M + i) * 8, f);
    f[0] = a.gan_weight * (-1.f / (pf + eps)) * invM * pf * (1.f - pf); store8<T>(dlg + (size_t)i * 8, f);
  }
  __shared__ double sm[64];
  block_sum<2>(acc, sm);
  if (threadIdx.x == 0) { a.losses[0] = (float)(acc[0] / a.M); a.losses[1] = (float)(acc[1] / a.M); }
}

template <typename T>
__global__ __launch_bounds__(256) void perceptual_kernel(const PerceptualArgs a) {
  constexpr int E = Elem<T>::E;
  const T* f = reinterpret_cast<const T*>(a.f3);
  T* df = reinterpret_cast<T*>(a.df3);
  const float s = a.l1_weight / (float)a.half;
  double acc[1] = {0};
  const size_t nv = a.half / E;
  for (size_t i = (size_t)blockIdx.x * 256 + threadIdx.x; i < nv; i += (size_t)gridDim.x * 256) {
    float fa[E], fb[E], d[E];
    Elem<T>::unpack(reinterpret_cast<const uint4*>(f)[i], fa);
    Elem<T>::unpack(reinterpret_cast<const uint4*>(f + a.half)[i], fb);
#pragma unroll
    for (int e = 0; e < E; ++e) {
      const float x = fa[e] - fb[e];
      acc[0] += (double)x * x;
      d[e] = (fb[e] > 0.f) ? -s * x : 0.f;
    }
    reinterpret_cast<uint4*>(df)[i] = Elem<T>::pack(d);
  }
  __shared__ double sm[64];
  block_sum<1>(acc, sm);
  if (threadIdx.x == 0) a.partial[blockIdx.x] = acc[0];
}

__global__ __launch_bounds__(256) void loss_final_kernel(const LossFinalArgs a) {
  double v[3] = {0, 0, 0};
  for (int i = threadIdx.x; i < a.n_comp; i += 256) { v[0] += a.comp_partial[2 * i]; v[1] += a.comp_partial[2 * i + 1]; }
  for (int i = threadIdx.x; i < a.n_perc; i += 256) v[2] += a.perc_partial[i];
  __shared__ double sm[64];
  block_sum<3>(v, sm);
  if (threadIdx.x != 0) return;
  const double content = v[2] / 2.0 / a.n_feat;
  const double gl1 = v[0] / a.n_out + v[1] / a.n_out + content;
  a.losses[2] = (float)gl1;
  a.losses[3] = (float)((double)a.losses[1] * a.gan_weight + gl1 * a.l1_weight);
  a.losses[4] = (float)content;
}

template <typename T>
__global__ __launch_bounds__(256) void maxpool_fwd_kernel(const T* __restrict__ x, T* __restrict__ y, int B, int H, int W, int C) {
  constexpr int E = Elem<T>::E;
  const int ncg = C / E, Ho = H / 2, Wo = W / 2;
  const size_t total = (size_t)B * Ho * Wo * ncg;
  for (size_t i = (size_t)blockIdx.x * 256 + threadIdx.x; i < total; i += (size_t)gridDim.x * 256) {
    const int cg = (int)(i % ncg);
    size_t t = i / ncg;
    const int ow = (int)(t % Wo); t /= Wo;
    const int oh = (int)(t % Ho);
    const int n = (int)(t / Ho);
    const T* p = x + (((size_t)n * H + 2 * oh) * W + 2 * ow) * C + cg * E;
    float m[E], v[E];
    Elem<T>::unpack(*reinterpret_cast<const uint4*>(p), m);
    Elem<T>::unpack(*reinterpret_cast<const uint4*>(p + C), v);
#pragma unroll
    for (int e = 0; e < E; ++e) m[e] = fmaxf(m[e], v[e]);
    Elem<T>::unpack(*reinterpret_cast<const uint4*>(p + (size_t)W * C), v);
#pragma unroll
    for (int e = 0; e < E; ++e) m[e] = fmaxf(m[e], v[e]);
    Elem<T>::unpack(*reinterpret_cast<const uint4*>(p + (size_t)W * C + C), v);
#pragma unroll
    for (int e = 0; e < E; ++e) m[e] = fmaxf(m[e], v[e]);
    *reinterpret_cast<uint4*>(y + i * E) = Elem<T>::pack(m);
  }
}

template <typename T>
__global__ __launch_bounds__(256) void maxpool_bwd_kernel(const T* __restrict__ x, const T* __restrict__ dy, T* __restrict__ dx, int B, int H, int W, int C) {
  constexpr int E = Elem<T>::E;
  const int ncg = C / E, Ho = H / 2, Wo = W / 2;
  const size_t total = (size_t)B * Ho * Wo * ncg;
  for (size_t i = (size_t)blockIdx.x * 256 + threadIdx.x; i < total; i += (size_t)gridDim.x * 256) {
    const int cg = (int)(i % ncg);
    size_t t = i / ncg;
    const int ow = (int)(t % Wo); t /= Wo;
    const int oh = (int)(t % Ho);
    const int n = (int)(t / Ho);
    const size_t base = (((size_t)n * H + 2 * oh) * W + 2 * ow) * C + cg * E;
    const size_t offs[4] = {0, (size_t)C, (size_t)W * C, (size_t)W * C + C};
    float v[4][E], g[E];
#pragma unroll
    for (int k = 0; k < 4; ++k) Elem<T>::unpack(*reinterpret_cast<const uint4*>(x + base + offs[k]), v[k]);
    Elem<T>::unpack(*reinterpret_cast<const uint4*>(dy + i * E), g);
    float o[4][E];
#pragma unroll
    for (int e = 0; e < E; ++e) {
      int best = 0;
      float m = v[0][e];
#pragma unroll
      for (int k = 1; k < 4; ++k) if (v[k][e] > m) { m = v[k][e]; best = k; }
#pragma unroll
      for (int k = 0; k < 4; ++k) o[k][e] = (k == best && m > 0.f) ? g[e] : 0.f;
    }
#pragma unroll
    for (int k = 0; k < 4; ++k) *reinterpret_cast<uint4*>(dx + base + offs[k]) = Elem<T>::pack(o[k]);
  }
}

template <typename T>
__global__ __launch_bounds__(256) void maxpool_bwd_code_kernel(const unsigned char* __restrict__ code, const T* __restrict__ dy, T* __restrict__ dx, int B, int H, int W, int C) {
  constexpr int E = Elem<T>::E;
  const int ncg = C / E, Ho = H / 2, Wo = W / 2;
  const size_t total = (size_t)B * Ho * Wo * ncg;
  for (size_t i = (size_t)blockIdx.x * 256 + threadIdx.x; i < total; i += (size_t)gridDim.x * 256) {
    const int cg = (int)(i % ncg);
    size_t t = i / ncg;
    const int ow = (int)(t % Wo); t /= Wo;
    const int oh = (int)(t % Ho);
    const int n = (int)(t / Ho);
    const size_t base = (((size_t)n * H + 2 * oh) * W + 2 * ow) * C + cg * E;
    const size_t offs[4] = {0, (size_t)C, (size_t)W * C, (size_t)W * C + C};
    unsigned cw[2];
    if constexpr (E == 8) { const uint2 c2 = *reinterpret_cast<const uint2*>(code + i * E); cw[0] = c2.x; cw[1] = c2.y; }
    else { cw[0] = *reinterpret_cast<const unsigned*>(code + i * E); cw[1] = 0; }
    float g[E];
    Elem<T>::unpack(*reinterpret_cast<const uint4*>(dy + i * E), g);
    float o[4][E];
#pragma unroll
    for (int e = 0; e < E; ++e) {
// ... 149 lines not shown
  hipLaunchKernelGGL(bn_bwd_finalize_kernel, dim3((a.C + 3) / 4), dim3(256), 0, st, a);
  const size_t work = (size_t)a.G * a.Pg * (a.C / (is_bf16 ? 8 : 4));
  VP_DISPATCH(is_bf16, bn_bwd_apply_kernel, dim3(nblocks(work)), dim3(256), st, a);
  return hipGetLastError();
}

hipError_t launch_bn_bwd_tail(const BnArgs& a, int is_bf16, hipStream_t st) {
  hipLaunchKernelGGL(bn_bwd_finalize_kernel, dim3((a.C + 3) / 4), dim3(256), 0, st, a);
  const size_t work = (size_t)a.G * a.Pg * (a.C / (is_bf16 ? 8 : 4));
  VP_DISPATCH(is_bf16, bn_bwd_apply_kernel, dim3(nblocks(work)), dim3(256), st, a);
  return hipGetLastError();
}

__global__ __launch_bounds__(256) void colsum_finalize_kernel(const BnArgs a, int creal, float* out, int accumulate) {
  const int c = blockIdx.x * 4 + (threadIdx.x >> 6), lane = threadIdx.x & 63;
  if (c >= creal) return;
  double s = 0;
  for (int grp = 0; grp < a.G; ++grp) {
    double s0, s1;
    chunk_sum(a, grp, c, lane, s0, s1);
    s += s0;
  }
  if (lane == 0) out[c] = (float)s + (accumulate ? out[c] : 0.f);
}

hipError_t launch_colsum(const BnArgs& a, int creal, float* out, int accumulate, int is_bf16, hipStream_t st) {
  dim3 grid(a.nchunk, a.G);
  if (is_bf16) hipLaunchKernelGGL((bn_reduce_kernel<bf16, 0>), grid, dim3(256), 0, st, a);
  else hipLaunchKernelGGL((bn_reduce_kernel<float, 0>), grid, dim3(256), 0, st, a);
  hipLaunchKernelGGL(colsum_finalize_kernel, dim3((creal + 3) / 4), dim3(256), 0, st, a, creal, out, accumulate);
  return hipGetLastError();
}

hipError_t launch_colsum_tail(const BnArgs& a, int creal, float* out, int accumulate, hipStream_t st) {
  hipLaunchKernelGGL(colsum_finalize_kernel, dim3((creal + 3) / 4), dim3(256), 0, st, a, creal, out, accumulate);
  return hipGetLastError();
}

hipError_t launch_act_apply(const void* y, const float* sc, const float* sh, int C, int Pg, size_t npix,
                            void* out_lrelu, void* out_relu, int is_bf16, hipStream_t st) {
  const size_t work = npix * (C / (is_bf16 ? 8 : 4));
  if (is_bf16) hipLaunchKernelGGL((act_apply_kernel<bf16>), dim3(nblocks(work)), dim3(256), 0, st, (const bf16*)y, sc, sh, C, Pg, npix, (bf16*)out_lrelu, (bf16*)out_relu);
  else hipLaunchKernelGGL((act_apply_kernel<float>), dim3(nblocks(work)), dim3(256), 0, st, (const float*)y, sc, sh, C, Pg, npix, (float*)out_lrelu, (float*)out_relu);
  return hipGetLastError();
}

hipError_t launch_tap_gather(const TapArgs& a, hipStream_t st) {
  hipLaunchKernelGGL(tap_gather_kernel, dim3((unsigned)(((size_t)a.N * a.Hout * a.Wout + 255) / 256)), dim3(256), 0, st, a);
  return hipGetLastError();
}

hipError_t launch_tap_spread(const TapArgs& a, int is_bf16, hipStream_t st) {
  VP_DISPATCH(is_bf16, tap_spread_kernel, dim3((unsigned)(((size_t)a.N * a.Hin * a.Win + 255) / 256)), dim3(256), st, a);
  return hipGetLastError();
}

hipError_t launch_pack_inputs(const PackInputsArgs& a, int is_bf16, hipStream_t st) {
  VP_DISPATCH(is_bf16, pack_inputs_kernel, dim3(nblocks((size_t)a.N * a.HW)), dim3(256), st, a);
  return hipGetLastError();
}

hipError_t launch_frame_pack(const FramePackArgs& a, hipStream_t st) {
  hipLaunchKernelGGL(frame_pack_kernel, dim3(nblocks((size_t)a.N * a.S * a.S * 2)), dim3(256), 0, st, a);
  return hipGetLastError();
}

int composite_nblocks(int N, int HW) { return nblocks((size_t)N * HW, 1024); }

hipError_t launch_composite_fwd(const CompositeArgs& a, int is_bf16, hipStream_t st) {
  VP_DISPATCH(is_bf16, composite_fwd_kernel, dim3(composite_nblocks(a.N, a.HW)), dim3(256), st, a);
  return hipGetLastError();
}

hipError_t launch_composite_bwd(const CompositeArgs& a, int is_bf16, hipStream_t st) {
  VP_DISPATCH(is_bf16, composite_bwd_kernel, dim3(nblocks((size_t)a.N * a.HW)), dim3(256), st, a);
  return hipGetLastError();
}

hipError_t launch_gan_loss(const GanLossArgs& a, int is_bf16, hipStream_t st) {
  VP_DISPATCH(is_bf16, gan_loss_kernel, dim3(1), dim3(1024), st, a);
  return hipGetLastError();
}

int perceptual_nblocks(size_t half, int is_bf16) { return nblocks(half / (is_bf16 ? 8 : 4), 1024); }

hipError_t launch_perceptual(const PerceptualArgs& a, int is_bf16, hipStream_t st) {
  VP_DISPATCH(is_bf16, perceptual_kernel, dim3(perceptual_nblocks(a.half, is_bf16)), dim3(256), st, a);
  return hipGetLastError();
}

hipError_t launch_loss_final(const LossFinalArgs& a, hipStream_t st) {
  hipLaunchKernelGGL(loss_final_kernel, dim3(1), dim3(256), 0, st, a);
  return hipGetLastError();
}

hipError_t launch_maxpool_fwd(const void* x, void* y, int B, int H, int W, int C, int is_bf16, hipStream_t st) {
  const size_t work = (size_t)B * (H / 2) * (W / 2) * (C / (is_bf16 ? 8 : 4));
  if (is_bf16) hipLaunchKernelGGL((maxpool_fwd_kernel<bf16>), dim3(nblocks(work)), dim3(256), 0, st, (const bf16*)x, (bf16*)y, B, H, W, C);
  else hipLaunchKernelGGL((maxpool_fwd_kernel<float>), dim3(nblocks(work)), dim3(256), 0, st, (const float*)x, (float*)y, B, H, W, C);
  return hipGetLastError();
}

hipError_t launch_maxpool_bwd(const void* x, const void* dy, void* dx, int B, int H, int W, int C, int is_bf16, hipStream_t st) {
  const size_t work = (size_t)B * (H / 2) * (W / 2) * (C / (is_bf16 ? 8 : 4));
  if (is_bf16) hipLaunchKernelGGL((maxpool_bwd_kernel<bf16>), dim3(nblocks(work)), dim3(256), 0, st, (const bf16*)x, (const bf16*)dy, (bf16*)dx, B, H, W, C);
  else hipLaunchKernelGGL((maxpool_bwd_kernel<float>), dim3(nblocks(work)), dim3(256), 0, st, (const float*)x, (const float*)dy, (float*)dx, B, H, W, C);
  return hipGetLastError();
}

hipError_t launch_maxpool_bwd_code(const void* code, const void* dy, void* dx, int B, int H, int W, int C, int is_bf16, hipStream_t st) {
  const size_t work = (size_t)B * (H / 2) * (W / 2) * (C / (is_bf16 ? 8 : 4));
  if (is_bf16) hipLaunchKernelGGL((maxpool_bwd_code_kernel<bf16>), dim3(nblocks(work)), dim3(256), 0, st, (const unsigned char*)code, (const bf16*)dy, (bf16*)dx, B, H, W, C);
  else hipLaunchKernelGGL((maxpool_bwd_code_kernel<float>), dim3(nblocks(work)), dim3(256), 0, st, (const unsigned char*)code, (const float*)dy, (float*)dx, B, H, W, C);
  return hipGetLastError();
}

hipError_t launch_relu_bwd(const void* y, void* d, size_t n, int is_bf16, hipStream_t st) {
  const size_t nvec = n / (is_bf16 ? 8 : 4);
  if (is_bf16) hipLaunchKernelGGL((relu_bwd_kernel<bf16>), dim3(nblocks(nvec)), dim3(256), 0, st, (const bf16*)y, (bf16*)d, nvec);
  else hipLaunchKernelGGL((relu_bwd_kernel<float>), dim3(nblocks(nvec)), dim3(256), 0, st, (const float*)y, (float*)d, nvec);
  return hipGetLastError();
}

hipError_t launch_grad_pack_bf16(const float* src, void* dst, size_t n, hipStream_t st) {
  hipLaunchKernelGGL(grad_pack_bf16_kernel, dim3(nblocks(n / 8 + 1, 4096)), dim3(256), 0, st, src, (bf16*)dst, n / 8, n);
  return hipGetLastError();
}

hipError_t launch_grad_unpack_bf16(const void* src, float* dst, size_t n, float scale, hipStream_t st) {
  hipLaunchKernelGGL(grad_unpack_bf16_kernel, dim3(nblocks(n / 8 + 1, 4096)), dim3(256), 0, st, (const bf16*)src, dst, n / 8, n, scale);
  return hipGetLastError();
}

hipError_t launch_adam(const AdamArgs& a, hipStream_t st) {
  hipLaunchKernelGGL(adam_tf_kernel, dim3(nblocks(a.n, 4096)), dim3(256), 0, st, a);
  return hipGetLastError();
}

}
```

voicepuppet_amd/csrc/pointwise_args.h:

```cpp
#pragma once
#include <stddef.h>
#include <stdint.h>

namespace vp {

struct PackDesc {
  size_t src_off;
  size_t dst_off;
  int nclass, rows_real, rows_pad, ntaps, C, C_real, Kpad;
  int kc;
  int perm;
  int kswap;
  int s_kh, s_kw, s_row, s_ch;
  int8_t kh[4][16];
  int8_t kw[4][16];
};

struct FetchArgs {
  const float* raw3;
  const float* fg3;
  const float* o4;
  void* dst;
  size_t npix;
  int mode;
};

struct BnArgs {
  const void* y;
  const void* dz;
  void* dy;
  int C, G, Pg;
  int nchunk;
  double* partial;
  const float* gamma;
  const float* beta;
  float* aff_a;
  float* aff_b;
  float* mu;
  float* rstd;
  float* c1;
  float* c2;
  float* dgamma;
  float* dbeta;
  int accumulate;
  float eps;
  float* dbias_zero;
  int raw;
};

struct PackInputsArgs {
  const float* inputs;
  const float* fg_inputs;
  void* gin;
  void* gfg;
  void* din;
  void* vin;
  int N, HW, train;
  int fg_c;
};

struct FramePackArgs {
  const unsigned char* ex;
  const unsigned char* cur;
  const int* crops;
  float* inputs;
  float* fg_inputs;
  float* targets;
  float* masks;
  int N, S;
};

struct CompositeArgs {
  const float* y4;
  const float* targets;
  const float* masks;
  float* o4;
  float* outputs;
  float* outputs_fg;
  void* din;
  void* vin;
  double* partial;
  int N, HW, train;
  const void* d_din;
  const void* d_vin;
  void* dy4;
  float l1_weight;
};

struct GanLossArgs {
  const float* logits;
  void* dl_d;
  void* dl_g;
  float* predict;
  float* losses;
  int M;
  float gan_weight;
};

struct PerceptualArgs {
  const void* f3;
  void* df3;
  double* partial;
  size_t half;
  float l1_weight;
};

struct LossFinalArgs {
  const double* comp_partial; int n_comp;
  const double* perc_partial; int n_perc;
  double n_out;
  double n_feat;
  float* losses;
  float l1_weight, gan_weight;
};

struct TapArgs {
  const float* S;
  const float* bias;
  float* y;
  const void* dy;
  void* dyS;
  int N, Hin, Win, Hout, Wout, ks, pad, ld_dy;
};

struct AdamArgs {
  float* p; const float* g; float* m; float* v;
  size_t n;
  float lr_t, beta1, beta2, eps;
};

}
```

Baseline: 4536 frames/s.

## Fold D head tap-gather into multi-block GAN loss kernel and loosen stream waits

Replaces the single-block 1024-thread GAN loss kernel with a grid kernel that writes per-block partial sums, which loss_final then reduces. When the last D layer uses the tap-gemm path, the tap gather and bias add are folded into that loss kernel, so a separate pass over the logits is skipped. New events (ev_loss, ev_perc) let the D backward fork and the split branch wait only on the loss and perceptual kernels rather than on the whole main stream. This adds a partial buffer and more cross-stream event bookkeeping, and the event logic could mis-order work if it is wrong.

```diff
diff --git a/include/vp_hip.h b/include/vp_hip.h
--- a/include/vp_hip.h
+++ b/include/vp_hip.h
@@ -203,6 +203,9 @@
                      void* stream);
 int vp_gan_loss(const float* logits, void* seed_d, void* seed_g, float* predict, float* losses, int m, float gan_weight, int dtype,
                 void* stream);
+size_t vp_gan_loss_head_partials(int m);
+int vp_gan_loss_head(const float* tap_s, const float* bias, float* logits, void* seed_d, void* seed_g, float* predict, float* losses,
+                     double* partial, int n, int hd, float gan_weight, int dtype, void* stream);
 int vp_dwconv7x3_bn_act(const float* x, const float* w, const float* bias, float* y, int b, int h, int wd, int c, void* stream);
 int vp_dwconv7x3_bn_act_t(const void* x, const float* w, const float* bias, void* y, int dtype, int b, int h, int wd, int c, void* stream);
 int vp_conv_first_fwd(const float* x, const float* w, const float* bias, float* y, int b, int h, int w_in, int cout, void* stream);
diff --git a/voicepuppet_amd/_lib.py b/voicepuppet_amd/_lib.py
--- a/voicepuppet_amd/_lib.py
+++ b/voicepuppet_amd/_lib.py
@@ -218,6 +218,8 @@
     "vp_maxpool2x2_bwd_code": (ctypes.c_int, [_P, _P, _P, ctypes.c_int, ctypes.c_int, ctypes.c_int, ctypes.c_int, ctypes.c_int, _P]),
     "vp_composite_fwd": (ctypes.c_int, [_P, _P, _P, _P, _P, ctypes.c_int, ctypes.c_int, _P]),
     "vp_gan_loss": (ctypes.c_int, [_P, _P, _P, _P, _P, ctypes.c_int, ctypes.c_float, ctypes.c_int, _P]),
+    "vp_gan_loss_head_partials": (ctypes.c_size_t, [ctypes.c_int]),
+    "vp_gan_loss_head": (ctypes.c_int, [_P, _P, _P, _P, _P, _P, _P, _P, ctypes.c_int, ctypes.c_int, ctypes.c_float, ctypes.c_int, _P]),
     "vp_dwconv7x3_bn_act": (ctypes.c_int, [_P, _P, _P, _P, ctypes.c_int, ctypes.c_int, ctypes.c_int, ctypes.c_int, _P]),
     "vp_dwconv7x3_bn_act_t": (ctypes.c_int, [_P, _P, _P, _P] + [ctypes.c_int] * 5 + [_P]),
     "vp_conv_first_fwd": (ctypes.c_int, [_P, _P, _P, _P] + [ctypes.c_int] * 4 + [_P]),
diff --git a/voicepuppet_amd/csrc/conv_ops.h b/voicepuppet_amd/csrc/conv_ops.h
--- a/voicepuppet_amd/csrc/conv_ops.h
+++ b/voicepuppet_amd/csrc/conv_ops.h
@@ -117,6 +117,7 @@
 inline int& c64_knob() { static int v = 1; return v; }
 inline int& pool_bwd_fused_knob() { static int v = 1; return v; }
 inline int& cout1_knob() { static int v = 256; return v; }
+inline int& loss_head_knob() { static int v = 1; return v; }
 inline int& wgrad1_rows_knob() { static int v = 512; return v; }
 inline int& dc64_knob() { static int v = 1; return v; }
 inline int& s2c64_knob() { static int v = 512; return v; }
diff --git a/voicepuppet_amd/csrc/launch.h b/voicepuppet_amd/csrc/launch.h
--- a/voicepuppet_amd/csrc/launch.h
+++ b/voicepuppet_amd/csrc/launch.h
@@ -74,6 +74,8 @@
 hipError_t launch_composite_fwd(const CompositeArgs& a, int is_bf16, hipStream_t st);
 hipError_t launch_composite_bwd(const CompositeArgs& a, int is_bf16, hipStream_t st);
 hipError_t launch_gan_loss(const GanLossArgs& a, int is_bf16, hipStream_t st);
+int gan_loss_nblocks(int M);
+hipError_t launch_gan_loss_grid(const GanLossArgs& a, int is_bf16, hipStream_t st);
 int perceptual_nblocks(size_t half, int is_bf16);
 hipError_t launch_perceptual(const PerceptualArgs& a, int is_bf16, hipStream_t st);
 hipError_t launch_loss_final(const LossFinalArgs& a, hipStream_t st);
diff --git a/voicepuppet_amd/csrc/ops_api.hip b/voicepuppet_amd/csrc/ops_api.hip
--- a/voicepuppet_amd/csrc/ops_api.hip
+++ b/voicepuppet_amd/csrc/ops_api.hip
@@ -68,6 +68,7 @@
   if (k == "pool_bwd_fused") { pool_bwd_fused_knob() = value < 0 || value > 4 ? 1 : value; return VP_OK; }
   if (k == "cout1_wgrad_rows" && value > 0) { wgrad1_rows_knob() = value; return VP_OK; }
   if (k == "cout1_bwd") { cout1_knob() = value < 0 ? 256 : value; return VP_OK; }
+  if (k == "loss_head") { loss_head_knob() = value != 0; return VP_OK; }
   if (k == "s2c64") { s2c64_knob() = value; return VP_OK; }
   if (k == "wgrad_big") { wgrad_big_knob() = value; return VP_OK; }
   if (k == "patch4") { patch4_knob() = value; return VP_OK; }
@@ -329,6 +330,25 @@
   return VP_OK;
 }
 
+size_t vp_gan_loss_head_partials(int m) { return m < 1 ? 0 : (size_t)gan_loss_nblocks(m) * 2; }
+
+int vp_gan_loss_head(const float* tap_s, const float* bias, float* logits, void* seed_d, void* seed_g, float* predict, float* losses,
+                     double* partial, int n, int hd, float gan_weight, int dtype, void* stream) {
+  if (!logits || !seed_d || !seed_g || !predict || !losses || !partial || n < 1 || hd < 1 || (tap_s && !bias) || (size_t)n * hd * hd > ((size_t)1 << 28)) {
+    set_err("vp_gan_loss_head: bad argument"); return VP_ERR_ARG;
+  }
+  GanLossArgs ga;
+  memset(&ga, 0, sizeof(ga));
+  ga.logits = logits; ga.dl_d = seed_d; ga.dl_g = seed_g; ga.predict = predict; ga.losses = losses; ga.M = n * hd * hd; ga.gan_weight = gan_weight;
+  ga.partial = partial; ga.S = tap_s; ga.bias = bias; ga.logits_out = logits; ga.Hin = hd + 1; ga.Win = hd + 1; ga.hd = hd; ga.ks = 4; ga.pad = 1;
+  VP_HIP_CHECK(launch_gan_loss_grid(ga, dtype == VP_BF16, (hipStream_t)stream));
+  LossFinalArgs lf;
+  memset(&lf, 0, sizeof(lf));
+  lf.losses = losses; lf.gan_partial = partial; lf.n_gan = gan_loss_nblocks(ga.M); lf.M = ga.M; lf.gan_only = 1;
+  VP_HIP_CHECK(launch_loss_final(lf, (hipStream_t)stream));
+  return VP_OK;
+}
+
 int vp_dwconv7x3_bn_act(const float* x, const float* w, const float* bias, float* y, int b, int h, int wd, int c, void* stream) {
   if (!x || !w || !bias || !y || b < 1 || h < 1 || wd < 1 || c < 4 || (c & 3)) { set_err("vp_dwconv7x3_bn_act: bad argument"); return VP_ERR_ARG; }
   VP_HIP_CHECK(launch_dwconv7x3(x, w, bias, y, 0, b, h, wd, c, (hipStream_t)stream));
diff --git a/voicepuppet_amd/csrc/plan_pixrefer.hip b/voicepuppet_amd/csrc/plan_pixrefer.hip
--- a/voicepuppet_amd/csrc/plan_pixrefer.hip
+++ b/voicepuppet_amd/csrc/plan_pixrefer.hip
@@ -134,6 +134,7 @@
   bool pool_bwd_fused;
   bool pool_dz_stale[2];
   double *comp_partial, *perc_partial, *bn_partial;
+  double* gan_partial;
   char* scratch;
   char* scratch2;
   double* bn_partial2;
@@ -146,6 +147,9 @@
   hipEvent_t ev_b2join;
   bool use_b2;
   hipEvent_t ev_fork, ev_join, ev_bfork, ev_bjoin;
+  hipEvent_t ev_loss, ev_perc;
+  bool head_fold;
+  bool head_ev;
   hipEvent_t ev_upd_b, ev_upd_m;
   bool overlap, forked;
   int bst_count;
@@ -161,7 +165,7 @@
   int dfork_pending;
   void* zeros;
   size_t scratch_bytes;
-  int n_comp, n_perc;
+  int n_comp, n_perc, n_gan;
   struct { bool active, d_done; float *m_g, *v_g, *m_d, *v_d; float lr_t_g, lr_t_d, beta1, beta2, eps; } upd;
   int upd_mask;
   bool params_dirty;
@@ -534,6 +538,8 @@
     h->n_perc = perceptual_nblocks((size_t)N * (H / 4) * (H / 4) * 256, h->bf16);
     h->comp_partial = (double*)ar.alloc((size_t)h->n_comp * 2 * sizeof(double));
     h->perc_partial = (double*)ar.alloc((size_t)h->n_perc * sizeof(double));
+    h->n_gan = gan_loss_nblocks(N * (H / 8 - 2) * (H / 8 - 2));
+    h->gan_partial = (double*)ar.alloc((size_t)h->n_gan * 2 * sizeof(double));
   }
   h->zeros = ar.alloc(256);
   h->bn_partial = (double*)ar.alloc((size_t)1024 * 2 * 512 * sizeof(double));
@@ -747,7 +753,7 @@
   }
   profile_tag((L.scope + ":fwd").c_str());
   VP_HIP_CHECK(launch_igemm(a, h->bf16, L.fwd.cfg, st));
-  if (L.tapgemm) {
+  if (L.tapgemm && !(h->head_fold && &n == &h->D)) {
     TapArgs ta;
     memset(&ta, 0, sizeof(ta));
     ta.S = L.tap_S; ta.bias = n.params + L.b_off; ta.y = (float*)to.y;
@@ -1185,6 +1191,8 @@
     const size_t M = (size_t)d->batch * hd * hd;
     region_of(h->din, 3 * px * 8 * es, "din"); region_of(h->vin, 2 * px * 8 * es, "vin");
     region_of(h->logits, 3 * M * 4, "logits"); region_of(h->predict, 2 * M * 4, "predict");
+    region_of(h->gan_partial, (size_t)gan_loss_nblocks((int)M) * 2 * sizeof(double), "gan_partial");
+    if (h->n_gan != gan_loss_nblocks((int)M)) fail("gan_partial: %d rows carved, the loss kernel launches %d blocks", h->n_gan, gan_loss_nblocks((int)M));
     region_of(h->dl_d, 3 * M * 8 * es, "dl_d"); region_of(h->dl_g, M * 8 * es, "dl_g");
     region_of(h->d_din, px * 8 * es, "d_din"); region_of(h->d_vin, px * 8 * es, "d_vin"); region_of(h->dy4, px * 8 * es, "dy4");
     for (const Tens& t : h->V.t) {
@@ -1276,6 +1284,8 @@
     VP_HIP_CHECK(hipEventCreateWithFlags(&h->ev_b2join, hipEventDisableTiming));
     VP_HIP_CHECK(hipEventCreateWithFlags(&h->ev_bfork, hipEventDisableTiming));
     VP_HIP_CHECK(hipEventCreateWithFlags(&h->ev_bjoin, hipEventDisableTiming));
+    VP_HIP_CHECK(hipEventCreateWithFlags(&h->ev_loss, hipEventDisableTiming));
+    VP_HIP_CHECK(hipEventCreateWithFlags(&h->ev_perc, hipEventDisableTiming));
     VP_HIP_CHECK(hipEventCreateWithFlags(&h->ev_upd_b, hipEventDisableTiming));
     VP_HIP_CHECK(hipEventCreateWithFlags(&h->ev_upd_m, hipEventDisableTiming));
     h->overlap = true;
@@ -1296,6 +1306,8 @@
     (void)hipEventDestroy(h->ev_bjoin);
     (void)hipEventDestroy(h->ev_b2join);
     if (h->branch2) (void)hipStreamSynchronize(h->branch2);
+    (void)hipEventDestroy(h->ev_loss);
+    (void)hipEventDestroy(h->ev_perc);
     (void)hipEventDestroy(h->ev_upd_b);
     (void)hipEventDestroy(h->ev_upd_m);
   }
@@ -1407,13 +1419,28 @@
     VP_HIP_CHECK(hipEventRecord(h->ev_bfork, st));
     VP_HIP_CHECK(hipStreamWaitEvent(h->branch, h->ev_bfork, 0));
   }
-  for (Layer& L : h->D.l) if ((rc = run_layer_fwd(h, h->D, L, sd, nullptr, ssd))) return rc;
+  const bool head = loss_head_knob() != 0;
+  const Layer& L5 = h->D.l.back();
+  h->head_fold = head && L5.tapgemm;
+  for (Layer& L : h->D.l) if ((rc = run_layer_fwd(h, h->D, L, sd, nullptr, ssd))) { h->head_fold = false; return rc; }
   const int hd = H / 8 - 2;
   GanLossArgs ga;
   memset(&ga, 0, sizeof(ga));
   ga.logits = h->logits; ga.dl_d = h->dl_d; ga.dl_g = h->dl_g; ga.predict = h->predict; ga.losses = h->losses;
   ga.M = N * hd * hd; ga.gan_weight = d.gan_weight;
-  VP_HIP_CHECK(launch_gan_loss(ga, bf, sd));
+  if (head) {
+    ga.partial = h->gan_partial; ga.hd = hd;
+    if (h->head_fold) {
+      ga.S = L5.tap_S; ga.bias = h->D.params + L5.b_off; ga.logits_out = h->logits;
+      ga.Hin = L5.g.Hin; ga.Win = L5.g.Win; ga.ks = L5.g.ks; ga.pad = L5.g.pad;
+    }
+    VP_HIP_CHECK(launch_gan_loss_grid(ga, bf, sd));
+  } else {
+    VP_HIP_CHECK(launch_gan_loss(ga, bf, sd));
+  }
+  h->head_fold = false;
+  h->head_ev = head && h->overlap;
+  if (h->head_ev) VP_HIP_CHECK(hipEventRecord(h->ev_loss, sd));
   if (split_d) VP_HIP_CHECK(hipEventRecord(h->ev_bjoin, h->branch));
 
   Net& V = h->V;
@@ -1457,10 +1484,12 @@
   memset(&pa, 0, sizeof(pa));
   pa.f3 = f3.y; pa.df3 = f3.dz; pa.partial = h->perc_partial; pa.half = f3.elems() / 2; pa.l1_weight = d.l1_weight;
   VP_HIP_CHECK(launch_perceptual(pa, bf, st));
+  if (h->head_ev) VP_HIP_CHECK(hipEventRecord(h->ev_perc, st));
 
   if (split_d) VP_HIP_CHECK(hipStreamWaitEvent(st, h->ev_bjoin, 0));
   LossFinalArgs lf;
   memset(&lf, 0, sizeof(lf));
+  if (head) { lf.gan_partial = h->gan_partial; lf.n_gan = h->n_gan; lf.M = ga.M; }
   lf.comp_partial = h->comp_partial; lf.n_comp = h->n_comp; lf.perc_partial = h->perc_partial; lf.n_perc = h->n_perc;
   lf.n_out = (double)N * H * H * 3; lf.n_feat = (double)pa.half; lf.losses = h->losses;
   lf.l1_weight = d.l1_weight; lf.gan_weight = d.gan_weight;
@@ -1470,7 +1499,7 @@
 }
 
 static int backward_d_on(vp_pixrefer_t* h, hipStream_t st, bool side);
-static int fork_d(vp_pixrefer_t* h, hipStream_t st);
+static int fork_d(vp_pixrefer_t* h, hipStream_t st, bool at_start = false);
 
 static int update_range(vp_pixrefer_t* h, Net& n, float* m, float* v, float lr_t, size_t off0, size_t off1, int l0, int l1, hipStream_t s) {
   if (off1 > off0) {
@@ -1498,7 +1527,7 @@
   }
   int rc;
   h->dfork_pending = h->dfork_point;
-  if (h->dfork_pending == 0 && (rc = fork_d(h, st))) { h->dfork_pending = 0; return rc; }
+  if (h->dfork_pending == 0 && (rc = fork_d(h, st, true))) { h->dfork_pending = 0; return rc; }
   rc = vp_pixrefer_backward_g(h, stream);
   h->dfork_pending = 0;
   if (rc) return rc;
@@ -1507,10 +1536,14 @@
   return VP_OK;
 }
 
-static int fork_d(vp_pixrefer_t* h, hipStream_t st) {
+static int fork_d(vp_pixrefer_t* h, hipStream_t st, bool at_start) {
   h->dfork_pending = 0;
-  VP_HIP_CHECK(hipEventRecord(h->ev_fork, st));
-  VP_HIP_CHECK(hipStreamWaitEvent(h->side, h->ev_fork, 0));
+  if (at_start && h->head_ev) {
+    VP_HIP_CHECK(hipStreamWaitEvent(h->side, h->ev_loss, 0));
+  } else {
+    VP_HIP_CHECK(hipEventRecord(h->ev_fork, st));
+    VP_HIP_CHECK(hipStreamWaitEvent(h->side, h->ev_fork, 0));
+  }
   int rc = backward_d_on(h, h->side, true);
   if (rc) return rc;
   if (h->upd.active && h->dfork_point == 2 && (rc = update_d(h, h->side))) return rc;
@@ -1575,7 +1608,7 @@
   h->forked = h->overlap && h->ov_on;
   if (!h->forked) return backward_d_on(h, st, false);
   h->dfork_pending = h->dfork_point;
-  if (h->dfork_pending == 0) return fork_d(h, st);
+  if (h->dfork_pending == 0) return fork_d(h, st, true);
   return VP_OK;
 }
 
@@ -1662,9 +1695,15 @@
   const bool split_d = h->overlap && h->ov_on && h->dsplit_on;
   hipStream_t sd = split_d ? h->branch : st;
   const int ssd = split_d ? 2 : 0;
-  if (split_d) {
+  if (split_d && h->head_ev) {
+    VP_HIP_CHECK(hipStreamWaitEvent(h->branch, h->ev_loss, 0));
+  } else if (split_d) {
     VP_HIP_CHECK(hipEventRecord(h->ev_bfork, st));
     VP_HIP_CHECK(hipStreamWaitEvent(h->branch, h->ev_bfork, 0));
+  }
+  if (h->head_ev) {
+    if (!split_d) VP_HIP_CHECK(hipStreamWaitEvent(st, h->ev_loss, 0));
+    VP_HIP_CHECK(hipStreamWaitEvent(st, h->ev_perc, 0));
   }
   for (Tens& t : D.t) { t.dz2_written = false; t.bst_chunks_g = 0; }
   for (int i = (int)D.l.size() - 1; i >= 0; --i) {
@@ -1820,6 +1859,8 @@
   const int hd = H / 8 - 2;
   if (s == "Predict") return ret(h->predict, 2, N, hd, hd, VP_F32);
   if (s == "logits") return ret(h->logits, 3 * N, hd, hd, 1, VP_F32);
+  if (s == "dl_d") return ret(h->dl_d, 3 * N, hd, hd, 8, cd);
+  if (s == "dl_g") return ret(h->dl_g, N, hd, hd, 8, cd);
   if (s == "d_gen_out4") return ret(h->dy4, N, H, H, 8, cd);
   if (s == "d_din") return ret(h->d_din, N, H, H, 8, cd);
   if (s == "d_vin") return ret(h->d_vin, N, H, H, 8, cd);
diff --git a/voicepuppet_amd/csrc/pointwise.hip b/voicepuppet_amd/csrc/pointwise.hip
--- a/voicepuppet_amd/csrc/pointwise.hip
+++ b/voicepuppet_amd/csrc/pointwise.hip
@@ -450,22 +450,26 @@
   }
 }
 
+__device__ __forceinline__ float tap_gather_at(const float* __restrict__ S, int Hin, int Win, int ks, int pad, int n, int i, int j) {
+  float acc = 0.f;
+  for (int kh = 0; kh < ks; ++kh) {
+    const int qi = i + kh - pad;
+    if (qi < 0 || qi >= Hin) continue;
+    for (int kw = 0; kw < ks; ++kw) {
+      const int qj = j + kw - pad;
+      if (qj < 0 || qj >= Win) continue;
+      acc += S[(((size_t)n * Hin + qi) * Win + qj) * 16 + kh * ks + kw];
+    }
+  }
+  return acc;
+}
+
 __global__ __launch_bounds__(256) void tap_gather_kernel(TapArgs a) {
   const size_t total = (size_t)a.N * a.Hout * a.Wout;
   const size_t p = (size_t)blockIdx.x * 256 + threadIdx.x;
   if (p >= total) return;
   const int j = (int)(p % a.Wout), i = (int)((p / a.Wout) % a.Hout), n = (int)(p / ((size_t)a.Wout * a.Hout));
-  float acc = 0.f;
-  for (int kh = 0; kh < a.ks; ++kh) {
-    const int qi = i + kh - a.pad;
-    if (qi < 0 || qi >= a.Hin) continue;
-    for (int kw = 0; kw < a.ks; ++kw) {
-      const int qj = j + kw - a.pad;
-      if (qj < 0 || qj >= a.Win) continue;
-      acc += a.S[(((size_t)n * a.Hin + qi) * a.Win + qj) * 16 + kh * a.ks + kw];
-    }
-  }
-  a.y[p] = acc + a.bias[0];
+  a.y[p] = tap_gather_at(a.S, a.Hin, a.Win, a.ks, a.pad, n, i, j) + a.bias[0];
 }
 
 template <typename T>
@@ -644,30 +648,58 @@
 }
 
 template <typename T>
-__global__ __launch_bounds__(1024) void gan_loss_kernel(const GanLossArgs a) {
+__device__ __forceinline__ void gan_loss_elem(const GanLossArgs& a, int i, float l0, float l1, float lf, double (&acc)[2]) {
   const float eps = 1e-12f;
-  double acc[2] = {0, 0};
   const float invM = 1.f / (float)a.M;
   T* dld = reinterpret_cast<T*>(a.dl_d);
   T* dlg = reinterpret_cast<T*>(a.dl_g);
-  for (int i = threadIdx.x; i < a.M; i += 1024) {
-    const float p0 = 1.f / (1.f + expf(-a.logits[i]));
-    const float p1 = 1.f / (1.f + expf(-a.logits[a.M + i]));
-    const float pf = 1.f / (1.f + expf(-a.logits[2 * a.M + i]));
-    const float pr = (p0 + p1) * 0.5f;
-    a.predict[i] = pr; a.predict[a.M + i] = pf;
-    acc[0] += -(logf(pr + eps) * 2.f + logf(1.f - pf + eps));
-    acc[1] += -logf(pf + eps);
-    const float dpr = -2.f / (pr + eps) * invM * 0.5f;
-    float f[8] = {0, 0, 0, 0, 0, 0, 0, 0};
-    f[0] = dpr * p0 * (1.f - p0); store8<T>(dld + (size_t)i * 8, f);
-    f[0] = dpr * p1 * (1.f - p1); store8<T>(dld + (size_t)(a.M + i) * 8, f);
-    f[0] = 1.f / (1.f - pf + eps) * invM * pf * (1.f - pf); store8<T>(dld + (size_t)(2 * a.M + i) * 8, f);
-    f[0] = a.gan_weight * (-1.f / (pf + eps)) * invM * pf * (1.f - pf); store8<T>(dlg + (size_t)i * 8, f);
-  }
+  const float p0 = 1.f / (1.f + expf(-l0));
+  const float p1 = 1.f / (1.f + expf(-l1));
+  const float pf = 1.f / (1.f + expf(-lf));
+  const float pr = (p0 + p1) * 0.5f;
+  a.predict[i] = pr; a.predict[a.M + i] = pf;
+  acc[0] += -(logf(pr + eps) * 2.f + logf(1.f - pf + eps));
+  acc[1] += -logf(pf + eps);
+  const float dpr = -2.f / (pr + eps) * invM * 0.5f;
+  float f[8] = {0, 0, 0, 0, 0, 0, 0, 0};
+  f[0] = dpr * p0 * (1.f - p0); store8<T>(dld + (size_t)i * 8, f);
+  f[0] = dpr * p1 * (1.f - p1); store8<T>(dld + (size_t)(a.M + i) * 8, f);
+  f[0] = 1.f / (1.f - pf + eps) * invM * pf * (1.f - pf); store8<T>(dld + (size_t)(2 * a.M + i) * 8, f);
+  f[0] = a.gan_weight * (-1.f / (pf + eps)) * invM * pf * (1.f - pf); store8<T>(dlg + (size_t)i * 8, f);
+}
+
+template <typename T>
+__global__ __launch_bounds__(1024) void gan_loss_kernel(const GanLossArgs a) {
+  double acc[2] = {0, 0};
+  for (int i = threadIdx.x; i < a.M; i += 1024) gan_loss_elem<T>(a, i, a.logits[i], a.logits[a.M + i], a.logits[2 * a.M + i], acc);
   __shared__ double sm[64];
   block_sum<2>(acc, sm);
   if (threadIdx.x == 0) { a.losses[0] = (float)(acc[0] / a.M); a.losses[1] = (float)(acc[1] / a.M); }
+}
+
+template <typename T>
+__global__ __launch_bounds__(256) void gan_loss_grid_kernel(const GanLossArgs a) {
+  double acc[2] = {0, 0};
+  const int hw = a.hd * a.hd;
+  for (int i = blockIdx.x * 256 + threadIdx.x; i < a.M; i += gridDim.x * 256) {
+    float l[3];
+    if (a.S) {
+      const int n = i / hw, r = i - n * hw, y = r / a.hd, x = r - y * a.hd;
+      const int N = a.M / hw;
+      const float b = a.bias[0];
+#pragma unroll
+      for (int g = 0; g < 3; ++g) {
+        l[g] = tap_gather_at(a.S, a.Hin, a.Win, a.ks, a.pad, g * N + n, y, x) + b;
+        a.logits_out[g * a.M + i] = l[g];
+      }
+    } else {
+      l[0] = a.logits[i]; l[1] = a.logits[a.M + i]; l[2] = a.logits[2 * a.M + i];
+    }
+    gan_loss_elem<T>(a, i, l[0], l[1], l[2], acc);
+  }
+  __shared__ double sm[64];
+  block_sum<2>(acc, sm);
+  if (threadIdx.x == 0) { a.partial[blockIdx.x * 2] = acc[0]; a.partial[blockIdx.x * 2 + 1] = acc[1]; }
 }
 
 template <typename T>
@@ -696,16 +728,25 @@
 }
 
 __global__ __launch_bounds__(256) void loss_final_kernel(const LossFinalArgs a) {
-  double v[3] = {0, 0, 0};
+  double v[5] = {0, 0, 0, 0, 0};
   for (int i = threadIdx.x; i < a.n_comp; i += 256) { v[0] += a.comp_partial[2 * i]; v[1] += a.comp_partial[2 * i + 1]; }
   for (int i = threadIdx.x; i < a.n_perc; i += 256) v[2] += a.perc_partial[i];
-  __shared__ double sm[64];
-  block_sum<3>(v, sm);
+  if (a.gan_partial) for (int i = threadIdx.x; i < a.n_gan; i += 256) { v[3] += a.gan_partial[2 * i]; v[4] += a.gan_partial[2 * i + 1]; }
+  __shared__ double sm[80];
+  block_sum<5>(v, sm);
   if (threadIdx.x != 0) return;
+  float gan = 0.f;
+  if (a.gan_partial) {
+    a.losses[0] = (float)(v[3] / a.M);
+    a.losses[1] = gan = (float)(v[4] / a.M);
+    if (a.gan_only) return;
+  } else {
+    gan = a.losses[1];
+  }
   const double content = v[2] / 2.0 / a.n_feat;
   const double gl1 = v[0] / a.n_out + v[1] / a.n_out + content;
   a.losses[2] = (float)gl1;
-  a.losses[3] = (float)((double)a.losses[1] * a.gan_weight + gl1 * a.l1_weight);
+  a.losses[3] = (float)((double)gan * a.gan_weight + gl1 * a.l1_weight);
   a.losses[4] = (float)content;
 }
 
@@ -1021,6 +1062,13 @@
   return hipGetLastError();
 }
 
+int gan_loss_nblocks(int M) { const int b = (M + 255) / 256; return b < 256 ? b : 256; }
+
+hipError_t launch_gan_loss_grid(const GanLossArgs& a, int is_bf16, hipStream_t st) {
+  VP_DISPATCH(is_bf16, gan_loss_grid_kernel, dim3(gan_loss_nblocks(a.M)), dim3(256), st, a);
+  return hipGetLastError();
+}
+
 int perceptual_nblocks(size_t half, int is_bf16) { return nblocks(half / (is_bf16 ? 8 : 4), 1024); }
 
 hipError_t launch_perceptual(const PerceptualArgs& a, int is_bf16, hipStream_t st) {
diff --git a/voicepuppet_amd/csrc/pointwise_args.h b/voicepuppet_amd/csrc/pointwise_args.h
--- a/voicepuppet_amd/csrc/pointwise_args.h
+++ b/voicepuppet_amd/csrc/pointwise_args.h
@@ -95,6 +95,11 @@
   float* losses;
   int M;
   float gan_weight;
+  double* partial;
+  const float* S;
+  const float* bias;
+  float* logits_out;
+  int Hin, Win, hd, ks, pad;
 };
 
 struct PerceptualArgs {
@@ -112,6 +117,9 @@
   double n_feat;
   float* losses;
   float l1_weight, gan_weight;
+  const double* gan_partial; int n_gan;
+  int M;
+  int gan_only;
 };
 
 struct TapArgs {
```

Result: no change. 4567 frames/s, median of 6 (+0.7%).
